# TeamOfProfGuo/Few_Shot_Seg_CWT

Measured on AMD Instinct MI355X. Metric: episodes/sec (473x473, 1-shot, R50) at 1/2/4/8 MI355X; mIoU vs ref, higher is better.
Workload: dtype fp32 (conv stack at fp32 width on the bf16 MFMA: every fp32 operand split exactly into bf16 hi + mid + lo, the six products >= 2^-24 |a||b| summed in fp32; inner loop, CWT, classifier fp32); 1 GPU; CWT inference episode (validate_transformer, batch_size_val=1): PASCAL split-0 1-shot ResNet-50 PSPNet 473x473, adapt_iter 200, heads 4; image_size=473, shot=1, layers=50

## Files before the change

### few_shot_seg_cwt_amd/_lib.py

```python
from __future__ import annotations

import ctypes as C
import os
import threading

import torch

_HERE = os.path.dirname(os.path.abspath(__file__))
LIB_PATH = os.environ.get("CWT_LIB_PATH") or os.path.join(_HERE, "libcwt.so")

_P = C.c_void_p
_I = C.c_int
_F = C.c_float
_I64 = C.c_int64

SIGNATURES = {
    "cwt_version": (C.c_char_p, []),
    "cwt_last_error": (C.c_char_p, []),
    "cwt_ctx_create": (_I, [_I, C.POINTER(_P)]),
    "cwt_ctx_destroy": (_I, [_P]),
    "cwt_backbone_load": (_I, [_P, _I, _I, C.POINTER(C.c_char_p), C.POINTER(_P), C.POINTER(_I64), _F,
                               C.POINTER(_P)]),
    "cwt_backbone_destroy": (_I, [_P]),
    "cwt_backbone_set_precision": (_I, [_P, _I]),
    "cwt_extract_features": (_I, [_P, _P, _P, _I, _I, _P, _P]),
    "cwt_extract_features_train_bn": (_I, [_P, _P, _P, _I, _I, _P, _F, _F, C.c_uint64, _P]),
    "cwt_backbone_read_bn": (_I, [_P, C.c_char_p, _P, _I]),
    "cwt_preprocess_image": (_I, [_P, _P, _I, _I, _I, _I, C.POINTER(_F), C.POINTER(_F), C.POINTER(_F), _I, _I, _P,
                                  _P]),
    "cwt_preprocess_label": (_I, [_P, _P, _I, _I, _I, _I, _I, _I, _P, _P]),
    "cwt_workspace_bytes": (C.c_size_t, [_P]),
    "cwt_inner_adapt": (_I, [_P, _P, _P, _I, _I, _I, _I, _I, _F, _I, _P, _P]),
    "cwt_inner_adapt_batch": (_I, [_P, _P, _P, _I, _I, _I, _I, _I, _I, _F, _I, _P, _P]),
    "cwt_normalize": (_I, [_P, _P, _I, _I, _I, _P, _P, _P, _P]),
    "cwt_attention_fwd": (_I, [_P, _P, _P, _I, _I, _I, _I, _P, _P, _P, _P, _P, _P, _P, _P]),
    "cwt_attention_saved_floats": (C.c_size_t, [_I, _I, _I, _I]),
    "cwt_attention_bwd": (_I, [_P, _P, _P, _I, _I, _I, _I, _P, _P, _P, _P, _P, _P, _P, _P, _P, _P, _P, _P, _P]),
    "cwt_attention_fwd_train": (_I, [_P, _P, _P, _I, _I, _I, _I, _P, _P, _P, _P, _P, _P, _P, _F, _F, C.c_uint64,
                                     _P]),
    "cwt_attention_bwd_train": (_I, [_P, _P, _P, _I, _I, _I, _I, _P, _P, _P, _P, _P, _P, _P, _P, _P, _P, _P, _P, _F,
                                     _F, C.c_uint64, _P]),
    "cwt_classify": (_I, [_P, _P, _P, _I, _I, _I, _P, _P]),
    "cwt_attention_infer": (_I, [_P, _P, _P, _I, _I, _I, _I, _P, _P, _P, _P, _P, _I64, _P, _P, _P, _P]),
    "cwt_classify_scaled": (_I, [_P, _P, _P, _P, _I, _I, _I, _P, _P]),
    "cwt_episode_tail": (_I, [_P, _P, _P, _I, _I, _I, _I, _P, _P, _P, _P, _P, _P, _I64, _P, _P, _P, _P, _P, _P,
                              _P]),
    "cwt_inner_adapt_tail": (_I, [_P, _P, _P, _I, _I, _I, _I, _I, _F, _I, _P, _P, _P, _P, _P, _P, _P, _P, _I64, _P, _P,
                                  _P, _P, _P, _P, _P]),
    "cwt_seg_metrics": (_I, [_P, _P, _P, _I, _I, _I, _I, _P, _P, _P]),
    "cwt_seg_metrics_pair": (_I, [_P, _P, _P, _P, _I, _I, _I, _I, _P, _P, _P, _P]),
    "cwt_seg_ce_fwd_bwd": (_I, [_P, _P, _P, _I, _I, _I, _I, _P, _P, _P]),
    "cwt_classify_bwd": (_I, [_P, _P, _P, _I, _I, _I, _P, _P]),
    "cwt_iou_preds": (_I, [_P, _P, _P, _I64, _I, _I, _P, _P]),
    "cwt_cos_classify": (_I, [_P, _P, _I, _I, _I, _I, _P, _P, _P, _P, _I, _P, _P]),
    "cwt_cos_classify_bwd": (_I, [_P, _P, _I, _I, _I, _I, _P, _P, _P, _P, _I, _P, _P, _P, _P, _P, _P]),
    "cwt_corr": (_I, [_P, _P, _P, _I, _I, _I, _I, _P, _P]),
    "cwt_mutual_matching": (_I, [_P, _P, _I, _I, _I, _I, _P, _P]),
    "cwt_match_corr_forward": (_I, [_P, _P, _I, _I, _I, _I, _P, _I, _F, _P, _I, _P, _P, _P]),
    "cwt_match_corr_forward_cv4": (_I, [_P, _P, _I, _I, _I, _I, _P, _I, _F, _P, _I, _P, _P, _P]),
    "cwt_match_masks": (_I, [_P, _P, _I, _I, _I, _P, _P, _P, _P]),
    "cwt_channel_sum": (_I, [_P, _P, _I, _I, _I64, _P, _P]),
    "cwt_sce_descriptor": (_I, [_P, _P, _I, _I, _I, _I, _I, _I, _P, _P]),
    "cwt_match_readout": (_I, [_P, _P, _I, _I, _I, _F, _P, _I, _P, _P]),
    "cwt_match_masks_train": (_I, [_P, _P, _I, _I, _I, _P, _P, _P, _F, C.c_uint64, _P]),
    "cwt_match_readout_backward": (_I, [_P, _P, _I, _I, _I, _F, _P, _I, _P, _P, _P, _P, _P]),
    "cwt_weight_average": (_I, [_P, _P, _I, _I, _I, _I, _P, _P, _P, _P, _P, _P, _P, _P]),
    "cwt_mmn_blend": (_I, [_P, _P, _P, _I, _I64, _F, _P, _P, _P]),
    "cwt_match_corr_saved_floats": (_I, [_I, _I, _I, _I, _I, _I, C.POINTER(_I64)]),
    "cwt_match_corr_forward_train": (_I, [_P, _P, _I, _I, _I, _I, _P, _I, _F, _P, _I, _P, _P, _P, _P]),
    "cwt_match_corr_backward": (_I, [_P, _P, _I, _I, _I, _I, _P, _I, _F, _P, _I, _P, _P, _P, _P, _P, _P, _P]),
    "cwt_corr_backward": (_I, [_P, _P, _P, _I, _I, _I, _I, _P, _P, _P, _I, _I, _P]),
    "cwt_weight_average_train": (_I, [_P, _P, _I, _I, _I, _I, _P, _P, _P, _P, _P, _P, _P, _P, _P, _P]),
    "cwt_weight_average_backward": (_I, [_P, _P, _I, _I, _I, _I, _P, _P, _P, _P, _P, _P, _P, _P, _P, _P, _P, _P, _P,
                                         _P, _P, _P]),
    "cwt_mmn_blend_backward": (_I, [_P, _P, _P, _I, _I64, _F, _P, _P, _P]),
    "cwt_linear_backward": (_I, [_P, _P, _I64, _I, _P, _I, _P, _P, _P, _P, _I, _P, _P]),
    "cwt_deform_attn_backward": (_I, [_P, _P, _P, _P, _I, _I, _I, _I, _I, _I, _P, _P, _P, _P, _P]),
    "cwt_norm_blend_backward": (_I, [_P, _P, _P, _I64, _I, _F, _P, _P, _P, _P]),
    "cwt_linear": (_I, [_P, _P, _I64, _I, _P, _P, _I, _I, _I, _P, _P]),
    "cwt_sine_pos_add": (_I, [_P, _P, _I, _I, _I, _I, _F, _I, _F, _F, _P, _P]),
    "cwt_deform_attn": (_I, [_P, _P, _P, _P, _I, _I, _I, _I, _I, _I, _P, _P]),
    "cwt_norm_blend": (_I, [_P, _P, _P, _I64, _I, _F, _P, _P]),
    "cwt_extract_features_mid": (_I, [_P, _P, _P, _I, _I, _P, _P, _P, _P, _P]),
    "cwt_sgd_step": (_I, [_P, _P, _P, _P, _I64, _F, _F, _F, _I, _I, _P]),
    "cwt_pretrain_create": (_I, [_P, _I, _I, _I, C.POINTER(C.c_char_p), C.POINTER(_P), C.POINTER(_I64), _F,
                                 C.POINTER(_P)]),
    "cwt_pretrain_destroy": (_I, [_P]),
    "cwt_pretrain_step": (_I, [_P, _P, _P, _P, _I, _I, _P, _P, _P]),
    "cwt_pretrain_forward": (_I, [_P, _P, _P, _I, _I, _I, _P, _P]),
    "cwt_pretrain_get": (_I, [_P, C.c_char_p, _I, _P, _I64]),
    "cwt_pretrain_evaluate": (_I, [_P, _P, _P, _P, _I, _I, _I, _P, _P, _P]),
    "cwt_pretrain_set": (_I, [_P, C.c_char_p, _I, _P, _I64]),
    "cwt_pretrain_num_params": (_I, [_P, C.POINTER(_I64), C.POINTER(_I64)]),
    "cwt_cu_count": (_I, [_P, _P]),
    "cwt_adapt_workgroups": (_I, [_P, _I, _I, _I, _I, _I, _P]),
    "cwt_adapt_fuses_tail": (_I, [_P, _I, _I, _I, _I, _P]),
    "cwt_stream_create_masked": (_I, [_P, _P, _I, _P]),
    "cwt_stream_destroy": (_I, [_P]),
    "cwt_debug_conv": (_I, [_P, _P, _I, _I, _I, _I, _I, _P, _P, _P, _I, _I, _I, _I, _I, _P, _I, _I, _P, _I, _I,
                            _I, _I, _I, _I, _P]),
    "cwt_debug_split_act": (_I, [_P, _P, _I64, _I, _I, _P, _P]),
    "cwt_debug_unsplit_act": (_I, [_P, _P, _I64, _I, _P, _I, _P]),
    "cwt_debug_pack_wsplit": (_I, [_P, _P, _I, _I, _I, _P, _P]),
    "cwt_debug_conv_s": (_I, [_P, _P, _I, _I, _I, _I, _P, _P, _P, _I, _I, _I, _I, _I, _P, _I, _P, _I, _P, _I, _I,
                              _P, _I, _I, _I, _P]),
    "cwt_debug_conv_b16": (_I, [_P, _P, _I, _I, _I, _I, _P, _P, _P, _I, _I, _I, _I, _I, _P, _I, _P, _I, _P, _I, _I,
                                _P, _I, _I, _I, _P]),
    "cwt_debug_cp4d_layer": (_I, [_P, _P, _I, _I, _I, _I, _I, _I, _I, _P, _P, _P, _P, _P, _I, _P]),
    "cwt_debug_conv_f32d": (_I, [_P, _P, _I, _I, _I, _I, _P, _P, _P, _I, _I, _I, _I, _I, _P, _I, _I, _P, _I, _I, _I,
                                 _I, _I, _P]),
    "cwt_debug_conv_x6": (_I, [_P, _P, _I, _I, _I, _I, _P, _P, _P, _I, _I, _I, _I, _I, _P, _I, _I, _P, _I, _I, _I,
                               _I, _I, _P]),
    "cwt_debug_conv_x6w": (_I, [_P, _P, _I, _I, _I, _I, _P, _P, _P, _I, _I, _I, _I, _I, _P, _I, _I, _P, _I, _I, _I,
                                _I, _I, _P]),
    "cwt_debug_conv_form": (_I, [_I, _I, _I, _I, C.POINTER(_I)]),
    "cwt_debug_conv_plan": (_I, [_I, _I, _I, _I, _I, C.POINTER(_I)]),
    "cwt_debug_census": (_I, [_P, _I, _P, _P]),
    "cwt_debug_tail_stamps": (_I, [_P, _P, _I64, _P]),
    "cwt_debug_occupy": (_I, [_P, _I, _I, _P]),
    "cwt_debug_pretrain_op": (_I, [_P, _I, C.POINTER(_P), C.POINTER(_I64), C.POINTER(_F), _P]),
    "cwt_debug_backbone_op": (_I, [_P, _I, C.POINTER(_P), C.POINTER(_I64), C.POINTER(_F), _P]),
    "cwt_debug_adapt_stamps": (_I, [_P, _P, _I64, C.POINTER(_I64)]),
    "cwt_ctx_set_adapt_units": (_I, [_P, _I]),
    "cwt_ctx_status": (_I, [_P, C.POINTER(C.c_uint32), _I]),
    "cwt_ctx_set_conv_arith": (_I, [_P, _I]),
    "cwt_debug_adapt_spin_limit": (_I, [_P, _I64]),
    "cwt_debug_pretrain_capture": (_I, [_P, _I]),
    "cwt_debug_pretrain_tensor": (_I, [_P, C.c_char_p, _P, _I64]),
    "cwt_profile_enable": (_I, [_P, _I]),
    "cwt_profile_count": (_I, [_P]),
    "cwt_profile_record": (_I, [_P, _I, C.c_char_p, _I, C.POINTER(C.c_double), C.POINTER(C.c_double),
                                C.POINTER(_F)]),
}

_lib = None
_lock = threading.RLock()
_ctx = {}


class CwtError(RuntimeError):
    pass


def check_provenance(version: str, path: str):
    from . import build as _build
    if os.environ.get("CWT_LIB_PATH") or not os.path.isdir(_build.CSRC):
        return
    want = _build.source_hash()
    got = version.rsplit("src=", 1)[-1] if "src=" in version else None
    if got != want:
        raise CwtError(f"{path} is stale: built from sources {got}, the tree's are {want}; "
                       "run `python -m few_shot_seg_cwt_amd.build`")


def load_library(path: str = LIB_PATH):
    global _lib
    with _lock:
        if _lib is None:
            if not os.path.exists(path):
                raise CwtError(f"{path} not built: run `python -m few_shot_seg_cwt_amd.build` "
                               "(the product path has no CPU fallback)")
            lib = C.CDLL(path)
            for name, (res, args) in SIGNATURES.items():
                fn = getattr(lib, name)
                fn.restype = res
                fn.argtypes = args
            check_provenance(lib.cwt_version().decode(), path)
            _lib = lib
    return _lib


def lib():
    return load_library()


def check(rc: int, what: str = ""):
    if rc != 0:
        msg = lib().cwt_last_error().decode(errors="replace")
        raise CwtError(f"{what} failed (code {rc}): {msg}")


_override = threading.local()
_extra_ctx = {}


def _create_ctx(device: int):
    p = C.c_void_p()
    rc = load_library().cwt_ctx_create(device, C.byref(p))
    if rc != 0:
        raise CwtError(f"cwt_ctx_create failed: {_lib.cwt_last_error().decode()}")
    return p


def ctx(device: int | None = None):
    if not torch.cuda.is_available():
        raise CwtError("libcwt needs a HIP device (torch.cuda.is_available() is False); no CPU fallback")
    if device is None:
        device = torch.cuda.current_device()
    sel = getattr(_override, "ctx", None)
    if sel is not None and sel[0] == device:
        return sel[1]
    with _lock:
        if device not in _ctx:
            _ctx[device] = _create_ctx(device)
        return _ctx[device]


def new_ctx(device: int | None = None):
    if device is None:
        device = torch.cuda.current_device()
    ctx(device)
    with _lock:
        p = _create_ctx(device)
        _extra_ctx.setdefault(device, []).append(p)
        return p


def destroy_ctx(p, device: int | None = None) -> None:
    if device is None:
        device = torch.cuda.current_device()
    with _lock:
        lst = _extra_ctx.get(device, [])
        for i, q in enumerate(lst):
            if q is p or getattr(q, "value", None) == getattr(p, "value", p):
                del lst[i]
                check(load_library().cwt_ctx_destroy(p), "cwt_ctx_destroy")
                return
    raise CwtError("destroy_ctx: not an additional context of this device")


class using_ctx:

    def __init__(self, c, device: int | None = None):
        self.c, self.device = c, torch.cuda.current_device() if device is None else device

    def __enter__(self):
        self.prev = getattr(_override, "ctx", None)
        _override.ctx = (self.device, self.c)
        return self.c

    def __exit__(self, *exc):
        _override.ctx = self.prev
        return False


def all_ctx(device: int | None = None):
    if device is None:
        device = torch.cuda.current_device()
    return [ctx(device)] + list(_extra_ctx.get(device, []))


STATUS_ADAPT_BARRIER = 1
STATUS_TAIL_BARRIER = 2


def check_status(device: int | None = None, clear: bool = True) -> None:
    w = C.c_uint32()
    bad = 0
    for c in all_ctx(device):
        check(lib().cwt_ctx_status(c, C.byref(w), int(clear)), "cwt_ctx_status")
        bad |= w.value
    if bad & STATUS_TAIL_BARRIER:
        raise CwtError("the fused episode tail's grid barrier timed out (its workgroups were not all co-resident): "
                       "the CWT output, logits and IoU counts of an episode on this device are wrong")
    if bad & STATUS_ADAPT_BARRIER:
        raise CwtError("the persistent inner loop's grid barrier timed out (its workgroups were not all "
                       "co-resident): the adapted classifier W of an episode on this device is wrong")
# ... 77 lines not shown
```

### few_shot_seg_cwt_amd/csrc/api_debug.hip

```cpp
#include <algorithm>
#include <cstdlib>

#include "../../include/cwt_debug.h"
#include "conv_forms.h"
#include "ctx.h"

using namespace cwt;

namespace cwt {
__global__ void census_kernel(unsigned* out) {
  unsigned hw, xcc;
  asm volatile("s_getreg_b32 %0, hwreg(HW_REG_HW_ID)" : "=s"(hw));
  asm volatile("s_getreg_b32 %0, hwreg(HW_REG_XCC_ID)" : "=s"(xcc));
  if (threadIdx.x == 0) {
    out[2 * blockIdx.x] = hw;
    out[2 * blockIdx.x + 1] = xcc;
  }
}
}

static int debug_conv_s(cwt_ctx* ctx, int prec, const void* xs, int N, int Hi, int Wi, int Ci, const void* ws,
                        const float* scale, const float* shift, int Co, int k, int stride, int pad, int dil,
                        const float* res, int res_ld, const void* res_s, int relu, float* y, int y_ld, int y_off,
                        void* ys, int bm, int bn, int nsplit, void* stream) {
// ... 96 lines not shown
  return launch_conv(a, p, 0, part, pf, (hipStream_t)stream);
}

int cwt_debug_census(cwt_ctx* ctx, int nblocks, unsigned* out, void* stream) {
  if (!ctx) return fail(CWT_EARG, "ctx is NULL");
  CWT_CHECK(out && nblocks > 0, "bad arguments");
  CWT_HIP(hipSetDevice(ctx->device));
  hipLaunchKernelGGL(census_kernel, dim3(nblocks), dim3(64), 0, (hipStream_t)stream, out);
  CWT_LAUNCH_CHECK();
  return 0;
}

int cwt_debug_split_act(cwt_ctx* ctx, const float* x, int64_t P, int C, int ld, void* out, void* stream) {
  if (!ctx) return fail(CWT_EARG, "ctx is NULL");
  CWT_CHECK(x && out && P >= 0 && C % 32 == 0 && ld >= C && ld % 4 == 0, "bad arguments");
  CWT_HIP(hipSetDevice(ctx->device));
  return launch_split_act(x, P, C, ld, (__bf16*)out, (hipStream_t)stream);
}

int cwt_debug_unsplit_act(cwt_ctx* ctx, const void* s, int64_t P, int C, float* out, int ld, void* stream) {
  if (!ctx) return fail(CWT_EARG, "ctx is NULL");
  CWT_CHECK(s && out && P >= 0 && C % 32 == 0 && ld >= C && ld % 4 == 0, "bad arguments");
  CWT_HIP(hipSetDevice(ctx->device));
  return launch_unsplit_act((const __bf16*)s, P, C, out, ld, (hipStream_t)stream);
}

int cwt_debug_pack_wsplit(cwt_ctx* ctx, const float* w, int Co, int k, int Ci, void* out, void* stream) {
  if (!ctx) return fail(CWT_EARG, "ctx is NULL");
  CWT_CHECK(w && out && Co > 0 && Ci % 32 == 0 && (k == 1 || k == 3), "bad arguments");
  CWT_HIP(hipSetDevice(ctx->device));
  float* wp;
  int rc;
  const long K = (long)k * k * Ci;
  if ((rc = ws(ctx, "dbg.wpack", (size_t)Co * K, &wp))) return rc;
  if ((rc = launch_repack_cblock(w, wp, Co, k * k, Ci, (hipStream_t)stream))) return rc;
  return launch_split_act(wp, Co, (int)K, (int)K, (__bf16*)out, (hipStream_t)stream);
}

int cwt_debug_backbone_op(cwt_ctx* ctx, int op, void* const* b, const int64_t* ia, const float* fa, void* stream) {
  if (!ctx) return fail(CWT_EARG, "ctx is NULL");
  CWT_CHECK(b && ia, "null argument");
  CWT_HIP(hipSetDevice(ctx->device));
  hipStream_t st = (hipStream_t)stream;
  auto lay_ok = [](int64_t l) { return l == ACT_F32 || l == ACT_SPLIT || l == ACT_BF16; };
  float* p;
  int rc;
  if (op == 0) {
    const int N = (int)ia[0], S = (int)ia[1];
    CWT_CHECK(b[0] && b[1] && b[2] && b[3] && b[4] && N > 0 && S > 0 && lay_ok(ia[2]), "stem conv1");
    return launch_stem_conv1((const float*)b[0], N, S, (const float*)b[1], (const float*)b[2], (const float*)b[3],
                             (float*)b[4], down2(S), st, (int)ia[2], (int)ia[3]);
  }
  if (op == 1) {
    const int N = (int)ia[0], H = (int)ia[1], W = (int)ia[2], C = (int)ia[3], lay = (int)ia[4];
    CWT_CHECK(b[0] && b[1] && N > 0 && H > 0 && W > 0 && C > 0 && lay_ok(ia[4]), "maxpool");
    const int Ho = down2(H), Wo = down2(W);
    if (lay == ACT_BF16) return launch_maxpool3s2_b16((const __bf16*)b[0], N, H, W, C, (__bf16*)b[1], Ho, Wo, st);
    if (lay == ACT_SPLIT) return launch_maxpool3s2_s((const __bf16*)b[0], N, H, W, C, (__bf16*)b[1], Ho, Wo, st);
    CWT_CHECK(C % 4 == 0, "maxpool: C % 4");
    return launch_maxpool3s2((const float*)b[0], N, H, W, C, (float*)b[1], Ho, Wo, st);
  }
  if (op == 2) {
    const int N = (int)ia[0], h = (int)ia[1], w = (int)ia[2], ld = (int)ia[3];
    CWT_CHECK(b[0] && b[1] && N > 0 && h > 0 && w > 0 && ld >= 2048 && lay_ok(ia[4]), "ppm");
    if ((rc = ws(ctx, "dbg.ppm", ((size_t)N * h * 16 + (size_t)N * 256) * 2048, &p))) return rc;
    return launch_ppm((const float*)b[0], N, h, w, ld, kBins, 4, p, (float*)b[1], st, (int)ia[4]);
  }
  if (op == 3) {
    int M[4];
    const float *Bt[4], *sc[4], *sh[4];
    long Mtot = 0;
    int nbn = 0;
    for (int q = 0; q < 4; ++q) {
      CWT_CHECK(ia[q] > 0 && ia[q] <= 4096 && b[1 + q], "ppm gemm: problem");
      M[q] = (int)ia[q];
      Mtot += M[q];
      Bt[q] = (const float*)b[1 + q];
      sc[q] = (const float*)b[5 + q];
      sh[q] = (const float*)b[9 + q];
      CWT_CHECK(!sc[q] == !sh[q], "ppm gemm: scale without shift");
      nbn += sc[q] != nullptr;
    }
    const int N = (int)ia[4], K = (int)ia[5], kc = (int)ia[6];
    int form = (int)ia[7];
    CWT_CHECK(b[0] && b[13] && N > 0 && K > 0 && (nbn == 0 || nbn == 4) && form <= 1, "ppm gemm");
    if (form < 0) form = Mtot <= kPpmGemmMaxRows ? 0 : 1;
    CWT_CHECK(form == 0 || kc == 32 || kc == 64, "ppm gemm: K chunk");
    const size_t part_floats = (size_t)(form == 0 ? 8 : K / kc) * Mtot * N;
    if ((rc = ws(ctx, "dbg.parts", part_floats, &p))) return rc;
    return form == 0 ? launch_ppm_gemm((const float*)b[0], K, Bt, M, 4, N, K, nbn ? sc : nullptr, nbn ? sh : nullptr,
                                       p, part_floats, (float*)b[13], st)
                     : launch_smallm_gemm((const float*)b[0], K, Bt, M, 4, N, K, kc, p, part_floats,
                                          nbn ? sc : nullptr, nbn ? sh : nullptr, (float*)b[13], st);
  }
  if (op == 4) {
    CWT_CHECK(fa && b[0] && b[2] && b[3] && b[4] && ia[0] > 0 && ia[1] > 0 && ia[1] <= 2048 && lay_ok(ia[2]) &&
                  ia[6] > 0,
              "bn_train");
    BnTrainArgs a;
    memset(&a, 0, sizeof(a));
    a.y = b[0];
    a.M = (long)ia[0];
    a.C = (int)ia[1];
    a.layout = (int)ia[2];
    a.ld = (int)ia[3];
    a.res = b[1];
    a.res_ld = (int)ia[4];
    a.relu = (int)ia[5];
    a.rows_per_image = (long)ia[6];
    a.seed = (unsigned long long)ia[7];
    a.bn = (float*)b[2];
    a.scale = (float*)b[3];
    a.shift = (float*)b[4];
    a.eps = fa[0];
    a.momentum = fa[1];
    a.drop_p = fa[2];
    CWT_CHECK(a.layout != ACT_F32 || a.ld >= a.C, "bn_train: ld < C");
    const size_t pf = bn_train_part_floats(a.M, a.C);
    float* bsc;
    if ((rc = ws(ctx, "dbg.bn.part", pf, &p)) || (rc = ws(ctx, "dbg.bn.bsc", 2 * 2048, &bsc))) return rc;
    return launch_bn_train(a, p, pf, bsc, st);
  }
  if (op == 5) {
    CWT_CHECK(b[0] && b[1] && ia[0] > 0, "widen");
    return launch_widen_bf16((const __bf16*)b[0], (long)ia[0], (float*)b[1], st);
  }
  return fail(CWT_EARG, "cwt_debug_backbone_op: unknown op");
}

int cwt_debug_conv_s(cwt_ctx* ctx, const void* xs, int N, int Hi, int Wi, int Ci, const void* ws, const float* scale,
                     const float* shift, int Co, int k, int stride, int pad, int dil, const float* res, int res_ld,
                     const void* res_s, int relu, float* y, int y_ld, int y_off, void* ys, int bm, int bn, int nsplit,
                     void* stream) {
  return debug_conv_s(ctx, 3, xs, N, Hi, Wi, Ci, ws, scale, shift, Co, k, stride, pad, dil, res, res_ld, res_s, relu, y,
                      y_ld, y_off, ys, bm, bn, nsplit, stream);
}

int cwt_debug_conv_f32d(cwt_ctx* ctx, const float* x, int N, int Hi, int Wi, int Ci, const float* w_packed,
                        const float* scale, const float* shift, int Co, int k, int stride, int pad, int dil,
                        const float* res, int res_ld, int relu, float* y, int y_ld, int y_off, int bm, int bn,
                        int nsplit, void* stream) {
  return debug_conv_s(ctx, 0, x, N, Hi, Wi, Ci, w_packed, scale, shift, Co, k, stride, pad, dil, res, res_ld, nullptr,
                      relu, y, y_ld, y_off, nullptr, bm, bn, nsplit, stream);
}

int cwt_debug_conv_x6(cwt_ctx* ctx, const float* x, int N, int Hi, int Wi, int Ci, const float* w_packed,
                      const float* scale, const float* shift, int Co, int k, int stride, int pad, int dil,
                      const float* res, int res_ld, int relu, float* y, int y_ld, int y_off, int bm, int bn,
                      int nsplit, void* stream) {
  return debug_conv_s(ctx, 6, x, N, Hi, Wi, Ci, w_packed, scale, shift, Co, k, stride, pad, dil, res, res_ld, nullptr,
                      relu, y, y_ld, y_off, nullptr, bm, bn, nsplit, stream);
}

int cwt_debug_conv_form(int prec, int bm, int bn, int var, int* out4) {
  CWT_CHECK(out4, "out4 is NULL");
  const ConvForm* f = find_conv_form(prec, bm, bn, var);
  if (!f) return fail(CWT_EARG, "no such conv form (conv_forms.h)");
  out4[0] = f->waves_m;
  out4[1] = f->waves_n;
  out4[2] = f->nstg;
  out4[3] = f->pf;
  return 0;
}

int cwt_debug_conv_plan(int prec, int M, int Co, int K, int batch, int* out5) {
  CWT_CHECK(out5 && M > 0 && Co > 0 && K > 0 && batch >= 0, "bad arguments");
  CWT_CHECK(prec == 0 || prec == 1 || prec == 3 || prec == 6, "prec must be 0, 1, 3 or 6");
  const ConvPlan p = plan_conv_s(prec, M, Co, K, batch);
  const int v[5] = {p.bm, p.bn, p.var, p.nsplit, p.kt_per_split};
  std::copy(v, v + 5, out5);
  if (!find_conv_form(prec, p.bm, p.bn, p.var)) return fail(CWT_EARG, "the plan's form is no such conv form");
  return 0;
}

int cwt_debug_conv_x6w(cwt_ctx* ctx, const float* x, int N, int Hi, int Wi, int Ci, const float* w_packed,
                       const float* scale, const float* shift, int Co, int k, int stride, int pad, int dil,
                       const float* res, int res_ld, int relu, float* y, int y_ld, int y_off, int bm, int bn,
                       int nsplit, void* stream) {
  const int m = nsplit == 4 ? 4 : 2;
  if (!ctx) return fail(CWT_EARG, "ctx is NULL");
  CWT_CHECK(x && w_packed && scale && shift && y, "null buffer");
  CWT_CHECK(nsplit == 0 || nsplit == 1 || nsplit == 2 || nsplit == 4, "nsplit (the Winograd tile) must be 0, 2 or 4");
  CWT_CHECK(k == 3 && stride == 1 && pad == dil && dil >= 1, "winograd form: 3x3, stride 1, padding = dilation");
  CWT_CHECK(Ci % 32 == 0 && Co % 64 == 0 && N >= 1 && Hi >= 1 && Wi >= 1, "need Ci % 32 == 0, Co % 64 == 0");
  CWT_CHECK(y_ld >= y_off + Co && y_ld % 4 == 0 && y_off % 4 == 0 && (!res || res_ld % 4 == 0), "bad strides");
  int rc;
  ConvPlan named;
  if (bm > 0 && (rc = force_conv_form(6, bm, bn, Co, &named))) return rc;
  CWT_HIP(hipSetDevice(ctx->device));
  const hipStream_t st = (hipStream_t)stream;
  const int P = (m + 2) * (m + 2);
  const size_t n = (size_t)P * Co * Ci;
  float* U;
  __bf16 *us, *ul;
  if ((rc = ws(ctx, "dbg.wU", n, &U)) || (rc = ws(ctx, "dbg.wUs", n * 2, &us)) || (rc = ws(ctx, "dbg.wUl", n, &ul)))
    return rc;
  static const bool w3_cache = getenv("CWT_DBG_W3_CACHE") && getenv("CWT_DBG_W3_CACHE")[0] == '1';
  static const void* u_src = nullptr;
  static long u_n = 0;
  static void* u_dst = nullptr;
  if (!(w3_cache && u_src == w_packed && u_n == (long)n * m && u_dst == us)) {
    if ((rc = launch_wino_weights(w_packed, Co, Ci, U, st, m)) ||
        (rc = launch_split_w3(U, (long)P * Co, Ci, us, ul, st)))
      return rc;
    u_src = w_packed;
    u_n = (long)n * m;
    u_dst = us;
  }
  return run_wino_conv(ctx, x, N, Hi, Wi, Ci, Co, dil, m, us, ul, scale, shift, res, res_ld, relu, y, y_ld, y_off, 0,
                       st, bm, bn);
}

int cwt_debug_conv_b16(cwt_ctx* ctx, const void* xs, int N, int Hi, int Wi, int Ci, const void* ws, const float* scale,
                       const float* shift, int Co, int k, int stride, int pad, int dil, const float* res, int res_ld,
                       const void* res_s, int relu, float* y, int y_ld, int y_off, void* ys, int bm, int bn,
                       int nsplit, void* stream) {
  return debug_conv_s(ctx, 1, xs, N, Hi, Wi, Ci, ws, scale, shift, Co, k, stride, pad, dil, res, res_ld, res_s, relu, y,
                      y_ld, y_off, ys, bm, bn, nsplit, stream);
}

int cwt_debug_cp4d_layer(cwt_ctx* ctx, const float* x, int B, int hA, int wA, int hB, int wB, int cin, int cout,
                         const float* Wa, const float* ba, const float* Wb, const float* bb, float* y, int variant,
                         void* stream) {
  if (!ctx || !x || !Wa || !ba || !Wb || !bb || !y) return fail(CWT_EARG, "null argument");
  if (B < 1 || hA < 1 || wA < 1 || hB < 1 || wB < 1) return fail(CWT_EARG, "bad shape");
  return launch_cp4d_layer_variant(x, B, hA, wA, hB, wB, cin, cout, Wa, ba, Wb, bb, y, variant, (hipStream_t)stream);
}

int cwt_debug_occupy(cwt_ctx* ctx, int nwg, int us, void* stream) {
  if (!ctx) return fail(CWT_EARG, "ctx is NULL");
  CWT_CHECK(nwg >= 1 && nwg <= 256 && us >= 1 && us <= 100000, "occupy: 1 <= nwg <= 256, 1 <= us <= 100000");
  CWT_HIP(hipSetDevice(ctx->device));
  return launch_occupy(nwg, us, (hipStream_t)stream);
}

int cwt_debug_tail_stamps(cwt_ctx* ctx, unsigned long long* host_out, int64_t max_count, int64_t* count) {
  if (!ctx || !count) return fail(CWT_EARG, "null argument");
  CWT_HIP(hipSetDevice(ctx->device));
  auto it = ctx->ws.find("tail.stamps");
  *count = (it == ctx->ws.end() || !ctx->tail_stamp_G) ? 0 : (int64_t)ctx->tail_stamp_G * 16;
  if (host_out && *count > 0 && max_count > 0) {
    CWT_HIP(hipDeviceSynchronize());
    CWT_HIP(hipMemcpy(host_out, it->second.p, (size_t)std::min<int64_t>(max_count, *count) * 8, hipMemcpyDeviceToHost));
  }
  return 0;
}

int cwt_debug_adapt_stamps(cwt_ctx* ctx, unsigned long long* host_out, int64_t max_count, int64_t* count) {
  if (!ctx || !count) return fail(CWT_EARG, "null argument");
  CWT_HIP(hipSetDevice(ctx->device));
  *count = g_adapt_stamps ? g_adapt_stamps_n : 0;
  if (host_out && g_adapt_stamps && max_count > 0) {
    CWT_HIP(hipDeviceSynchronize());
    CWT_HIP(hipMemcpy(host_out, g_adapt_stamps, (size_t)std::min<int64_t>(max_count, g_adapt_stamps_n) * 8,
                      hipMemcpyDeviceToHost));
  }
  return 0;
}

int cwt_debug_adapt_spin_limit(cwt_ctx* ctx, int64_t limit) {
  if (!ctx) return fail(CWT_EARG, "ctx is NULL");
  CWT_CHECK(limit >= 0, "limit must be >= 0");
  ctx->adapt_spin_limit = (long)limit;
  return 0;
}

}
```

### few_shot_seg_cwt_amd/csrc/api_extract.hip

```cpp
#include <algorithm>
#include <cmath>
#include <cstdlib>

#include "conv_forms.h"
#include "ctx.h"

namespace cwt {

struct Block {
  ConvLayer c1, c2, c3, down;
  bool has_down = false;
};

struct Backbone {
  int layers = 0;
  int device = 0;
  int precision = CWT_CONV_FP32;
  ConvLayer stem[3];
  std::vector<Block> blocks[4];
  ConvLayer ppm[4];
  float* ppm_wt[4] = {};
  ConvLayer bott;
  float* ppm_q[4] = {};
  float* ppm_q_raw[4] = {};
  float* ones = nullptr;
  float* zeros = nullptr;
  float eps = 1e-5f;
  std::map<std::string, std::pair<float*, int>> bn_by_name;
  std::vector<void*> allocs;
};

struct HostParams {
  std::map<std::string, std::pair<const float*, int64_t>> m;
  const float* get(const std::string& k, int64_t numel, std::string* err) const {
    auto it = m.find(k);
    if (it == m.end() || it->second.first == nullptr) {
      *err = "missing tensor '" + k + "'";
      return nullptr;
    }
    if (it->second.second != numel) {
      *err = "tensor '" + k + "' has " + std::to_string(it->second.second) + " elements, expected " +
             std::to_string(numel);
      return nullptr;
    }
    return it->second.first;
  }
};

static int upload(Backbone* bb, const std::vector<float>& v, float** out) {
  void* p = nullptr;
  CWT_HIP(hipMalloc(&p, v.size() * sizeof(float)));
  CWT_HIP(hipMemcpy(p, v.data(), v.size() * sizeof(float), hipMemcpyHostToDevice));
  bb->allocs.push_back(p);
  *out = (float*)p;
  return 0;
}

static uint16_t bf16_rne(float f) {
  uint32_t u;
  memcpy(&u, &f, 4);
  if ((u & 0x7F800000u) == 0x7F800000u) return (uint16_t)(u >> 16);
  u += 0x7FFFu + ((u >> 16) & 1u);
  return (uint16_t)(u >> 16);
}

static float bf16_to_float(uint16_t h) {
  uint32_t u = (uint32_t)h << 16;
  float f;
  memcpy(&f, &u, 4);
  return f;
}

static int upload_u16(Backbone* bb, const std::vector<uint16_t>& v, __bf16** out) {
  void* p = nullptr;
  CWT_HIP(hipMalloc(&p, v.size() * sizeof(uint16_t)));
  CWT_HIP(hipMemcpy(p, v.data(), v.size() * sizeof(uint16_t), hipMemcpyHostToDevice));
  bb->allocs.push_back(p);
  *out = (__bf16*)p;
  return 0;
}

static int load_conv(Backbone* bb, const HostParams& hp, const std::string& wname, const std::string& bnp, int Ci,
                     int Co, int k, int stride, int pad, int dil, float eps, bool stem1, ConvLayer* L,
                     int ci_total = -1, int ci_off = 0) {
  if (ci_total < 0) ci_total = Ci;
  std::string err;
  const float* w = hp.get(wname, (int64_t)Co * ci_total * k * k, &err);
  if (!w) return fail(CWT_EARG, err);
  const float* g = hp.get(bnp + ".weight", Co, &err);
  const float* b = g ? hp.get(bnp + ".bias", Co, &err) : nullptr;
  const float* rm = b ? hp.get(bnp + ".running_mean", Co, &err) : nullptr;
  const float* rv = rm ? hp.get(bnp + ".running_var", Co, &err) : nullptr;
  if (!rv) return fail(CWT_EARG, err);
  L->Ci = Ci;
  L->Co = Co;
  L->k = k;
  L->stride = stride;
  L->pad = pad;
  L->dil = dil;
  const int K = k * k * Ci;
  std::vector<float> packed((size_t)Co * K);
  for (int co = 0; co < Co; ++co)
    for (int ci = 0; ci < Ci; ++ci)
      for (int ky = 0; ky < k; ++ky)
        for (int kx = 0; kx < k; ++kx) {
          const float v = w[(((size_t)co * ci_total + ci_off + ci) * k + ky) * k + kx];
          if (stem1)
            packed[((size_t)(ci * 9 + ky * 3 + kx)) * Co + co] = v;
          else
            packed[(size_t)co * K + packed_k(ci, ky * k + kx, k * k)] = v;
        }
  std::vector<float> sc(Co), sh(Co);
  for (int c = 0; c < Co; ++c) {
    const float invstd = 1.0f / std::sqrt(rv[c] + eps);
    sc[c] = g[c] * invstd;
    sh[c] = b[c] - rm[c] * sc[c];
  }
  int rc;
  if ((rc = upload(bb, packed, &L->w))) return rc;
  if (!stem1) {
    std::vector<uint16_t> hi(packed.size()), lo(packed.size()), lo3(packed.size());
    for (size_t i = 0; i < packed.size(); ++i) {
      const float v = packed[i];
      hi[i] = bf16_rne(v);
      const float r = v - bf16_to_float(hi[i]);
      lo[i] = bf16_rne(r);
      lo3[i] = bf16_rne(r - bf16_to_float(lo[i]));
    }
    std::vector<uint16_t> sl(2 * packed.size());
    for (size_t r = 0; r < (size_t)Co; ++r)
      for (int kb = 0; kb < K / 32; ++kb)
        for (int i = 0; i < 32; ++i) {
          const size_t src = r * K + kb * 32 + i, dst = (r * (K / 32) + kb) * 64 + i;
          sl[dst] = hi[src];
          sl[dst + 32] = lo[src];
        }
    if ((rc = upload_u16(bb, sl, &L->w_s))) return rc;
    if (K % 32 == 0 && (rc = upload_u16(bb, lo3, &L->w_l))) return rc;
    static const bool wino4 = getenv("CWT_WINO") && getenv("CWT_WINO")[0] == '4';
    if (k == 3 && stride == 1 && Ci >= 128 && Ci % 32 == 0) {
      for (const int m : {2, 4}) {
        if ((m == 2 && Ci < 256) || (m == 4 && !wino4)) continue;
        const int P = (m + 2) * (m + 2);
        const size_t n = (size_t)P * Co * Ci;
        void *U = nullptr, *us = nullptr, *ul = nullptr;
        CWT_HIP(hipMalloc(&us, n * 4));
        bb->allocs.push_back(us);
        CWT_HIP(hipMalloc(&ul, n * 2));
        bb->allocs.push_back(ul);
        CWT_HIP(hipMalloc(&U, n * 4));
        rc = launch_wino_weights(L->w, Co, Ci, (float*)U, nullptr, m);
        if (!rc) rc = launch_split_w3((const float*)U, (long)P * Co, Ci, (__bf16*)us, (__bf16*)ul, nullptr);
        const hipError_t e = hipDeviceSynchronize();
        (void)hipFree(U);
        if (rc) return rc;
        if (e != hipSuccess) return fail((int)e, "winograd weight transform");
        (m == 2 ? L->wino_s : L->wino4_s) = (__bf16*)us;
        (m == 2 ? L->wino_l : L->wino4_l) = (__bf16*)ul;
      }
    }
    if (Ci % 64 == 0) {
      std::vector<uint16_t> b16(packed.size());
      for (int co = 0; co < Co; ++co)
        for (int ci = 0; ci < Ci; ++ci)
          for (int tap = 0; tap < k * k; ++tap)
            b16[(size_t)co * K + packed_k64(ci, tap, k * k)] = hi[(size_t)co * K + packed_k(ci, tap, k * k)];
      if ((rc = upload_u16(bb, b16, &L->w_b))) return rc;
    }
  }
  if ((rc = upload(bb, sc, &L->scale))) return rc;
  if ((rc = upload(bb, sh, &L->shift))) return rc;
  std::vector<float> bnp4((size_t)4 * Co);
  for (int c = 0; c < Co; ++c) {
    bnp4[c] = g[c];
    bnp4[Co + c] = b[c];
    bnp4[2 * Co + c] = rm[c];
    bnp4[3 * Co + c] = rv[c];
  }
  if ((rc = upload(bb, bnp4, &L->bn))) return rc;
  bb->bn_by_name[bnp] = {L->bn, Co};
  return 0;
}

static int load_ppm_fold(Backbone* bb, const HostParams& hp, float eps) {
  std::string err;
  for (int b = 0; b < 4; ++b) {
    const float* w = hp.get("ppm.features." + std::to_string(b) + ".1.weight", (int64_t)512 * 2048, &err);
    if (!w) return fail(CWT_EARG, err);
    std::vector<float> t((size_t)2048 * 512);
    for (int co = 0; co < 512; ++co)
      for (int ci = 0; ci < 2048; ++ci) t[(size_t)ci * 512 + co] = w[(size_t)co * 2048 + ci];
    int rc;
    if ((rc = upload(bb, t, &bb->ppm_wt[b]))) return rc;
  }
  const float* w = hp.get("bottleneck.0.weight", (int64_t)512 * 4096 * 9, &err);
  const float* g = w ? hp.get("bottleneck.1.weight", 512, &err) : nullptr;
  const float* rv = g ? hp.get("bottleneck.1.running_var", 512, &err) : nullptr;
  if (!rv) return fail(CWT_EARG, err);
  for (int b = 0; b < 4; ++b) {
    std::vector<float> q((size_t)512 * 4608), qr((size_t)512 * 4608);
    for (int co = 0; co < 512; ++co) {
      const float sc = g[co] * (1.0f / std::sqrt(rv[co] + eps));
      for (int ci = 0; ci < 512; ++ci)
        for (int tap = 0; tap < 9; ++tap) {
          const float v = w[((size_t)co * 4096 + 2048 + 512 * b + ci) * 9 + tap];
          qr[(size_t)ci * 4608 + tap * 512 + co] = v;
          q[(size_t)ci * 4608 + tap * 512 + co] = v * sc;
        }
    }
    int rc;
    if ((rc = upload(bb, q, &bb->ppm_q[b])) || (rc = upload(bb, qr, &bb->ppm_q_raw[b]))) return rc;
  }
  return 0;
}

static int load_backbone(int layers, const HostParams& hp, float eps, Backbone** out) {
  if (layers != 50 && layers != 101) return fail(CWT_EARG, "layers must be 50 or 101");
  Backbone* bb = new Backbone();
  bb->layers = layers;
  bb->eps = eps;
  int rc = 0;
  auto cleanup = [&]() {
    for (void* p : bb->allocs) (void)hipFree(p);
    delete bb;
  };
  if ((rc = load_conv(bb, hp, "layer0.0.weight", "layer0.1", 3, 64, 3, 2, 1, 1, eps, true, &bb->stem[0])) ||
      (rc = load_conv(bb, hp, "layer0.3.weight", "layer0.4", 64, 64, 3, 1, 1, 1, eps, false, &bb->stem[1])) ||
      (rc = load_conv(bb, hp, "layer0.6.weight", "layer0.7", 64, 128, 3, 1, 1, 1, eps, false, &bb->stem[2]))) {
    cleanup();
    return rc;
  }
  const int* nb = (layers == 50) ? kBlocks50 : kBlocks101;
  int inplanes = 128;
  const int planes_of[4] = {64, 128, 256, 512};
  for (int li = 0; li < 4; ++li) {
    const int planes = planes_of[li];
    for (int bi = 0; bi < nb[li]; ++bi) {
      Block B;
      int s2 = 1, d2 = 1, sd = 1;
      if (li == 1 && bi == 0) {
        s2 = 2;
        sd = 2;
      }
      if (li == 2) d2 = 2;
      if (li == 3) d2 = 4;
      const std::string p = "layer" + std::to_string(li + 1) + "." + std::to_string(bi);
      if ((rc = load_conv(bb, hp, p + ".conv1.weight", p + ".bn1", inplanes, planes, 1, 1, 0, 1, eps, false, &B.c1)) ||
          (rc = load_conv(bb, hp, p + ".conv2.weight", p + ".bn2", planes, planes, 3, s2, d2, d2, eps, false, &B.c2)) ||
          (rc = load_conv(bb, hp, p + ".conv3.weight", p + ".bn3", planes, planes * 4, 1, 1, 0, 1, eps, false,
                          &B.c3))) {
        cleanup();
        return rc;
      }
      if (bi == 0) {
        B.has_down = true;
        if ((rc = load_conv(bb, hp, p + ".downsample.0.weight", p + ".downsample.1", inplanes, planes * 4, 1, sd, 0, 1,
                            eps, false, &B.down))) {
          cleanup();
          return rc;
        }
      }
      inplanes = planes * 4;
      bb->blocks[li].push_back(B);
    }
  }
  for (int i = 0; i < 4; ++i) {
    const std::string p = "ppm.features." + std::to_string(i);
    if ((rc = load_conv(bb, hp, p + ".1.weight", p + ".2", 2048, 512, 1, 1, 0, 1, eps, false, &bb->ppm[i]))) {
      cleanup();
      return rc;
    }
  }
  if ((rc = load_conv(bb, hp, "bottleneck.0.weight", "bottleneck.1", 2048, 512, 3, 1, 1, 1, eps, false, &bb->bott,
                      4096, 0)) ||
      (rc = load_ppm_fold(bb, hp, eps)) || (rc = upload(bb, std::vector<float>(2048, 1.0f), &bb->ones)) ||
      (rc = upload(bb, std::vector<float>(2048, 0.0f), &bb->zeros))) {
    cleanup();
    return rc;
  }
  *out = bb;
  return 0;
}

ConvArgs make_args(const ConvCall& c) {
  ConvArgs a;
  memset(&a, 0, sizeof(a));
  const ConvLayer& L = *c.L;
  a.x = c.x;
  a.w = L.w;
  a.scale = L.scale;
  a.shift = L.shift;
  a.res = c.res;
  a.y = c.y;
  a.N = c.N;
  a.Hi = c.Hi;
  a.Wi = c.Wi;
  a.Ci = L.Ci;
  a.x_ld = c.x_ld;
  a.Ho = conv_out_size(c.Hi, L.k, L.stride, L.pad, L.dil);
  a.Wo = conv_out_size(c.Wi, L.k, L.stride, L.pad, L.dil);
  a.Co = L.Co;
  a.kh = a.kw = L.k;
  a.stride = L.stride;
  a.pad = L.pad;
  a.dil = L.dil;
  a.M = c.N * a.Ho * a.Wo;
  a.K = L.k * L.k * L.Ci;
  a.y_ld = c.y_ld;
  a.y_off = c.y_off;
  a.res_ld = c.res_ld;
  a.relu = c.relu;
  return a;
}

static int wino_tile_default(int Ci, int Co, int d, int Ho) {
  (void)Co;
  (void)d;
  (void)Ho;
  return Ci >= 256 ? 2 : 0;
}

int force_conv_form(int prec, int bm, int bn, int Co, ConvPlan* p) {
  const int var = bm / 1000;
  bm %= 1000;
  CWT_CHECK(find_conv_form(prec, bm, bn, 0),
            "tile must be one of 256x256, 256x128, 128x256, 128x128, 128x64, 64x128, 64x64");
  const ConvForm* f = fixed_tile_form(prec, var);
  if (!f) f = find_conv_form(prec, bm, bn, var);
  CWT_CHECK(f, "no such conv form: the variant does not exist on this tile (conv_forms.h)");
  CWT_CHECK(Co % f->bn == 0, "Co % bn");
  p->bm = f->bm;
  p->bn = f->bn;
  p->var = var;
  return 0;
}

int run_wino_conv(cwt_ctx* ctx, const float* x, int N, int H, int W, int Ci, int Co, int d, int m,
                         const __bf16* us, const __bf16* ul, const float* scale, const float* shift, const float* res,
                         int res_ld, int relu, float* y, int y_ld, int y_off, int stage, hipStream_t st, int bm,
                         int bn) {
  if (m != 2 && m != 4) return fail(CWT_EARG, "winograd: output tile must be 2 or 4");
  const WinoGeom g = wino_geom(N, H, W, d, m);
  if (g.T * Ci * 4 >= (1L << 31) || g.T * Co * 4 >= (1L << 31)) return fail(CWT_EARG, "winograd: plane too large");
  float *V, *Mb;
  const __bf16* zero = nullptr;
  int rc;
  ConvPlan p = plan_conv_s(6, (int)g.T, Co, Ci, g.P);
  if (bm > 0 && (rc = force_conv_form(6, bm, bn, Co, &p))) return rc;
  if ((rc = ws(ctx, "wino.V", (size_t)g.P * g.T * Ci, &V)) || (rc = ws(ctx, "wino.M", (size_t)g.P * g.T * Co, &Mb)) ||
      (rc = zero_line(ctx, &zero)))
    return rc;
  const int plev = 3;
  (void)stage;
  const double vb = 4.0 * g.P * g.T * Ci, mb = 4.0 * g.P * g.T * Co;
  Prof pin(ctx, st, "wino_in " + std::to_string(Ci) + "@" + std::to_string(H), 0.0,
           4.0 * N * H * W * Ci + vb, plev);
  rc = launch_wino_in(x, g, Ci, V, st);
  pin.end();
  if (rc) return rc;
  ConvSArgs a = conv_s_geom(1, (int)g.T, 1, Ci, Co, 1, 1, 0, 1);
  a.xs = (const __bf16*)V;
  a.ws = us;
  a.ws_lo = ul;
  a.zero = zero;
  a.scale = scale;
  a.shift = shift;
  a.part = Mb;
  a.batch = g.P;
  a.xs_bstride = g.T * Ci * 4;
  a.ws_bstride = (long)Co * Ci * 2;
  a.wl_bstride = (long)Co * Ci;
  Prof pg(ctx, st, "wino_gemm " + std::to_string(Ci) + "x" + std::to_string(Co) + "@" + std::to_string(H),
          2.0 * g.P * g.T * Ci * Co, vb + 6.0 * g.P * Co * Ci + mb, plev);
  rc = launch_conv_x3s(a, p, m == 4 ? 8 : stage == 6 ? 6 : 7, nullptr, 0, st, 6);
  pg.end();
  if (rc) return rc;
  const double ob = 4.0 * N * H * W * Co * (res ? 2.0 : 1.0);
  Prof pout(ctx, st, "wino_out " + std::to_string(Co) + "@" + std::to_string(H), 0.0, mb + ob, plev);
  rc = launch_wino_out(Mb, g, Co, scale, shift, res, res_ld, relu, y, y_ld, y_off, st);
  pout.end();
  return rc;
}

struct TrainBn {
  float momentum, drop_p;
  unsigned long long seed;
};

static int run_extract(cwt_ctx* ctx, const Backbone* bb, const float* img, int N, int S, float* feat,
                       hipStream_t st, const TrainBn* tb = nullptr, float* const* mid = nullptr) {
  const bool b16 = bb->precision == CWT_CONV_BF16 && !tb;
  const bool conv_split = ctx->conv_arith == CWT_CONV_ARITH_BF16X3 && !tb;
  const bool s_path = b16 || conv_split;
  const int layout = b16 ? ACT_BF16 : conv_split ? ACT_SPLIT : ACT_F32;
  static const bool f32d_env = !(getenv("CWT_CONV_F32D") && getenv("CWT_CONV_F32D")[0] == '0');
  const bool x6 = !s_path && !tb && ctx->conv_arith == CWT_CONV_ARITH_BF16X6;
  const bool f32d = !s_path && !tb && !x6 && f32d_env;
  const bool f32ops = f32d || x6;
  const bool dma = s_path || f32ops;
  const int prec = b16 ? 1 : conv_split ? 3 : x6 ? 6 : 0;
  const int Hs = down2(S), H1 = down2(Hs), h = down2(H1);
  const long sA = std::max({(long)N * Hs * Hs * 128, (long)N * H1 * H1 * 256, (long)N * h * h * 2048});
  const long sT1 = std::max((long)N * H1 * H1 * 128, (long)N * h * h * 512);
  const long sT2 = std::max((long)N * H1 * H1 * 64, (long)N * h * h * 512);
  const long sD = std::max((long)N * H1 * H1 * 256, (long)N * h * h * 2048);
  const long sCol = (long)N * h * 16 * 2048 + (long)N * 16 * 16 * 2048;
  const long sPool = (long)N * 50 * 2048;
  const long sPpm = (long)N * 50 * 512;
  const long sQ = (long)N * 50 * 4608;
  const long sR = (long)N * 12 * h * 3 * 512;
  const long sF = (long)N * h * h * 512;
  constexpr int kKcPpm = 32, kKcQ = 64;
  const long sPartS = std::max((long)(2048 / kKcPpm) * N * 50 * 512, (long)(512 / kKcQ) * N * 50 * 4608);

  float *A, *B, *T1, *T2, *D, *COL, *POOL, *PPM, *QB, *RB, *FB, *PARTS;
  int rc;
  if ((rc = ws(ctx, "bb.A", sA, &A)) || (rc = ws(ctx, "bb.B", sA, &B)) || (rc = ws(ctx, "bb.T1", sT1, &T1)) ||
      (rc = ws(ctx, "bb.T2", sT2, &T2)) || (rc = ws(ctx, "bb.D", sD, &D)) || (rc = ws(ctx, "bb.COL", sCol, &COL)) ||
      (rc = ws(ctx, "bb.POOL", sPool, &POOL)) || (rc = ws(ctx, "bb.PPM", sPpm, &PPM)) ||
      (rc = ws(ctx, "bb.Q", sQ, &QB)) || (rc = ws(ctx, "bb.R", sR, &RB)) || (rc = ws(ctx, "bb.F", sF, &FB)) ||
      (rc = ws(ctx, "bb.PARTS", sPartS, &PARTS)))
    return rc;

  std::vector<ConvCall> calls;
  std::vector<ConvArgs> args;
  int stage = 0;
  auto cc = [&](const ConvLayer* L, const float* x, int n, int Hi, int Wi, int x_ld, float* y, int y_ld, int y_off,
                const float* res, int res_ld, int relu) {
    ConvCall c{stage, L, x, n, Hi, Wi, x_ld, y, y_ld, y_off, res, res_ld, relu, stage == 6};
    calls.push_back(c);
    args.push_back(make_args(c));
  };
  cc(&bb->stem[1], A, N, Hs, Hs, 64, B, 64, 0, nullptr, 0, 1);
  cc(&bb->stem[2], B, N, Hs, Hs, 64, A, 128, 0, nullptr, 0, 1);
  const size_t n_stem_calls = calls.size();
  size_t last_of_layer[4] = {0, 0, 0, 0};
  float* cur = B;
  float* other = A;
  int H = H1;
  for (int li = 0; li < 4; ++li) {
    stage = li + 1;
    const int nbk = (int)bb->blocks[li].size();
    for (int bi = 0; bi < nbk; ++bi) {
      const Block& blk = bb->blocks[li][bi];
      const int Cin = blk.c1.Ci;
      const int Ho = (blk.c2.stride == 2) ? down2(H) : H;
      cc(&blk.c1, cur, N, H, H, Cin, T1, blk.c1.Co, 0, nullptr, 0, 1);
      cc(&blk.c2, T1, N, H, H, blk.c2.Ci, T2, blk.c2.Co, 0, nullptr, 0, 1);
      const float* res = cur;
      int res_ld = Cin;
      if (blk.has_down) {
        cc(&blk.down, cur, N, H, H, Cin, D, blk.down.Co, 0, nullptr, 0, 0);
        res = D;
        res_ld = blk.down.Co;
      }
      cc(&blk.c3, T2, N, Ho, Ho, blk.c3.Ci, other, blk.c3.Co, 0, res, res_ld, 1);
      if (bi == nbk - 1) last_of_layer[li] = calls.size() - 1;
      std::swap(cur, other);
      H = Ho;
    }
  }
  const size_t n_backbone_calls = calls.size();
  const float* L4 = cur;
  stage = 6;
  cc(&bb->bott, L4, N, h, h, 2048, feat, 512, 0, FB, 512, 1);

  size_t part_floats = 0;
  std::vector<ConvPlan> plans;
  for (size_t i = 0; i < calls.size(); ++i) {
    const ConvArgs& a = args[i];
    if (b16 && !calls[i].L->w_b) return fail(CWT_ESTATE, "bf16 conv weights missing (Ci % 64 != 0)");
    ConvPlan pl = dma ? plan_conv_s(prec, a.M, a.Co, a.K) : plan_conv(a.M, a.Co, a.K);
    plans.push_back(pl);
    if (pl.nsplit > 1) part_floats = std::max(part_floats, (size_t)pl.nsplit * a.M * a.Co);
  }
  const __bf16* zero = nullptr;
  if (dma && (rc = zero_line(ctx, &zero))) return rc;
  float *BNPART = nullptr, *BNSC = nullptr;
  size_t bn_part_floats = 0;
  if (tb) {
    bn_part_floats = bn_train_part_floats((long)N * Hs * Hs, 64);
    for (auto& a : args) bn_part_floats = std::max(bn_part_floats, bn_train_part_floats(a.M, a.Co));
    if ((rc = ws(ctx, "bn.part", bn_part_floats, &BNPART)) || (rc = ws(ctx, "bn.bsc", 2 * 2048, &BNSC))) return rc;
  }
  auto bn_train = [&](const ConvLayer* L, void* y, int lay, int ld, long M, const void* res, int res_ld, int relu,
                      float drop_p, long rows_per_image) -> int {
    BnTrainArgs b;
    memset(&b, 0, sizeof(b));
    b.y = y;
    b.layout = lay;
    b.ld = ld;
    b.M = M;
    b.C = L->Co;
    b.res = res;
    b.res_ld = res_ld;
    b.relu = relu;
    b.bn = L->bn;
    b.scale = L->scale;
    b.shift = L->shift;
    b.eps = bb->eps;
    b.momentum = tb->momentum;
    b.drop_p = drop_p;
    b.seed = tb->seed;
    b.rows_per_image = rows_per_image;
    return launch_bn_train(b, BNPART, bn_part_floats, BNSC, st);
  };
  float* PART = nullptr;
  if (part_floats && (rc = ws(ctx, "bb.PART", part_floats, &PART))) return rc;
  auto c_wino = [&](const ConvCall& c) {
    return (c.L->wino_s || c.L->wino4_s) && c.L->k == 3 && c.L->stride == 1 && c.L->pad == c.L->dil &&
           c.x_ld == c.L->Ci;
  };
  auto run_call = [&](size_t i) -> int {
    ConvArgs a = args[i];
    const bool keep_res = calls[i].stage == 6;
    if (tb) {
      a.scale = bb->ones;
      a.shift = bb->zeros;
      a.relu = 0;
      if (!keep_res) a.res = nullptr;
    }
    static const int wino_env = getenv("CWT_WINO") && getenv("CWT_WINO")[0] ? atoi(getenv("CWT_WINO")) : -1;
    int wm = x6 && wino_env != 0 && c_wino(calls[i])
                 ? (wino_env == 2 || wino_env == 4 ? wino_env : wino_tile_default(a.Ci, a.Co, a.dil, a.Ho))
                 : 0;
    if (wm && !(wm == 4 ? calls[i].L->wino4_s : calls[i].L->wino_s)) wm = 0;
    const bool wino = wm != 0;
    const WinoGeom wg = wino_geom(a.N, a.Hi, a.Wi, a.dil, wm ? wm : 2);
    const ConvPlan pl = wino ? plan_conv_s(6, (int)wg.T, a.Co, a.Ci, wg.P) : plans[i];
    const double flops = 2.0 * a.M * a.Co * a.K;
    const double eb = b16 ? 2.0 : 4.0, ob = calls[i].out_f32 ? 4.0 : eb;
    const double bytes = eb * ((double)a.N * a.Hi * a.Wi * a.Ci + (double)a.Co * a.K) +
                         ob * ((double)a.M * a.Co + (a.res ? (double)a.M * a.Co : 0.0));
    Prof p(ctx, st,
           std::string(b16 ? "conv_igemm_b16<" : conv_split ? "conv_igemm_x3s<" : wino ? (wm == 4 ? "conv_igemm_x6w4<" : "conv_igemm_x6w<")
                       : x6 ? "conv_igemm_x6<" : f32d ? "conv_igemm_f32d<" : "conv_igemm_f32<") +
               std::to_string(pl.bm) + "," +
               std::to_string(pl.bn) + "," +
               std::to_string(calls[i].stage) + ">" +
               (pl.nsplit > 1 ? "+splitk" + std::to_string(pl.nsplit) : std::string()) + " " +
               std::to_string(a.Ci) + "x" + std::to_string(a.Co) + "k" + std::to_string(a.kh) + "s" +
               std::to_string(a.stride) + "d" + std::to_string(a.dil) + "@" + std::to_string(a.Ho),
           flops, bytes, calls[i].stage == 6 ? 1 : 2);
    int r;
    if (wino) {
      const ConvCall& c = calls[i];
      r = run_wino_conv(ctx, c.x, a.N, a.Hi, a.Wi, a.Ci, a.Co, a.dil, wm, wm == 4 ? c.L->wino4_s : c.L->wino_s,
                        wm == 4 ? c.L->wino4_l : c.L->wino_l, a.scale, a.shift, a.res, c.res_ld, a.relu, c.y, c.y_ld,
                        c.y_off, c.stage, st);
    } else if (dma) {
      ConvSArgs sa = conv_s_geom(a.N, a.Hi, a.Wi, a.Ci, a.Co, a.kh, a.stride, a.pad, a.dil);
      const ConvCall& c = calls[i];
      sa.xs = (const __bf16*)c.x;
      sa.ws = b16 ? c.L->w_b : f32d ? (const __bf16*)c.L->w : c.L->w_s;
      sa.ws_lo = x6 ? c.L->w_l : nullptr;
      sa.zero = zero;
      sa.scale = a.scale;
      sa.shift = a.shift;
      if (c.out_f32 || f32ops) {
        sa.y = c.y;
        sa.y_ld = c.y_ld;
        sa.y_off = c.y_off;
        sa.res = a.res;
        sa.res_ld = c.res_ld;
      } else {
        sa.ys = (__bf16*)c.y;
        sa.res_s = (const __bf16*)a.res;
      }
      sa.relu = a.relu;
      r = launch_conv_x3s(sa, pl, c.stage, PART, part_floats, st, prec);
    } else {
      r = launch_conv(a, pl, calls[i].stage, PART, part_floats, st);
    }
    p.end();
    if (r || !tb) return r;
    const ConvCall& c = calls[i];
    const bool f32 = c.out_f32 || !s_path;
    return bn_train(c.L, c.y, f32 ? ACT_F32 : layout, f32 ? c.y_ld : c.L->Co, a.M, keep_res ? nullptr : c.res,
                    f32 ? c.res_ld : c.L->Co, c.relu, c.stage == 6 ? tb->drop_p : 0.f, (long)a.Ho * a.Wo);
  };

  const long cells = (long)N * 50;
  const double ppm_flops = 2.0 * cells * 512 * 2048 + 2.0 * cells * 4608 * 512 +
                           2.0 * N * 12 * h * 3 * 512 * 3 * 6 + 2.0 * N * h * h * 512 * 36;
  double all_flops = 2.0 * N * Hs * Hs * 64 * 27 + ppm_flops, all_bytes = 0.0;
  for (auto& a : args) {
    all_flops += 2.0 * a.M * a.Co * a.K;
    all_bytes += 4.0 * ((double)a.N * a.Hi * a.Wi * a.Ci + (double)a.Co * a.K + (double)a.M * a.Co);
  }
  Prof whole(ctx, st, "extract_features N=" + std::to_string(N) + " S=" + std::to_string(S), all_flops, all_bytes, 1);
  {
    Prof p(ctx, st, "stem_conv1 3x64k3s2", 2.0 * N * Hs * Hs * 64 * 27, 4.0 * ((double)N * 3 * S * S + (double)N * Hs * Hs * 64));
    if ((rc = launch_stem_conv1(img, N, S, bb->stem[0].w, tb ? bb->ones : bb->stem[0].scale,
                                tb ? bb->zeros : bb->stem[0].shift, A, Hs, st, layout, tb ? 0 : 1)))
      return rc;
    p.end();
    if (tb && (rc = bn_train(&bb->stem[0], A, layout, 64, (long)N * Hs * Hs, nullptr, 0, 1, 0.f, (long)Hs * Hs)))
      return rc;
  }
  for (size_t i = 0; i < n_stem_calls; ++i)
    if ((rc = run_call(i))) return rc;
  {
    Prof p(ctx, st, "maxpool3s2", 0.0, 4.0 * ((double)N * Hs * Hs * 128 + (double)N * H1 * H1 * 128));
    if ((rc = layout == ACT_BF16    ? launch_maxpool3s2_b16((const __bf16*)A, N, Hs, Hs, 128, (__bf16*)B, H1, H1, st)
              : layout == ACT_SPLIT ? launch_maxpool3s2_s((const __bf16*)A, N, Hs, Hs, 128, (__bf16*)B, H1, H1, st)
                                    : launch_maxpool3s2(A, N, Hs, Hs, 128, B, H1, H1, st)))
      return rc;
    p.end();
  }
  for (size_t i = n_stem_calls; i < n_backbone_calls; ++i) {
    if ((rc = run_call(i))) return rc;
    for (int li = 1; li < 4 && mid; ++li) {
      if (i != last_of_layer[li] || !mid[li - 1]) continue;
      const ConvCall& c = calls[i];
      const ConvArgs& a = args[i];
      const long P = (long)a.M;
      if (layout == ACT_SPLIT)
        rc = launch_unsplit_act((const __bf16*)c.y, P, a.Co, mid[li - 1], a.Co, st);
      else if (layout == ACT_BF16)
        rc = launch_widen_bf16((const __bf16*)c.y, P * a.Co, mid[li - 1], st);
      else {
        const hipError_t e = hipMemcpyAsync(mid[li - 1], c.y, (size_t)P * a.Co * 4, hipMemcpyDeviceToDevice, st);
        rc = e == hipSuccess ? 0 : fail((int)e, "mid feature copy");
      }
      if (rc) return rc;
    }
  }
  {
    Prof p(ctx, st, "ppm_pool", 0.0, 4.0 * ((double)N * h * h * 2048 + (double)N * 50 * 2048));
    if ((rc = launch_ppm(L4, N, h, h, 2048, kBins, 4, COL, POOL, st, layout))) return rc;
    p.end();
  }
  int Mb[4];
  const float *Wp[4], *Wq[4], *Sc[4], *Sh[4];
  static const bool ppm_splitk = getenv("CWT_PPM_SPLITK") != nullptr;
  const bool few_cells = cells <= kPpmGemmMaxRows && !ppm_splitk;
  for (int i = 0; i < 4; ++i) {
    Mb[i] = N * kBins[i] * kBins[i];
    Wp[i] = bb->ppm_wt[i];
    Wq[i] = tb ? bb->ppm_q_raw[i] : bb->ppm_q[i];
    Sc[i] = bb->ppm[i].scale;
    Sh[i] = bb->ppm[i].shift;
  }
  {
    Prof p(ctx, st, "ppm_conv smallm 2048x512", 2.0 * cells * 512 * 2048, 4.0 * (4.0 * 2048 * 512 + cells * 2560.0));
    if ((rc = few_cells ? launch_ppm_gemm(POOL, 2048, Wp, Mb, 4, 512, 2048, tb ? nullptr : Sc, tb ? nullptr : Sh, PARTS,
                                          (size_t)sPartS, PPM, st)
                        : launch_smallm_gemm(POOL, 2048, Wp, Mb, 4, 512, 2048, kKcPpm, PARTS, (size_t)sPartS,
                                             tb ? nullptr : Sc, tb ? nullptr : Sh, PPM, st)))
      return rc;
    p.end();
  }
  if (tb) {
    long row0 = 0;
    for (int i = 0; i < 4; ++i) {
      if ((rc = bn_train(&bb->ppm[i], PPM + row0 * 512, ACT_F32, 512, Mb[i], nullptr, 0, 1, 0.f,
                         (long)kBins[i] * kBins[i])))
        return rc;
      row0 += Mb[i];
    }
  }
  {
    Prof p(ctx, st, "ppm_fold_q smallm 512x4608", 2.0 * cells * 4608 * 512, 4.0 * (4.0 * 512 * 4608 + cells * 5120.0));
    if ((rc = few_cells ? launch_ppm_gemm(PPM, 512, Wq, Mb, 4, 4608, 512, nullptr, nullptr, PARTS, (size_t)sPartS, QB, st)
                        : launch_smallm_gemm(PPM, 512, Wq, Mb, 4, 4608, 512, kKcQ, PARTS, (size_t)sPartS, nullptr,
                                             nullptr, QB, st)))
      return rc;
    p.end();
  }
  {
    Prof p(ctx, st, "ppm_field", 2.0 * N * 12 * h * 3 * 512 * 3 * 6 + 2.0 * N * h * h * 512 * 36,
           4.0 * ((double)cells * 4608 + 2.0 * sR + sF));
    if ((rc = launch_ppm_field(QB, N, h, h, kBins, RB, FB, st))) return rc;
    p.end();
  }
  rc = run_call(n_backbone_calls);
  whole.end();
  if (!rc && tb)
    for (int i = 0; i < 4 && !rc; ++i)
      rc = launch_scale_cols(bb->ppm_q_raw[i], bb->ppm_q[i], 512L * 4608, 512, bb->bott.scale, st);
  return rc;
}

}

using namespace cwt;

extern "C" {

int cwt_backbone_load(cwt_ctx* ctx, int layers, int n_tensors, const char* const* names,
                      const float* const* host_data, const int64_t* numel, float bn_eps, cwt_backbone** out) {
  if (!ctx || !names || !host_data || !numel || n_tensors <= 0 || !out) return fail(CWT_EARG, "null argument");
  CWT_HIP(hipSetDevice(ctx->device));
  HostParams hp;
  for (int i = 0; i < n_tensors; ++i) hp.m[names[i]] = {host_data[i], numel[i]};
  Backbone* bb = nullptr;
  int rc = load_backbone(layers, hp, bn_eps, &bb);
  if (rc) return rc;
  bb->device = ctx->device;
  *out = reinterpret_cast<cwt_backbone*>(bb);
  return 0;
}

int cwt_backbone_destroy(cwt_backbone* handle) {
  Backbone* bb = reinterpret_cast<Backbone*>(handle);
  if (!bb) return 0;
  (void)hipSetDevice(bb->device);
  (void)hipDeviceSynchronize();
  for (void* p : bb->allocs) (void)hipFree(p);
  delete bb;
  return 0;
}

int cwt_backbone_set_precision(cwt_backbone* handle, int precision) {
  Backbone* bb = reinterpret_cast<Backbone*>(handle);
  if (!bb) return fail(CWT_EARG, "backbone is NULL");
  if (precision != CWT_CONV_FP32 && precision != CWT_CONV_BF16)
    return fail(CWT_EARG, "precision must be CWT_CONV_FP32 (0) or CWT_CONV_BF16 (1)");
  bb->precision = precision;
  return 0;
}

int cwt_extract_features(cwt_ctx* ctx, const cwt_backbone* handle, const float* img, int N, int S, float* feat,
                         void* stream) {
  if (!ctx) return fail(CWT_EARG, "ctx is NULL");
  const Backbone* bb = reinterpret_cast<const Backbone*>(handle);
  if (!bb) return fail(CWT_ESTATE, "backbone is NULL (cwt_backbone_load)");
  if (bb->device != ctx->device) return fail(CWT_EARG, "backbone and context are on different devices");
  CWT_CHECK(img && feat, "null buffer");
  CWT_CHECK(N >= 1 && S >= 9 && (S - 1) % 8 == 0, "need N >= 1 and (S-1) % 8 == 0 (pspnet.py:150)");
  CWT_HIP(hipSetDevice(ctx->device));
  return run_extract(ctx, bb, img, N, S, feat, (hipStream_t)stream);
}

int cwt_extract_features_mid(cwt_ctx* ctx, const cwt_backbone* handle, const float* img, int N, int S, float* feat,
                             float* l2, float* l3, float* l4, void* stream) {
  if (!ctx) return fail(CWT_EARG, "ctx is NULL");
  const Backbone* bb = reinterpret_cast<const Backbone*>(handle);
  if (!bb) return fail(CWT_ESTATE, "backbone is NULL (cwt_backbone_load)");
  if (bb->device != ctx->device) return fail(CWT_EARG, "backbone and context are on different devices");
  CWT_CHECK(img && feat, "null buffer");
  CWT_CHECK(N >= 1 && S >= 9 && (S - 1) % 8 == 0, "need N >= 1 and (S-1) % 8 == 0 (pspnet.py:150)");
  CWT_HIP(hipSetDevice(ctx->device));
  float* const mid[3] = {l2, l3, l4};
  return run_extract(ctx, bb, img, N, S, feat, (hipStream_t)stream, nullptr, mid);
}

int cwt_extract_features_train_bn(cwt_ctx* ctx, cwt_backbone* handle, const float* img, int N, int S, float* feat,
                                  float momentum, float dropout_p, uint64_t seed, void* stream) {
  if (!ctx) return fail(CWT_EARG, "ctx is NULL");
  Backbone* bb = reinterpret_cast<Backbone*>(handle);
  if (!bb) return fail(CWT_ESTATE, "backbone is NULL (cwt_backbone_load)");
  if (bb->device != ctx->device) return fail(CWT_EARG, "backbone and context are on different devices");
  CWT_CHECK(img && feat, "null buffer");
  CWT_CHECK(N >= 1 && S >= 9 && (S - 1) % 8 == 0, "need N >= 1 and (S-1) % 8 == 0 (pspnet.py:150)");
  CWT_CHECK(N >= 2, "Expected more than 1 value per channel when training (the PPM bin-1 BatchNorm2d needs N >= 2)");
  CWT_CHECK(momentum >= 0.f && momentum <= 1.f && dropout_p >= 0.f && dropout_p < 1.f, "bad momentum / dropout_p");
  CWT_HIP(hipSetDevice(ctx->device));
  TrainBn tb{momentum, dropout_p, (unsigned long long)seed};
  return run_extract(ctx, bb, img, N, S, feat, (hipStream_t)stream, &tb);
}

int cwt_backbone_read_bn(const cwt_backbone* handle, const char* name, float* out, int C) {
  const Backbone* bb = reinterpret_cast<const Backbone*>(handle);
  if (!bb) return fail(CWT_ESTATE, "backbone is NULL (cwt_backbone_load)");
  CWT_CHECK(name && out, "null argument");
  auto it = bb->bn_by_name.find(name);
  if (it == bb->bn_by_name.end()) return fail(CWT_EARG, std::string("no BatchNorm2d named ") + name);
  CWT_CHECK(it->second.second == C, "C does not match the BatchNorm2d's channel count");
  CWT_HIP(hipSetDevice(bb->device));
  CWT_HIP(hipDeviceSynchronize());
  CWT_HIP(hipMemcpy(out, it->second.first, sizeof(float) * 4 * C, hipMemcpyDeviceToHost));
  return 0;
}

int cwt_preprocess_image(cwt_ctx* ctx, const void* src, int src_dtype, int H, int W, int S, const float* mean,
                         const float* std_, const float* pad, int flip_h, int flip_v, float* dst, void* stream) {
  if (!ctx) return fail(CWT_EARG, "ctx is NULL");
  CWT_CHECK(src && dst && mean && std_, "null argument");
  CWT_CHECK(src_dtype == CWT_U8 || src_dtype == CWT_F32, "src_dtype must be CWT_U8 or CWT_F32");
  CWT_CHECK(H >= 1 && W >= 1 && S >= 8, "bad sizes");
  CWT_HIP(hipSetDevice(ctx->device));
  return launch_episode_image(src, src_dtype == CWT_F32, H, W, S, mean, std_, pad, flip_h, flip_v, dst,
                              (hipStream_t)stream);
}

int cwt_preprocess_label(cwt_ctx* ctx, const uint8_t* src, int H, int W, int S, int class_chosen, int flip_h,
                         int flip_v, int64_t* dst, void* stream) {
  if (!ctx) return fail(CWT_EARG, "ctx is NULL");
  CWT_CHECK(src && dst, "null argument");
  CWT_CHECK(H >= 1 && W >= 1 && S >= 8, "bad sizes");
  CWT_HIP(hipSetDevice(ctx->device));
  return launch_episode_label(src, H, W, S, class_chosen, flip_h, flip_v, (long long*)dst, (hipStream_t)stream);
}

}
```

### few_shot_seg_cwt_amd/csrc/bn_train.hip

```cpp
#include "common.h"
#include "kernels.h"

namespace cwt {

typedef __bf16 bf16x8 __attribute__((ext_vector_type(8)));

constexpr int kBnRows = 256;

__device__ __forceinline__ float act_load1(const void* y, int layout, int ld, int C, long row, int c) {
  if (layout == ACT_F32) return ((const float*)y)[row * ld + c];
  if (layout == ACT_BF16) return (float)((const __bf16*)y)[row * C + c];
  const __bf16* p = (const __bf16*)y + (row * (C >> 5) + (c >> 5)) * 64 + (c & 31);
  return (float)p[0] + (float)p[32];
}

__device__ __forceinline__ void act_load8(const void* y, int layout, int ld, int C, long row, int c0, float* v) {
  if (layout == ACT_F32) {
    const float* p = (const float*)y + row * ld + c0;
    const f32x4 a = *(const f32x4*)p, b = *(const f32x4*)(p + 4);
#pragma unroll
    for (int q = 0; q < 4; ++q) {
      v[q] = a[q];
      v[q + 4] = b[q];
    }
// ... 6 lines not shown
    const bf16x8 h = *(const bf16x8*)p, l = *(const bf16x8*)(p + 32);
#pragma unroll
    for (int q = 0; q < 8; ++q) v[q] = (float)h[q] + (float)l[q];
  }
}

__device__ __forceinline__ void act_store8(void* y, int layout, int ld, int C, long row, int c0, const float* v) {
  if (layout == ACT_F32) {
    float* p = (float*)y + row * ld + c0;
    *(f32x4*)p = f32x4{v[0], v[1], v[2], v[3]};
    *(f32x4*)(p + 4) = f32x4{v[4], v[5], v[6], v[7]};
  } else if (layout == ACT_BF16) {
    bf16x8 h;
#pragma unroll
    for (int q = 0; q < 8; ++q) h[q] = (__bf16)v[q];
    *(bf16x8*)((__bf16*)y + row * C + c0) = h;
  } else {
    bf16x8 h, l;
#pragma unroll
    for (int q = 0; q < 8; ++q) {
      h[q] = (__bf16)v[q];
      l[q] = (__bf16)(v[q] - (float)h[q]);
    }
    __bf16* p = (__bf16*)y + (row * (C >> 5) + (c0 >> 5)) * 64 + (c0 & 31);
    *(bf16x8*)p = h;
    *(bf16x8*)(p + 32) = l;
  }
}

__global__ __launch_bounds__(256) void bn_stats_kernel(const void* __restrict__ y, int layout, int ld, long M, int C,
                                                       float* __restrict__ part) {
  __shared__ float sn[4][64], sm[4][64], sq[4][64];
  const int lane = threadIdx.x & 63, rg = threadIdx.x >> 6;
  const int c = blockIdx.y * 64 + lane;
  const long r0 = (long)blockIdx.x * kBnRows;
  float n = 0.f, mean = 0.f, m2 = 0.f;
  if (c < C) {
    for (int i = rg; i < kBnRows; i += 4) {
      const long r = r0 + i;
      if (r >= M) break;
      const float v = act_load1(y, layout, ld, C, r, c);
      n += 1.f;
      const float d = v - mean;
      mean += d / n;
      m2 += d * (v - mean);
    }
  }
  sn[rg][lane] = n;
  sm[rg][lane] = mean;
  sq[rg][lane] = m2;
  __syncthreads();
  if (rg == 0 && c < C) {
    for (int g = 1; g < 4; ++g) {
      const float nb = sn[g][lane];
      if (nb == 0.f) continue;
      const float nt = n + nb, d = sm[g][lane] - mean;
      mean += d * (nb / nt);
      m2 += sq[g][lane] + d * d * (n * nb / nt);
      n = nt;
    }
    const long plane = (long)gridDim.x * C;
    const long o = (long)blockIdx.x * C + c;
    part[o] = n;
    part[plane + o] = mean;
    part[2 * plane + o] = m2;
  }
}

__global__ void bn_finalize_kernel(const float* __restrict__ part, int nblk, int C, float* __restrict__ bn,
                                   float* __restrict__ scale, float* __restrict__ shift, float eps, float momentum,
                                   float* __restrict__ bsc) {
  const int c = blockIdx.x * blockDim.x + threadIdx.x;
  if (c >= C) return;
  const long plane = (long)nblk * C;
  double n = 0.0, mean = 0.0, m2 = 0.0;
  for (int b = 0; b < nblk; ++b) {
    const double nb = part[(long)b * C + c];
    if (nb == 0.0) continue;
    const double mb = part[plane + (long)b * C + c], qb = part[2 * plane + (long)b * C + c];
    const double nt = n + nb, d = mb - mean;
    mean += d * (nb / nt);
    m2 += qb + d * d * (n * nb / nt);
    n = nt;
  }
  const float gamma = bn[c], beta = bn[C + c];
  const float var_b = (float)(m2 / n);
  const float mu = (float)mean;
  const float sc = gamma / sqrtf(var_b + eps);
  bsc[c] = sc;
  bsc[C + c] = beta - mu * sc;
  const float rm = (1.f - momentum) * bn[2 * C + c] + momentum * mu;
  const float rv = (1.f - momentum) * bn[3 * C + c] + momentum * (float)(m2 / (n - 1.0));
  bn[2 * C + c] = rm;
  bn[3 * C + c] = rv;
  const float esc = gamma * (1.0f / sqrtf(rv + eps));
  scale[c] = esc;
  shift[c] = beta - rm * esc;
}

__global__ __launch_bounds__(256) void bn_apply_kernel(BnTrainArgs a, const float* __restrict__ bsc) {
  const long idx = (long)blockIdx.x * blockDim.x + threadIdx.x;
  const int cg = a.C >> 3;
  if (idx >= a.M * cg) return;
  const long row = idx / cg;
  const int c0 = (int)(idx - row * cg) * 8;
  float v[8], r[8];
  act_load8(a.y, a.layout, a.ld, a.C, row, c0, v);
  if (a.res) act_load8(a.res, a.layout, a.res_ld, a.C, row, c0, r);
  const long img = row / a.rows_per_image;
#pragma unroll
  for (int q = 0; q < 8; ++q) {
    const int c = c0 + q;
    float t = fmaf(v[q], bsc[c], bsc[a.C + c]);
    if (a.res) t += r[q];
    if (a.relu) t = fmaxf(t, 0.f);
    if (a.drop_p > 0.f) t *= dropout_scale(a.drop_p, a.seed, 3, (unsigned long long)img * a.C + c);
    v[q] = t;
  }
  act_store8(a.y, a.layout, a.ld, a.C, row, c0, v);
}

size_t bn_train_part_floats(long M, int C) { return (size_t)3 * cdiv(M, (long)kBnRows) * C; }

int launch_bn_train(const BnTrainArgs& a, float* part, size_t part_floats, float* batch_sc, hipStream_t st) {
  if (a.M < 2) return fail(CWT_EARG, "Expected more than 1 value per channel when training (BatchNorm2d)");
  if (a.C % 64 != 0 || (a.layout == ACT_F32 && (a.ld % 4 != 0 || a.res_ld % 4 != 0)))
    return fail(CWT_EARG, "bn_train: C % 64 == 0 and 16 B aligned rows required");
  if (bn_train_part_floats(a.M, a.C) > part_floats) return fail(CWT_ESTATE, "bn_train: partial workspace too small");
  const int nblk = (int)cdiv(a.M, (long)kBnRows);
  hipLaunchKernelGGL(bn_stats_kernel, dim3(nblk, a.C / 64), dim3(256), 0, st, (const void*)a.y, a.layout, a.ld, a.M,
                     a.C, part);
  CWT_LAUNCH_CHECK();
  hipLaunchKernelGGL(bn_finalize_kernel, dim3(cdiv(a.C, 256)), dim3(256), 0, st, (const float*)part, nblk, a.C, a.bn,
                     a.scale, a.shift, a.eps, a.momentum, batch_sc);
  CWT_LAUNCH_CHECK();
  const long total = a.M * (a.C / 8);
  hipLaunchKernelGGL(bn_apply_kernel, dim3(cdiv(total, 256L)), dim3(256), 0, st, a, (const float*)batch_sc);
  CWT_LAUNCH_CHECK();
  return 0;
}

__global__ void scale_cols_kernel(const float* __restrict__ src, float* __restrict__ dst, long n, int period,
                                  const float* __restrict__ sc) {
  const long i = (long)blockIdx.x * blockDim.x + threadIdx.x;
  if (i < n) dst[i] = src[i] * sc[i % period];
}

int launch_scale_cols(const float* src, float* dst, long n, int period, const float* sc, hipStream_t st) {
  hipLaunchKernelGGL(scale_cols_kernel, dim3(cdiv(n, 256L)), dim3(256), 0, st, src, dst, n, period, sc);
  CWT_LAUNCH_CHECK();
  return 0;
}

}
```

### few_shot_seg_cwt_amd/csrc/conv_body.h

```cpp
#pragma once
#include "common.h"
#include "kernels.h"

namespace cwt {

typedef __bf16 bf16x8 __attribute__((ext_vector_type(8)));

#define CWT_LDS __attribute__((address_space(3)))
#define CWT_GLB __attribute__((address_space(1)))

__device__ __forceinline__ void glds16(const void* src, char* lds_dst) {
  __builtin_amdgcn_global_load_lds((const CWT_GLB void*)src, (CWT_LDS void*)lds_dst, 16, 0, 0);
}

template <int N>
__device__ __forceinline__ void wait_vmcnt() {
  asm volatile("s_waitcnt vmcnt(%0)" ::"n"(N) : "memory");
}

template <int LPT>
__device__ __forceinline__ void wait_tiles(int n) {
  if (n <= 0)
    wait_vmcnt<0>();
  else if (n == 1)
// ... 30 lines not shown
      r.b = f32x4{0.f, 0.f, 0.f, 0.f};
    } else {
      const __bf16* rp = a.res_s + ((long)m * (a.Co >> 5) + (co >> 5)) * 64 + (co & 31);
      r.a = *(const f32x4*)rp;
      r.b = *(const f32x4*)(rp + 32);
    }
  } else {
    r.a = r.b = f32x4{0.f, 0.f, 0.f, 0.f};
  }
  return r;
}

template <int PREC>
__device__ __forceinline__ void store_out8(const ConvSArgs& a, int m, int co, const float* v, const float* sc,
                                           const float* sh, const Res8& rs) {
  float o[8];
#pragma unroll
  for (int i = 0; i < 8; ++i) o[i] = fmaf(v[i], sc[i], sh[i]);
  if (a.res) {
#pragma unroll
    for (int i = 0; i < 4; ++i) {
      o[i] += rs.a[i];
      o[4 + i] += rs.b[i];
    }
  } else if (a.res_s) {
    const bf16x8 rh = __builtin_bit_cast(bf16x8, rs.a), rl = __builtin_bit_cast(bf16x8, rs.b);
#pragma unroll
    for (int i = 0; i < 8; ++i) o[i] += PREC == 1 ? (float)rh[i] : (float)rh[i] + (float)rl[i];
  }
  if (a.relu) {
#pragma unroll
    for (int i = 0; i < 8; ++i) o[i] = fmaxf(o[i], 0.f);
  }
  if (a.y) {
    f32x4* yp = (f32x4*)(a.y + (long)m * a.y_ld + a.y_off + co);
    yp[0] = f32x4{o[0], o[1], o[2], o[3]};
    yp[1] = f32x4{o[4], o[5], o[6], o[7]};
  }
  if (a.ys) {
    bf16x8 hi, lo;
#pragma unroll
    for (int i = 0; i < 8; ++i) {
      hi[i] = (__bf16)o[i];
      lo[i] = (__bf16)(o[i] - (float)hi[i]);
    }
    if (PREC == 1) {
      *(bf16x8*)(a.ys + (long)m * a.Co + co) = hi;
    } else {
      __bf16* sp = a.ys + ((long)m * (a.Co >> 5) + (co >> 5)) * 64 + (co & 31);
      *(bf16x8*)sp = hi;
      *(bf16x8*)(sp + 32) = lo;
    }
  }
}

__device__ __forceinline__ void split3_bf16(const f32x4& x0, const f32x4& x1, bf16x8& h, bf16x8& m, bf16x8& l) {
#pragma unroll
  for (int i = 0; i < 8; ++i) {
    const float v = i < 4 ? x0[i] : x1[i - 4];
    const __bf16 hv = (__bf16)v;
    const float r = v - (float)hv;
    const __bf16 mv = (__bf16)r;
    h[i] = hv;
    m[i] = mv;
    l[i] = (__bf16)(r - (float)mv);
  }
}

template <int BM, int BN, int WAVES_M, int WAVES_N, int NSTG, int PREC, int PF>
__device__ __forceinline__ void conv_s_body(const ConvSArgs& a) {
  static_assert(PREC == 0 || PREC == 1 || PREC == 3 || PREC == 6,
                "PREC: 3 = bf16x3 over the S-layout, 1 = plain bf16, 0 = exact fp32 (f32 MFMA), "
                "6 = fp32 operands split three ways in registers (bf16x6)");
  constexpr int NW = WAVES_M * WAVES_N;
  constexpr int WM = BM / WAVES_M, WN = BN / WAVES_N;
  constexpr int FM = WM / 16, FN = WN / 16;
  constexpr int LA = BM / (8 * NW), LB = BN / (8 * NW);
  constexpr int NLO = PREC == 6 ? BN / 16 : 0;
  constexpr int LBL = PREC == 6 ? (NLO + NW - 1) / NW : 0;
  constexpr int LPT = LA + LB + LBL;
  constexpr int LO_OFF = (BM + BN) * 128;
  constexpr int STG_BYTES = (BM + BN) * 128 + (PREC == 6 ? BN * 64 : 0);
  static_assert(LA * 8 * NW == BM && LB * 8 * NW == BN, "tile rows must split into 8-row pieces per wave");
  static_assert(NSTG >= 2 && NSTG <= 6, "ring depth");
  constexpr int EP_ROWS = WM < 32 ? WM : 32;
  constexpr int EP_LD = WN + 4;
  constexpr int EP_BYTES = NW * EP_ROWS * EP_LD * 4;
  constexpr int SMEM = NSTG * STG_BYTES > EP_BYTES ? NSTG * STG_BYTES : EP_BYTES;
  __shared__ __attribute__((aligned(16))) char smem[SMEM];

  const int tid = threadIdx.x;
  const int lane = tid & 63;
  const int wv = __builtin_amdgcn_readfirstlane(tid >> 6);
  const int wm = wv / WAVES_N, wn = wv % WAVES_N;
  int mt, nt, ks;
  conv_tile_coords(mt, nt, ks);
  const bool batched = PREC == 6 && a.batch > 1;
  const int bidx = batched ? ks : 0;
  if (batched) ks = 0;
  const char* xs_b = (const char*)a.xs + (batched ? bidx * a.xs_bstride : 0L);
  const __bf16* ws_b = a.ws + (batched ? bidx * a.ws_bstride : 0L);
  const __bf16* wl_b = a.ws_lo + (batched ? bidx * a.wl_bstride : 0L);
  float* part_b = a.part + (batched ? (long)bidx * a.M * a.Co : 0L);
  const int m0 = mt * BM, n0 = nt * BN;
  const int kt_begin = ks * a.kt_per_split;
  const int kt_end = min(a.ktiles, kt_begin + a.kt_per_split);
  const int T = kt_end - kt_begin;
  if constexpr ((PF & 64) != 0) {
    asm volatile("" ::"s"(T));
    return;
  }


  const int lrow = lane >> 3, lslot = lane & 7;
  const int cblocks = a.Ci >> (PREC == 1 ? 6 : 5);
  int a_ih0[LA], a_iw0[LA], a_pix0[LA], a_ch[LA];
  const int HoWo = a.Ho * a.Wo;
#pragma unroll
  for (int j = 0; j < LA; ++j) {
    const int r = (wv * LA + j) * 8 + lrow;
    a_ch[j] = (lslot ^ ((r >> 1) & 7)) * 8;
    const int m = m0 + r;
    if (m < a.M) {
      const int n = m / HoWo;
      const int rem = m - n * HoWo;
      const int oh = rem / a.Wo;
      const int ow = rem - oh * a.Wo;
      a_ih0[j] = oh * a.stride - a.pad;
      a_iw0[j] = ow * a.stride - a.pad;
      a_pix0[j] = (n * a.Hi + a_ih0[j]) * a.Wi + a_iw0[j];
    } else {
      a_ih0[j] = -(1 << 28);
      a_iw0[j] = 0;
      a_pix0[j] = 0;
    }
  }
  const int b_rowlen = a.ktiles_total * 64;
  int b_off[LB];
#pragma unroll
  for (int j = 0; j < LB; ++j) {
    const int r = (wv * LB + j) * 8 + lrow;
    b_off[j] = (n0 + r) * b_rowlen + (lslot ^ ((r >> 1) & 7)) * 8;
  }

  int i_cb, i_ky, i_kx;
  {
    const int taps = a.kh * a.kw;
    i_cb = kt_begin / taps;
    const int tap = kt_begin - i_cb * taps;
    i_ky = tap / a.kw;
    i_kx = tap - i_ky * a.kw;
  }
  int i_kt = kt_begin;
  __amdgpu_buffer_rsrc_t rsA, rsB, rsL;
  int a_roff[LA], b_voff[LB], l_voff[LBL > 0 ? LBL : 1];
#if defined(__HIP_DEVICE_COMPILE__)
  if constexpr ((PF & 8) != 0) {
    const int cbl = a.Ci >> (PREC == 1 ? 6 : 5);
    const long a_bytes = (long)a.N * a.Hi * a.Wi * cbl * 128;
    rsA = __builtin_amdgcn_make_buffer_rsrc((void*)xs_b, (short)0, (int)a_bytes, 0x00020000);
    rsB = __builtin_amdgcn_make_buffer_rsrc((void*)ws_b, (short)0, (int)((long)a.Co * a.ktiles_total * 128), 0x00020000);
#pragma unroll
    for (int j = 0; j < LA; ++j) a_roff[j] = (a_pix0[j] * cbl * 64 + a_ch[j]) * 2;
#pragma unroll
    for (int j = 0; j < LB; ++j) b_voff[j] = b_off[j] * 2;
    if constexpr (PREC == 6) {
      rsL = __builtin_amdgcn_make_buffer_rsrc((void*)wl_b, (short)0, (int)((long)a.Co * a.ktiles_total * 64),
                                              0x00020000);
#pragma unroll
      for (int j = 0; j < LBL; ++j) {
        const int q = (wv * LBL + j) % NLO;
        const int r = q * 16 + (lane >> 2);
        l_voff[j] = (n0 + r) * a.ktiles_total * 64 + (((lane & 3) ^ ((r >> 2) & 3)) << 4);
      }
    }
  }
#endif
  auto issue = [&](int stg) {
    if (PF & 4) return;
    char* sb = smem + stg * STG_BYTES;
#if defined(__HIP_DEVICE_COMPILE__)
    if constexpr ((PF & 8) != 0) {
      const int dy = i_ky * a.dil, dx = i_kx * a.dil;
      const int uni = ((dy * a.Wi + dx) * cblocks + i_cb) * 128;
#pragma unroll
      for (int j = 0; j < LA; ++j) {
        const int ih = a_ih0[j] + dy, iw = a_iw0[j] + dx;
        const bool in = (unsigned)ih < (unsigned)a.Hi && (unsigned)iw < (unsigned)a.Wi;
        __builtin_amdgcn_raw_ptr_buffer_load_lds(rsA, (CWT_LDS void*)(sb + (wv * LA + j) * 1024), 16,
                                                 in ? a_roff[j] + uni : (int)0x80000000, 0, 0, 0);
      }
#pragma unroll
      for (int j = 0; j < LB; ++j)
        __builtin_amdgcn_raw_ptr_buffer_load_lds(rsB, (CWT_LDS void*)(sb + BM * 128 + (wv * LB + j) * 1024), 16,
                                                 b_voff[j], i_kt * 128, 0, 0);
      if constexpr (PREC == 6) {
#pragma unroll
        for (int j = 0; j < LBL; ++j)
          __builtin_amdgcn_raw_ptr_buffer_load_lds(rsL, (CWT_LDS void*)(sb + LO_OFF + ((wv * LBL + j) % NLO) * 1024), 16,
                                                   l_voff[j], i_kt * 64, 0, 0);
      }
      ++i_kt;
      if (++i_kx == a.kw) {
        i_kx = 0;
        if (++i_ky == a.kh) {
          i_ky = 0;
          ++i_cb;
        }
      }
      return;
    }
#endif
    const int dy = i_ky * a.dil, dx = i_kx * a.dil;
    const int shift = dy * a.Wi + dx;
#pragma unroll
    for (int j = 0; j < LA; ++j) {
      const int ih = a_ih0[j] + dy, iw = a_iw0[j] + dx;
      const bool in = (unsigned)ih < (unsigned)a.Hi && (unsigned)iw < (unsigned)a.Wi;
      const __bf16* src = in ? a.xs + ((a_pix0[j] + shift) * cblocks + i_cb) * 64 + a_ch[j] : a.zero;
      glds16(src, sb + (wv * LA + j) * 1024);
    }
#pragma unroll
    for (int j = 0; j < LB; ++j) glds16(a.ws + b_off[j] + i_kt * 64, sb + BM * 128 + (wv * LB + j) * 1024);
    ++i_kt;
    if (++i_kx == a.kw) {
      i_kx = 0;
      if (++i_ky == a.kh) {
        i_ky = 0;
        ++i_cb;
      }
    }
  };

  f32x4 acc[FM][FN];
#pragma unroll
  for (int i = 0; i < FM; ++i)
#pragma unroll
    for (int j = 0; j < FN; ++j) acc[i][j] = f32x4{0.f, 0.f, 0.f, 0.f};

  const int fr = lane & 15, fk = lane >> 4;
  const int swz = (fr >> 1) & 7;
  const int off_hi = fr * 128 + ((fk ^ swz) << 4);
  const int off_lo = fr * 128 + (((4 + fk) ^ swz) << 4);
  const int off_a0 = PREC == 6 ? fr * 128 + (((2 * fk) ^ swz) << 4) : off_hi;
  const int off_a1 = PREC == 6 ? fr * 128 + (((2 * fk + 1) ^ swz) << 4) : off_lo;
  const int off_l = fr * 64 + ((fk ^ ((fr >> 2) & 3)) << 4);
  const int a_row0 = wm * WM, b_row0 = BM + wn * WN;

  constexpr bool LAZY_B = PREC == 6 && (PF & 3) == 0 && FN >= 8;
  struct Frags {
    bf16x8 ah[FM], al[FM], bh[LAZY_B ? 1 : FN], bl[LAZY_B ? 1 : FN];
    bf16x8 bo[PREC == 6 && !LAZY_B ? FN : 1];
  };
  auto read_frags = [&](Frags& F, int stg) {
    const char* sb = smem + stg * STG_BYTES;
#pragma unroll
    for (int j = 0; j < (LAZY_B ? 0 : FN); ++j) {
      const char* p = sb + (b_row0 + j * 16) * 128;
      F.bh[j] = *(const bf16x8*)(p + off_hi);
      F.bl[j] = *(const bf16x8*)(p + off_lo);
    }
#pragma unroll
    for (int i = 0; i < FM; ++i) {
      const char* p = sb + (a_row0 + i * 16) * 128;
      F.ah[i] = *(const bf16x8*)(p + off_a0);
      F.al[i] = *(const bf16x8*)(p + off_a1);
    }
    if constexpr (PREC == 6 && !LAZY_B) {
#pragma unroll
      for (int j = 0; j < FN; ++j) F.bo[j] = *(const bf16x8*)(sb + LO_OFF + (wn * WN + j * 16) * 64 + off_l);
    }
  };
  auto mfmas = [&](const Frags& F, int stg) {
    if (PF & 2) {
#pragma unroll
      for (int i = 0; i < FM; ++i) asm volatile("" ::"v"(F.ah[i]), "v"(F.al[i]));
#pragma unroll
      for (int j = 0; j < (LAZY_B ? 1 : FN); ++j)
        asm volatile("" ::"v"(F.bh[j]), "v"(F.bl[j]), "v"(F.bo[j < (PREC == 6 && !LAZY_B ? FN : 1) ? j : 0]));
      return;
    }
    if constexpr (LAZY_B) {
      const char* sb = smem + stg * STG_BYTES;
      bf16x8 as[FM][3];
#pragma unroll
      for (int i = 0; i < FM; ++i)
        if constexpr ((PF & 16) != 0) {
          as[i][0] = F.ah[i];
          as[i][1] = F.al[i];
          as[i][2] = F.ah[i];
        } else {
          split3_bf16(__builtin_bit_cast(f32x4, F.ah[i]), __builtin_bit_cast(f32x4, F.al[i]), as[i][0], as[i][1],
                      as[i][2]);
        }
#pragma unroll
      for (int j = 0; j < FN; ++j) {
        const char* p = sb + (b_row0 + j * 16) * 128;
        const bf16x8 bh = *(const bf16x8*)(p + off_hi), bm = *(const bf16x8*)(p + off_lo);
        const bf16x8 bl = *(const bf16x8*)(sb + LO_OFF + (wn * WN + j * 16) * 64 + off_l);
#pragma unroll
        for (int i = 0; i < FM; ++i) {
          acc[i][j] = __builtin_amdgcn_mfma_f32_16x16x32_bf16(as[i][1], bm, acc[i][j], 0, 0, 0);
          acc[i][j] = __builtin_amdgcn_mfma_f32_16x16x32_bf16(as[i][2], bh, acc[i][j], 0, 0, 0);
          acc[i][j] = __builtin_amdgcn_mfma_f32_16x16x32_bf16(as[i][0], bl, acc[i][j], 0, 0, 0);
          acc[i][j] = __builtin_amdgcn_mfma_f32_16x16x32_bf16(as[i][1], bh, acc[i][j], 0, 0, 0);
          acc[i][j] = __builtin_amdgcn_mfma_f32_16x16x32_bf16(as[i][0], bm, acc[i][j], 0, 0, 0);
          acc[i][j] = __builtin_amdgcn_mfma_f32_16x16x32_bf16(as[i][0], bh, acc[i][j], 0, 0, 0);
        }
      }
    } else if constexpr (PREC == 6) {
#pragma unroll
      for (int i = 0; i < FM; ++i) {
        bf16x8 ah, am, al;
        split3_bf16(__builtin_bit_cast(f32x4, F.ah[i]), __builtin_bit_cast(f32x4, F.al[i]), ah, am, al);
#pragma unroll
        for (int j = 0; j < FN; ++j) {
          acc[i][j] = __builtin_amdgcn_mfma_f32_16x16x32_bf16(am, F.bl[j], acc[i][j], 0, 0, 0);
          acc[i][j] = __builtin_amdgcn_mfma_f32_16x16x32_bf16(al, F.bh[j], acc[i][j], 0, 0, 0);
          acc[i][j] = __builtin_amdgcn_mfma_f32_16x16x32_bf16(ah, F.bo[j], acc[i][j], 0, 0, 0);
          acc[i][j] = __builtin_amdgcn_mfma_f32_16x16x32_bf16(am, F.bh[j], acc[i][j], 0, 0, 0);
          acc[i][j] = __builtin_amdgcn_mfma_f32_16x16x32_bf16(ah, F.bl[j], acc[i][j], 0, 0, 0);
          acc[i][j] = __builtin_amdgcn_mfma_f32_16x16x32_bf16(ah, F.bh[j], acc[i][j], 0, 0, 0);
        }
      }
    } else {
#pragma unroll
    for (int i = 0; i < FM; ++i)
#pragma unroll
      for (int j = 0; j < FN; ++j) {
        if (PREC == 0) {
          const f32x4 a0 = __builtin_bit_cast(f32x4, F.ah[i]), a1 = __builtin_bit_cast(f32x4, F.al[i]);
          const f32x4 b0 = __builtin_bit_cast(f32x4, F.bh[j]), b1 = __builtin_bit_cast(f32x4, F.bl[j]);
#pragma unroll
          for (int s = 0; s < 4; ++s) acc[i][j] = __builtin_amdgcn_mfma_f32_16x16x4f32(a0[s], b0[s], acc[i][j], 0, 0, 0);
#pragma unroll
          for (int s = 0; s < 4; ++s) acc[i][j] = __builtin_amdgcn_mfma_f32_16x16x4f32(a1[s], b1[s], acc[i][j], 0, 0, 0);
        } else if (PREC == 1) {
          acc[i][j] = __builtin_amdgcn_mfma_f32_16x16x32_bf16(F.ah[i], F.bh[j], acc[i][j], 0, 0, 0);
          acc[i][j] = __builtin_amdgcn_mfma_f32_16x16x32_bf16(F.al[i], F.bl[j], acc[i][j], 0, 0, 0);
        } else {
          acc[i][j] = __builtin_amdgcn_mfma_f32_16x16x32_bf16(F.al[i], F.bh[j], acc[i][j], 0, 0, 0);
          acc[i][j] = __builtin_amdgcn_mfma_f32_16x16x32_bf16(F.ah[i], F.bl[j], acc[i][j], 0, 0, 0);
          acc[i][j] = __builtin_amdgcn_mfma_f32_16x16x32_bf16(F.ah[i], F.bh[j], acc[i][j], 0, 0, 0);
// ... 115 lines not shown
```

### few_shot_seg_cwt_amd/csrc/conv_forms.h

```cpp
#pragma once
#include <type_traits>

#include "kernels.h"

namespace cwt {

#define CWT_CONV_FORMS(X, A)                                                                   \
  X(256, 256, 0, 2, 4, 2, 0, 0) A(256, 256, 1, 0) A(256, 256, 2, 0)                            \
  X(256, 128, 0, 4, 2, 3, 0, 0) X(256, 128, 1, 4, 2, 3, 1, 0) A(256, 128, 2, 1)                \
  X(128, 256, 0, 2, 4, 3, 0, 0) X(128, 256, 1, 2, 4, 3, 1, 0) A(128, 256, 2, 1)                \
  X(128, 128, 0, 2, 2, 3, 0, 0) X(128, 128, 1, 2, 2, 3, 1, 0) X(128, 128, 2, 2, 4, 3, 1, 0)    \
  X(128, 128, 4, 2, 2, 2, 0, 0)                                                                \
  X(128, 64, 0, 2, 2, 3, 0, 0) X(128, 64, 1, 2, 2, 3, 1, 0) X(128, 64, 2, 4, 2, 3, 1, 0)       \
  X(64, 128, 0, 2, 2, 3, 0, 0) X(64, 128, 1, 2, 2, 3, 1, 0) X(64, 128, 2, 2, 4, 3, 1, 0)       \
  X(64, 64, 0, 2, 2, 4, 0, 0) X(64, 64, 1, 2, 2, 4, 1, 0) X(64, 64, 2, 2, 4, 4, 1, 0)          \
         \
  X(64, 64, 8, 2, 2, 4, 2, 1) X(64, 64, 9, 2, 2, 4, 4, 1)                                      \
                                             \
  X(128, 128, 10, 2, 4, 3, 3, 1) X(128, 128, 11, 2, 4, 3, 5, 1)

#define CWT_CONV_FORMS_X6(X, A)                                                                \
  X(256, 256, 3, 4, 2, 2, 0, 0) X(256, 128, 3, 8, 1, 2, 0, 0) X(128, 256, 3, 4, 2, 2, 0, 0)    \
  X(128, 128, 3, 4, 1, 3, 0, 0) X(128, 128, 5, 4, 1, 2, 0, 0)                                  \
  X(128, 64, 3, 4, 1, 3, 0, 0) X(128, 64, 5, 4, 1, 2, 0, 0)                                    \
  X(64, 128, 3, 4, 1, 3, 0, 0) X(64, 128, 5, 4, 1, 2, 0, 0)                                    \
  X(64, 64, 3, 4, 1, 4, 0, 0)                                                                  \
    \
      \
                                           \
  X(128, 128, 12, 4, 1, 2, 16, 0) X(128, 128, 14, 4, 1, 2, 4, 0) X(128, 128, 15, 4, 1, 2, 2, 0) \
  X(128, 128, 16, 4, 1, 2, 6, 0) X(128, 128, 17, 4, 1, 2, 38, 0) X(128, 128, 18, 4, 1, 2, 64, 0) \
                                                \
  X(256, 256, 13, 4, 2, 2, 16, 0)

struct ConvForm {
  int bm, bn, var, waves_m, waves_n, nstg, pf;
  bool fixed_tile;
  int alias;
};
const ConvForm* find_conv_form(int prec, int bm, int bn, int var);
const ConvForm* fixed_tile_form(int prec, int var);

template <int LAST, class F>
void with_stage(int stage, F&& f) {
  if constexpr (LAST > 0)
    if (stage >= 0 && stage < LAST) return with_stage<LAST - 1>(stage, f);
  f(std::integral_constant<int, LAST>{});
}

template <class Fam, int STAGE>
void launch_form(const ConvPlan& p, const ConvSArgs& a, dim3 grid, hipStream_t st) {
#define CWT_ROW(BM, BN, VAR, WM, WN, NS, PF, FIXED)     \
  if (p.bm == BM && p.bn == BN && p.var == VAR)         \
    return Fam::template launch<BM, BN, WM, WN, NS, (FIXED && Fam::kStudyStage0) ? 0 : STAGE, PF>(a, grid, st);
#define CWT_ALIAS(BM, BN, VAR, TARGET)
  CWT_CONV_FORMS(CWT_ROW, CWT_ALIAS)
  if constexpr (Fam::kX6) {
    CWT_CONV_FORMS_X6(CWT_ROW, CWT_ALIAS)
  }
#undef CWT_ROW
#undef CWT_ALIAS
}

#define CWT_CONV_FAMILY(NAME, KERNEL, X6, STUDY_STAGE0)                                        \
  struct NAME {                                                                                \
    static constexpr bool kX6 = X6, kStudyStage0 = STUDY_STAGE0;                               \
    template <int BM, int BN, int WM, int WN, int NS, int STAGE, int PF>                       \
    static void launch(const ConvSArgs& a, dim3 grid, hipStream_t st) {                        \
      hipLaunchKernelGGL((KERNEL<BM, BN, WM, WN, NS, STAGE, PF>), grid, dim3(WM * WN * 64), 0, st, a); \
    }                                                                                          \
  }

}
```

### few_shot_seg_cwt_amd/csrc/conv_plans_x6.inc

```
{1800, 128, 128, 128, 128, 1, 5, 16},
{1800, 256, 256, 128, 128, 1, 5, 16},
{1800, 512, 2048, 128, 128, 1, 5, 16},
{2048, 512, 512, 128, 128, 1, 5, 16},
{3362, 128, 128, 128, 128, 1, 5, 16},
{3362, 512, 2048, 128, 128, 1, 5, 16},
{3528, 256, 256, 128, 128, 1, 5, 16},
{3600, 128, 128, 128, 128, 1, 4, 16},
{3600, 256, 256, 128, 128, 1, 5, 16},
{3600, 512, 2048, 128, 128, 1, 5, 16},
{3872, 512, 512, 128, 128, 1, 5, 16},
{4096, 512, 512, 128, 128, 1, 5, 16},
{5400, 128, 128, 128, 128, 1, 4, 16},
{5400, 256, 256, 128, 128, 1, 5, 16},
{5400, 512, 2048, 128, 128, 1, 5, 16},
{6144, 512, 512, 128, 128, 1, 5, 16},
{13122, 256, 512, 128, 128, 1, 5},
{13122, 256, 1024, 128, 128, 2, 5},
{13122, 256, 2304, 128, 128, 2, 5},
{13122, 512, 1024, 128, 128, 1, 5},
{13122, 512, 2048, 128, 128, 1, 5},
{13122, 512, 4608, 128, 128, 1, 5},
{13122, 512, 18432, 128, 128, 1, 5},
{13122, 1024, 256, 256, 256, 1, 0},
{13122, 1024, 512, 256, 256, 1, 0},
{13122, 2048, 512, 128, 128, 1, 4},
{13122, 2048, 1024, 128, 128, 1, 4},
{14400, 128, 512, 64, 64, 1, 0},
{14400, 128, 1152, 128, 128, 4, 5},
{14400, 256, 512, 128, 128, 1, 5},
{14400, 256, 1024, 128, 128, 2, 5},
{14400, 256, 2304, 128, 128, 2, 5},
{14400, 512, 128, 128, 256, 1, 0},
{14400, 512, 256, 128, 128, 1, 5},
{14400, 512, 1024, 128, 128, 1, 5},
{14400, 512, 2048, 128, 128, 1, 5},
{14400, 512, 4608, 128, 128, 1, 5},
{14400, 512, 18432, 128, 128, 1, 5},
{14400, 1024, 256, 256, 256, 1, 0},
{14400, 1024, 512, 256, 256, 1, 0},
{14400, 2048, 512, 128, 128, 1, 4},
{14400, 2048, 1024, 128, 128, 1, 5},
{21600, 256, 512, 128, 128, 1, 5},
{21600, 256, 1024, 128, 128, 1, 5},
{21600, 256, 2304, 128, 128, 2, 5},
{21600, 512, 1024, 128, 128, 1, 4},
{21600, 512, 2048, 128, 128, 1, 5},
{21600, 512, 4608, 128, 128, 2, 5},
{21600, 512, 18432, 128, 128, 4, 5},
{21600, 1024, 256, 128, 128, 1, 4},
{21600, 1024, 512, 128, 128, 1, 4},
{21600, 2048, 512, 128, 128, 1, 4},
{21600, 2048, 1024, 128, 128, 1, 4},
{56644, 64, 128, 64, 64, 1, 0},
{56644, 64, 256, 64, 64, 1, 0},
{56644, 64, 576, 64, 64, 1, 0},
{56644, 128, 256, 128, 128, 1, 5},
{56644, 256, 64, 256, 256, 1, 0},
{56644, 256, 128, 256, 256, 1, 0},
{224676, 64, 576, 64, 64, 1, 0},
{224676, 128, 576, 128, 128, 1, 4},
{450, 128, 128, 128, 128, 1, 5, 36},
{450, 512, 2048, 128, 128, 1, 5, 36},
{512, 256, 256, 128, 128, 1, 5, 36},
{512, 512, 512, 128, 128, 1, 5, 36},
{7200, 256, 2304, 128, 128, 4, 5},
{7200, 512, 4608, 128, 128, 2, 5},
{7200, 512, 18432, 128, 128, 2, 5},
{7200, 128, 512, 64, 64, 1, 3},
{7200, 128, 1152, 64, 64, 2, 3},
{7200, 256, 512, 64, 128, 1, 5},
{7200, 256, 1024, 64, 128, 2, 5},
{7200, 512, 128, 128, 64, 1, 5},
{7200, 512, 256, 64, 128, 1, 5},
{7200, 512, 1024, 64, 128, 1, 5},
{7200, 512, 2048, 128, 128, 2, 5},
{7200, 1024, 256, 128, 128, 1, 5},
{7200, 1024, 512, 128, 128, 1, 5},
{7200, 2048, 512, 128, 128, 1, 5},
{7200, 2048, 1024, 128, 128, 1, 5},
{13122, 128, 512, 64, 64, 1, 3},
{13122, 128, 1152, 64, 64, 1, 3},
{13122, 512, 128, 128, 128, 1, 4},
{13122, 512, 256, 128, 128, 1, 5},
{21600, 128, 512, 64, 128, 1, 5},
{21600, 128, 1152, 64, 128, 1, 5},
{21600, 512, 128, 128, 128, 1, 4},
{21600, 512, 256, 128, 128, 1, 4},
{28322, 64, 128, 64, 64, 1, 0},
{28322, 64, 256, 64, 64, 1, 3},
{28322, 64, 576, 64, 64, 1, 3},
{28322, 128, 256, 128, 64, 1, 5},
{28322, 256, 64, 128, 128, 1, 4},
{28322, 256, 128, 128, 128, 1, 4},
{51842, 64, 128, 128, 64, 1, 5},
{51842, 64, 256, 128, 64, 1, 5},
{51842, 64, 576, 128, 64, 1, 5},
{51842, 128, 256, 128, 128, 1, 5},
{51842, 256, 64, 256, 256, 1, 0},
{51842, 256, 128, 256, 256, 1, 0},
{84966, 64, 128, 128, 64, 1, 5},
{84966, 64, 256, 128, 64, 1, 5},
{84966, 64, 576, 128, 64, 1, 5},
{84966, 128, 256, 128, 128, 1, 4},
{84966, 256, 64, 128, 128, 1, 4},
{84966, 256, 128, 128, 128, 1, 4},
{112338, 64, 576, 128, 64, 1, 5},
{112338, 128, 576, 128, 128, 1, 5},
{206082, 64, 576, 128, 64, 1, 5},
{206082, 128, 576, 128, 128, 1, 4},
{337014, 64, 576, 128, 64, 1, 5},
{337014, 128, 576, 128, 128, 1, 5},
```

### few_shot_seg_cwt_amd/csrc/conv_x3s.hip

```cpp
#include <algorithm>
#include <iterator>

#include "conv_body.h"
#include "conv_forms.h"

namespace cwt {
template <int BM, int BN, int WAVES_M, int WAVES_N, int NSTG, int STAGE, int PF = 0>
__global__ __launch_bounds__(WAVES_M* WAVES_N * 64) void conv_igemm_x3s(ConvSArgs a) {
  conv_s_body<BM, BN, WAVES_M, WAVES_N, NSTG, 3, (PF | 8)>(a);
}
template <int BM, int BN, int WAVES_M, int WAVES_N, int NSTG, int STAGE, int PF = 0>
__global__ __launch_bounds__(WAVES_M* WAVES_N * 64) void conv_igemm_b16(ConvSArgs a) {
  conv_s_body<BM, BN, WAVES_M, WAVES_N, NSTG, 1, (PF | 8)>(a);
}
template <int BM, int BN, int WAVES_M, int WAVES_N, int NSTG, int STAGE, int PF = 0>
__global__ __launch_bounds__(WAVES_M* WAVES_N * 64) void conv_igemm_f32d(ConvSArgs a) {
  conv_s_body<BM, BN, WAVES_M, WAVES_N, NSTG, 0, (PF | 8)>(a);
}

template <int NS, int PREC>
__global__ void conv_s_splitk_epilogue(ConvSArgs a, int nsplit) {
  const int g8 = a.Co >> 3;
  const long idx = (long)blockIdx.x * blockDim.x + threadIdx.x;
  if (idx >= (long)a.M * g8) return;
// ... 53 lines not shown
  const int g8 = C >> 3;
  const long idx = (long)blockIdx.x * blockDim.x + threadIdx.x;
  if (idx >= P * g8) return;
  const long p = idx / g8;
  const int c = (int)(idx - p * g8) * 8;
  const __bf16* sp = s + (p * (C >> 5) + (c >> 5)) * 64 + (c & 31);
  const bf16x8 hi = *(const bf16x8*)sp, lo = *(const bf16x8*)(sp + 32);
  f32x4 v0, v1;
#pragma unroll
  for (int i = 0; i < 4; ++i) {
    v0[i] = (float)hi[i] + (float)lo[i];
    v1[i] = (float)hi[4 + i] + (float)lo[4 + i];
  }
  *(f32x4*)(out + p * ld + c) = v0;
  *(f32x4*)(out + p * ld + c + 4) = v1;
}

__global__ void widen_bf16_kernel(const __bf16* x, long n, float* y) {
  for (long i = (long)blockIdx.x * 256 + threadIdx.x; i < n; i += (long)gridDim.x * 256) y[i] = (float)x[i];
}

int launch_widen_bf16(const __bf16* x, long n, float* y, hipStream_t st) {
  hipLaunchKernelGGL(widen_bf16_kernel, dim3((unsigned)std::min<long>(65536, (n + 255) / 256)), dim3(256), 0, st, x, n, y);
  CWT_LAUNCH_CHECK();
  return 0;
}

int launch_split_act(const float* x, long P, int C, int ld, __bf16* out, hipStream_t st) {
  if (C % 32) return fail(CWT_EARG, "split_act: C % 32");
  const long n = P * (C / 8);
  hipLaunchKernelGGL(split_act_kernel, dim3((unsigned)((n + 255) / 256)), dim3(256), 0, st, x, P, C, ld, out);
  CWT_LAUNCH_CHECK();
  return 0;
}

int launch_unsplit_act(const __bf16* s, long P, int C, float* out, int ld, hipStream_t st) {
  if (C % 32) return fail(CWT_EARG, "unsplit_act: C % 32");
  const long n = P * (C / 8);
  hipLaunchKernelGGL(unsplit_act_kernel, dim3((unsigned)((n + 255) / 256)), dim3(256), 0, st, s, P, C, out, ld);
  CWT_LAUNCH_CHECK();
  return 0;
}

CWT_CONV_FAMILY(FamX3s, conv_igemm_x3s, false, true);
CWT_CONV_FAMILY(FamB16, conv_igemm_b16, false, true);
CWT_CONV_FAMILY(FamF32d, conv_igemm_f32d, false, true);

#define CWT_ROW(BM, BN, VAR, WM, WN, NS, PF, FIXED) {BM, BN, VAR, WM, WN, NS, PF, FIXED != 0, -1},
#define CWT_ALIAS(BM, BN, VAR, TARGET) {BM, BN, VAR, 0, 0, 0, 0, false, TARGET},
static constexpr ConvForm kConvForms[] = {CWT_CONV_FORMS(CWT_ROW, CWT_ALIAS)};
static constexpr ConvForm kConvFormsX6[] = {CWT_CONV_FORMS(CWT_ROW, CWT_ALIAS) CWT_CONV_FORMS_X6(CWT_ROW, CWT_ALIAS)};
#undef CWT_ROW
#undef CWT_ALIAS

template <class Pred>
static const ConvForm* find_form_if(int prec, Pred pred) {
  if (prec != 0 && prec != 1 && prec != 3 && prec != 6) return nullptr;
  const ConvForm* t = prec == 6 ? kConvFormsX6 : kConvForms;
  const size_t n = prec == 6 ? std::size(kConvFormsX6) : std::size(kConvForms);
  const ConvForm* e = std::find_if(t, t + n, pred);
  return e == t + n ? nullptr : e;
}

const ConvForm* find_conv_form(int prec, int bm, int bn, int var) {
  const auto row = [&](int v) {
    return find_form_if(prec, [=](const ConvForm& f) { return f.bm == bm && f.bn == bn && f.var == v; });
  };
  const ConvForm* f = row(var);
  return f && f->alias >= 0 ? row(f->alias) : f;
}

const ConvForm* fixed_tile_form(int prec, int var) {
  return find_form_if(prec, [=](const ConvForm& f) { return f.fixed_tile && f.var == var; });
}

struct MeasuredPlan {
  int M, Co, K, bm, bn, nsplit, var, batch = 0;
};
static const MeasuredPlan kMeasuredPlansS[] = {
#include "conv_plans_x3s.inc"
    {}};
static const MeasuredPlan kMeasuredPlansB16[] = {
#include "conv_plans_b16.inc"
    {}};
static const MeasuredPlan kMeasuredPlansF32D[] = {
#include "conv_plans_f32d.inc"
    {}};
static const MeasuredPlan kMeasuredPlansX6[] = {
#include "conv_plans_x6.inc"
    {}};

static const int kPlanTiles[7][2] = {{256, 256}, {256, 128}, {128, 256}, {128, 128}, {128, 64}, {64, 128}, {64, 64}};

ConvPlan plan_heuristic_s(int M, int Co, int ktiles) {
  constexpr long kMinWG = 200;
  ConvPlan best;
  for (auto& c : kPlanTiles) {
    if (Co % c[1] != 0) continue;
    const long tiles = (long)cdiv(M, c[0]) * (Co / c[1]);
    int ks = 1;
    while (tiles * ks < kMinWG && ktiles / (ks * 2) >= 8) ks *= 2;
    ConvPlan p;
    p.bm = c[0];
    p.bn = c[1];
    p.kt_per_split = cdiv(ktiles, ks);
    p.nsplit = cdiv(ktiles, p.kt_per_split);
    if (tiles * p.nsplit >= kMinWG) return p;
    best = p;
  }
  return best;
}

static ConvPlan plan_heuristic_batched(int M, int Co, int ktiles, int batch) {
  ConvPlan best;
  for (auto& c : kPlanTiles) {
    if (Co % c[1] != 0) continue;
    ConvPlan p;
    p.bm = c[0];
    p.bn = c[1];
    p.kt_per_split = ktiles;
    p.nsplit = 1;
    best = p;
    if ((long)cdiv(M, c[0]) * (Co / c[1]) * batch >= 200) return p;
  }
  return best;
}

template <size_t N>
static ConvPlan plan_from_table(const MeasuredPlan (&table)[N], int M, int Co, int K, int kdepth, int batch) {
  const int ktiles = K / kdepth;
  for (const MeasuredPlan& e : table)
    if (e.batch == batch && e.M == M && e.Co == Co && e.K == K && e.bn > 0 && Co % e.bn == 0 &&
        (batch == 0 || e.nsplit == 1)) {
      ConvPlan p;
      p.bm = e.bm;
      p.bn = e.bn;
      p.var = e.var;
      p.kt_per_split = cdiv(ktiles, e.nsplit);
      p.nsplit = cdiv(ktiles, p.kt_per_split);
      return p;
    }
  return batch ? plan_heuristic_batched(M, Co, ktiles, batch) : plan_heuristic_s(M, Co, ktiles);
}

ConvPlan plan_conv_s(int prec, int M, int Co, int K, int batch) {
  switch (prec) {
    case 0: return plan_from_table(kMeasuredPlansF32D, M, Co, K, 32, batch);
    case 1: return plan_from_table(kMeasuredPlansB16, M, Co, K, 64, batch);
    case 6: return plan_from_table(kMeasuredPlansX6, M, Co, K, 32, batch);
    default: return plan_from_table(kMeasuredPlansS, M, Co, K, 32, batch);
  }
}

template <int PREC>
static void launch_splitk_s(const ConvSArgs& a, int nsplit, hipStream_t st) {
  const long n = (long)a.M * (a.Co / 8);
  const dim3 g((unsigned)((n + 255) / 256)), b(256);
  switch (nsplit) {
    case 2: hipLaunchKernelGGL((conv_s_splitk_epilogue<2, PREC>), g, b, 0, st, a, nsplit); break;
    case 3: hipLaunchKernelGGL((conv_s_splitk_epilogue<3, PREC>), g, b, 0, st, a, nsplit); break;
    case 4: hipLaunchKernelGGL((conv_s_splitk_epilogue<4, PREC>), g, b, 0, st, a, nsplit); break;
    case 8: hipLaunchKernelGGL((conv_s_splitk_epilogue<8, PREC>), g, b, 0, st, a, nsplit); break;
    default: hipLaunchKernelGGL((conv_s_splitk_epilogue<0, PREC>), g, b, 0, st, a, nsplit); break;
  }
}

int launch_conv_x3s(ConvSArgs a, const ConvPlan& p, int stage, float* part_ws, size_t part_ws_floats,
                    hipStream_t st, int prec) {
  if (prec != 0 && prec != 1 && prec != 3 && prec != 6)
    return fail(CWT_EARG, "conv precision must be 3 (bf16x3), 1 (bf16), 0 (exact fp32) or 6 (bf16x6)");
  const ConvForm* form = find_conv_form(prec, p.bm, p.bn, p.var);
  if (!form) return fail(CWT_EARG, "no such conv form (conv_forms.h)");
  const bool batched = prec == 6 && a.batch > 1;
  if ((prec == 0 || prec == 6) && (a.ys || a.res_s || (!a.y && !batched)))
    return fail(CWT_EARG, "fp32-operand conv: fp32 output and residual only");
  if (batched && (p.nsplit != 1 || !a.part || a.kh != 1 || a.kw != 1))
    return fail(CWT_EARG, "batched x6 GEMMs: 1x1, no split-K, raw output to part");
  if (prec == 6 && !a.ws_lo) return fail(CWT_ESTATE, "x6 conv: the weights' lo plane is missing");
  if (!a.xs || !a.ws || !a.zero) return fail(CWT_ESTATE, "S-layout conv needs its input, weights and a zero line");
  const int kb = prec == 1 ? 64 : 32;
  if (a.Ci % kb || a.Co % 64 || a.Co % p.bn)
    return fail(CWT_EARG, prec == 1 ? "bf16 conv: need Ci % 64 == 0, Co % 64 == 0"
                                    : "x3s conv: need Ci % 32 == 0, Co % 64 == 0");
  a.ktiles = a.K / kb;
  a.ktiles_total = a.ktiles;
  a.kt_per_split = p.kt_per_split;
  const int nsplit = p.nsplit;
  if (nsplit < 1 || (long)p.kt_per_split * nsplit < a.ktiles) return fail(CWT_EARG, "conv plan does not cover K");
  ConvSArgs main = a;
  if (batched) {
  } else if (nsplit > 1) {
    if ((size_t)nsplit * a.M * a.Co > part_ws_floats) return fail(CWT_ESTATE, "split-K workspace too small");
    main.part = part_ws;
  } else {
    main.part = nullptr;
  }
  dim3 grid(cdiv(a.M, p.bm), a.Co / p.bn, nsplit * (batched ? a.batch : 1));
  ConvPlan row = p;
  row.var = form->var;
  const auto launch = [&](auto fam) {
    with_stage<6>(stage, [&](auto s) { launch_form<decltype(fam), decltype(s)::value>(row, main, grid, st); });
  };
  if (prec == 6)
    launch_tiles_x6(stage, main, row, grid, st);
  else if (prec == 0)
    launch(FamF32d{});
  else if (prec == 1)
    launch(FamB16{});
  else
    launch(FamX3s{});
  CWT_LAUNCH_CHECK();
  if (nsplit > 1 && !batched) {
    main.part = part_ws;
    if (prec == 1)
      launch_splitk_s<1>(main, nsplit, st);
    else if (prec == 0 || prec == 6)
      launch_splitk_s<0>(main, nsplit, st);
    else
      launch_splitk_s<3>(main, nsplit, st);
    CWT_LAUNCH_CHECK();
  }
  return 0;
}

}
```

### few_shot_seg_cwt_amd/csrc/ctx.h

```cpp
#pragma once
#include <hip/hip_runtime.h>

#include <cstring>
#include <map>
#include <string>
#include <vector>

#include "../../include/cwt.h"
#include "common.h"
#include "kernels.h"

namespace cwt {

struct WsBuf {
  void* p = nullptr;
  size_t bytes = 0;
};

}

struct cwt_ctx {
  int device = 0;
  std::map<std::string, cwt::WsBuf> ws;
  size_t ws_total = 0;
  int prof_level = 0;
  struct Rec {
    std::string name;
    double flops, bytes;
    hipEvent_t e0, e1;
    int fslot = -1;
    int fpart = 0;
  };
  unsigned long long* fstamps = nullptr;
  int fstamp_next = 0;
  std::vector<Rec> recs;
  std::vector<hipEvent_t> evpool;
  size_t ev_used = 0;
  cwt::AdaptGraphCache adapt_graphs;
  bool use_graph = true;
  int conv_arith = CWT_CONV_ARITH_BF16X6;
  int adapt_upw = 0;
  unsigned* status_host = nullptr;
  unsigned* status_dev = nullptr;
  long adapt_spin_limit = 0;
  unsigned tail_epoch = ~0u;
  int tail_G = 0;
  int tail_stamp_G = 0;
  const float* fold_w = nullptr;
  const float* fold_fc = nullptr;
  int64_t fold_ver = -1;
  int fold_H = 0;
  hipStream_t aux = nullptr;
  hipEvent_t ev_fork = nullptr, ev_join = nullptr;
};

namespace cwt {

struct Prof {
  cwt_ctx* c;
  hipStream_t st;
  int idx = -1;
  Prof(cwt_ctx* ctx, hipStream_t s, const std::string& name, double flops, double bytes, int level = 2,
       bool deferred = false)
      : c(ctx), st(s) {
    if (c->prof_level < level || !push(name, flops, bytes) || deferred) return;
    (void)hipEventRecord(c->recs[idx].e0, st);
  }
  void end() {
    if (idx >= 0) (void)hipEventRecord(c->recs[idx].e1, st);
    idx = -1;
  }
  hipEvent_t ev0() const { return idx >= 0 ? c->recs[idx].e0 : nullptr; }
  hipEvent_t ev1() const { return idx >= 0 ? c->recs[idx].e1 : nullptr; }

 private:
  bool push(const std::string& name, double flops, double bytes) {
    hipEvent_t ev[2];
    for (int k = 0; k < 2; ++k) {
      if (c->ev_used == c->evpool.size()) {
        hipEvent_t e;
        if (hipEventCreate(&e) != hipSuccess) return false;
        c->evpool.push_back(e);
      }
      ev[k] = c->evpool[c->ev_used++];
    }
    c->recs.push_back({name, flops, bytes, ev[0], ev[1]});
    idx = (int)c->recs.size() - 1;
    return true;
  }
};

int ensure_ws(cwt_ctx* ctx, const std::string& name, size_t bytes, void** out);
template <class T>
int ws(cwt_ctx* ctx, const char* name, size_t count, T** out) {
  void* p = nullptr;
  const int rc = ensure_ws(ctx, name, count * sizeof(T), &p);
  *out = (T*)p;
  return rc;
}
int zero_line(cwt_ctx* ctx, const __bf16** out);

int gemm_f32d_mode();
bool gemm_f32d_ok(int M, int N, int K, const void* A, const void* Bm, const void* Cm, const void* res);
int gemm_f32d(cwt_ctx* ctx, const float* A, const float* Bm, int M, int N, int K, float* Cm, const float* bias,
              const float* res, int res_ld, hipStream_t st, int relu = 0);
int readout_gemm(cwt_ctx* ctx, const float* P, const float* vt, int B, int NA, int Cv, int ldp, float* out,
                 hipStream_t st);
int gemm_nt(cwt_ctx* ctx, const float* A, const float* W, int M, int N, int K, float* C, hipStream_t st);

static const int kBlocks50[4] = {3, 4, 6, 3};
static const int kBlocks101[4] = {3, 4, 23, 3};
static const int kBins[4] = {1, 2, 3, 6};

static inline int down2(int x) { return (x - 1) / 2 + 1; }
static inline long ld32(long n) { return (n + 31) & ~31L; }

static inline int conv_out_size(int in, int k, int stride, int pad, int dil) {
  return (in + 2 * pad - dil * (k - 1) - 1) / stride + 1;
}

static inline ConvSArgs conv_s_geom(int N, int Hi, int Wi, int Ci, int Co, int k, int stride, int pad, int dil) {
  ConvSArgs a;
  memset(&a, 0, sizeof(a));
  a.N = N;
  a.Hi = Hi;
  a.Wi = Wi;
  a.Ci = Ci;
  a.Ho = conv_out_size(Hi, k, stride, pad, dil);
  a.Wo = conv_out_size(Wi, k, stride, pad, dil);
  a.Co = Co;
  a.kh = a.kw = k;
  a.stride = stride;
  a.pad = pad;
  a.dil = dil;
  a.M = N * a.Ho * a.Wo;
  a.K = k * k * Ci;
  return a;
}

struct ConvLayer {
  int Ci = 0, Co = 0, k = 1, stride = 1, pad = 0, dil = 1;
  float* w = nullptr;
  __bf16* w_s = nullptr;
  __bf16* w_l = nullptr;
  __bf16* wino_s = nullptr;
  __bf16* wino_l = nullptr;
  __bf16* wino4_s = nullptr;
  __bf16* wino4_l = nullptr;
  __bf16* w_b = nullptr;
  float* scale = nullptr;
  float* shift = nullptr;
  float* bn = nullptr;
};

struct ConvCall {
  int stage;
  const ConvLayer* L;
  const float* x;
  int N, Hi, Wi, x_ld;
  float* y;
  int y_ld, y_off;
  const float* res;
  int res_ld;
  int relu;
  bool out_f32;
};

ConvArgs make_args(const ConvCall& c);
int force_conv_form(int prec, int bm, int bn, int Co, ConvPlan* p);
int run_wino_conv(cwt_ctx* ctx, const float* x, int N, int H, int W, int Ci, int Co, int d, int m, const __bf16* us,
                  const __bf16* ul, const float* scale, const float* shift, const float* res, int res_ld, int relu,
                  float* y, int y_ld, int y_off, int stage, hipStream_t st, int bm = 0, int bn = 0);

}
```

### few_shot_seg_cwt_amd/csrc/kernels.h

```cpp
#pragma once
#include <vector>

#include "common.h"

namespace cwt {

struct ConvArgs {
  const float* x;
  const float* w;
  const float* scale;
  const float* shift;
  const float* res;
  float* y;
  float* part;
  int N, Hi, Wi, Ci, x_ld;
  int Ho, Wo, Co, kh, kw, stride, pad, dil;
  int M, K, ktiles, kt_per_split;
  int y_ld, y_off, res_ld;
  int relu;
};

struct ConvSArgs {
  const __bf16* xs;
  const __bf16* ws;
  const __bf16* ws_lo;
  const __bf16* zero;
  const float* scale;
  const float* shift;
  const float* res;
  const __bf16* res_s;
  float* y;
  __bf16* ys;
  float* part;
  int N, Hi, Wi, Ci;
  int Ho, Wo, Co, kh, kw, stride, pad, dil;
  int M, K, ktiles, ktiles_total, kt_per_split;
  int y_ld, y_off, res_ld;
  int relu;
  int batch;
  long xs_bstride, ws_bstride, wl_bstride;
};

__host__ __device__ __forceinline__ long packed_k(int ci, int tap, int taps) {
  return (long)(ci >> 5) * (taps * 32) + tap * 32 + (ci & 31);
}
__host__ __device__ __forceinline__ long packed_k64(int ci, int tap, int taps) {
  return (long)(ci >> 6) * (taps * 64) + tap * 64 + (ci & 63);
}

__device__ __forceinline__ void conv_tile_coords(int& mt, int& nt, int& ks) {
  const int T = gridDim.x * gridDim.y * gridDim.z;
  const int lin = blockIdx.x + gridDim.x * (blockIdx.y + gridDim.y * blockIdx.z);
  const int q = T >> 3, r = T & 7;
  const int xcd = lin & 7, slot = lin >> 3;
  const int L = (xcd < r) ? xcd * (q + 1) + slot : r * (q + 1) + (xcd - r) * q + slot;
  nt = L % gridDim.y;
  const int rest = L / gridDim.y;
  mt = rest % gridDim.x;
  ks = rest / gridDim.x;
}

__device__ __forceinline__ void conv_store_fragment(const ConvArgs& a, const f32x16& acc, int mbase, int co, int h,
                                                    int ks, float sc, float sh) {
  if (a.part) {
#pragma unroll
    for (int r = 0; r < 16; ++r) {
      const int m = mbase + (r & 3) + 8 * (r >> 2) + 4 * h;
      if (m < a.M) a.part[((long)ks * a.M + m) * a.Co + co] = acc[r];
    }
    return;
  }
  float rv[16];
  if (a.res) {
#pragma unroll
    for (int r = 0; r < 16; ++r) {
      const int m = min(mbase + (r & 3) + 8 * (r >> 2) + 4 * h, a.M - 1);
      rv[r] = a.res[(long)m * a.res_ld + co];
    }
  } else {
#pragma unroll
    for (int r = 0; r < 16; ++r) rv[r] = 0.f;
  }
#pragma unroll
  for (int r = 0; r < 16; ++r) {
    const int m = mbase + (r & 3) + 8 * (r >> 2) + 4 * h;
    float v = fmaf(acc[r], sc, sh) + rv[r];
    if (a.relu) v = fmaxf(v, 0.f);
    if (m < a.M) a.y[(long)m * a.y_ld + a.y_off + co] = v;
  }
}

struct ConvPlan {
  int bm = 128, bn = 128, kt_per_split = 1, nsplit = 1;
  int var = 0;
};

ConvPlan plan_conv(int M, int Co, int K);
int launch_conv(ConvArgs a, const ConvPlan& p, int stage, float* part_ws, size_t part_ws_floats, hipStream_t st);
int launch_splitk_epilogue(const ConvArgs& a, int nsplit, hipStream_t st);
ConvPlan plan_conv_s(int prec, int M, int Co, int K, int batch = 0);
struct WinoGeom {
  int N, H, W, d;
  int m;
  int P;
  int TY, TX;
  long T;
};
WinoGeom wino_geom(int N, int H, int W, int d, int m = 2);
int launch_wino_weights(const float* w_packed, int Co, int Ci, float* U, hipStream_t st, int m = 2);
int launch_wino_in(const float* x, const WinoGeom& g, int Ci, float* V, hipStream_t st);
int launch_wino_out(const float* Mb, const WinoGeom& g, int Co, const float* scale, const float* shift, const float* res,
                    int res_ld, int relu, float* y, int y_ld, int y_off, hipStream_t st);
int launch_conv_x3s(ConvSArgs a, const ConvPlan& p, int stage, float* part_ws, size_t part_ws_floats,
                    hipStream_t st, int prec = 3);
int launch_split_act(const float* x, long P, int C, int ld, __bf16* out, hipStream_t st);
int launch_split_w3(const float* w, long R, int K, __bf16* ws, __bf16* wl, hipStream_t st);
int launch_occupy(int nwg, int us, hipStream_t st);

struct AdaptGraphCache {
  struct Entry {
    int E, n, h, w, S, iters;
    const void *fws, *lbl, *sc, *acc, *wbuf, *dargs;
    hipGraphExec_t exec;
    bool same(const Entry& o) const {
      return E == o.E && n == o.n && h == o.h && w == o.w && S == o.S && iters == o.iters && fws == o.fws &&
             lbl == o.lbl && sc == o.sc && acc == o.acc && wbuf == o.wbuf && dargs == o.dargs;
    }
  };
  std::vector<Entry> entries;
  hipStream_t cap_stream = nullptr;
  ~AdaptGraphCache();
};

enum ActLayout { ACT_F32 = 0, ACT_SPLIT = 1, ACT_BF16 = 2 };
int launch_stem_conv1(const float* img, int N, int S, const float* w27x64, const float* scale,
                      const float* shift, float* out, int Ho, hipStream_t st, int layout = ACT_F32,
                      int relu = 1);
struct BnTrainArgs {
  void* y;
  int layout, ld;
  long M;
  int C;
  const void* res;
  int res_ld;
  int relu;
  float* bn;
  float* scale;
  float* shift;
  float eps, momentum;
  float drop_p;
  unsigned long long seed;
  long rows_per_image;
};
size_t bn_train_part_floats(long M, int C);
int launch_bn_train(const BnTrainArgs& a, float* part, size_t part_floats, float* batch_sc, hipStream_t st);
int launch_scale_cols(const float* src, float* dst, long n, int period, const float* sc, hipStream_t st);
void find_new_hw(int h, int w, int S, int* nh, int* nw);
int launch_episode_image(const void* src, int src_f32, int H, int W, int S, const float* mean, const float* stdv,
                         const float* pad, int flip_h, int flip_v, float* dst, hipStream_t st);
int launch_episode_label(const unsigned char* src, int H, int W, int S, int cls, int flip_h, int flip_v,
                         long long* dst, hipStream_t st);
int launch_maxpool3s2_s(const __bf16* in, int N, int H, int W, int C, __bf16* out, int Ho, int Wo, hipStream_t st);
int launch_maxpool3s2_b16(const __bf16* in, int N, int H, int W, int C, __bf16* out, int Ho, int Wo, hipStream_t st);
int launch_maxpool3s2(const float* in, int N, int H, int W, int C, float* out, int Ho, int Wo,
                      hipStream_t st);
int launch_ppm(const float* x, int N, int h, int w, int ld, const int* bins, int nbins, float* ws,
               float* pooled, hipStream_t st, int layout = ACT_F32);
int launch_repack_cblock(const float* src, float* dst, int Co, int taps, int Ci, hipStream_t st);
int launch_smallm_gemm(const float* A, int lda, const float* const* Bt, const int* M, int np, int N, int K, int kc,
                       float* part, size_t part_floats, const float* const* scale, const float* const* shift,
                       float* out, hipStream_t st);
constexpr int kPpmGemmMaxRows = 200;
int launch_ppm_gemm(const float* A, int lda, const float* const* Bt, const int* M, int np, int N, int K,
                    const float* const* scale, const float* const* shift, float* part, size_t part_floats,
                    float* out, hipStream_t st);
int launch_ppm_field(const float* Q, int N, int h, int w, const int* bins, float* R, float* F, hipStream_t st);
int launch_ppm_field_bwd(const float* dF, int N, int h, int w, const int* bins, float* dR, float* dQ, hipStream_t st);

struct MmBwdWs {
  float* rowmax;
  int* rowarg;
  float* colpv;
  int* colpi;
  float* colmax;
  int* colarg;
  float* srow;
  float* scol;
};
int launch_mutual_matching_bwd(const float* x, const float* dy, int B, int NA, int NB, int C, float* dx,
                               const MmBwdWs& ws, hipStream_t st);
int launch_relu_mask(const float* g, const float* out, long n, float* gm, hipStream_t st);
int cp4d_wgrad_part_floats(int cin, int cout);
int launch_cp4d_wgrad_mfma(const float* x, const float* gm, int B, int hA, int wA, int hB, int wB, int cin, int cout,
                           int G, float* part, hipStream_t st);
int launch_cp4d_wgrad(const float* x, const float* gm, int B, int hA, int wA, int hB, int wB, int cin, int cout,
                      float* part, size_t part_floats, float* dWa, float* dWb, float* db1, float* db2, hipStream_t st);
int launch_cp4d_dgrad(const float* g, int B, int hA, int wA, int hB, int wB, int gin, int gout, const float* Wa,
                      const float* Wb, float* dx, int accum, hipStream_t st);
int launch_match_softmax_bwd(const float* P, int ldp, const float* dA, int rows, int NB, float temp, int accum,
                             float* g, hipStream_t st);
int launch_token_norm(const float* x, long T, int C, float eps, float* xn, float* nrm, hipStream_t st);
int launch_token_norm_bwd(const float* xn, const float* nrm, const float* dxn, long T, int C, int ld_d, float eps,
                          int accum, float* dx, hipStream_t st);
int launch_wa_bwd(const float* tpg, int N, int h, int w, int co, const float* bt, const float* bp, const float* bg,
                  const float* dwavg, float* coef, float* dtpg, hipStream_t st);
size_t colsum_ws_floats(long R, int Cc);
int launch_colsum(const float* X, long R, int Cc, long ld, int accum, float* out, float* ws, size_t ws_floats,
                  hipStream_t st);
int launch_to_channels_first(const float* x, int B, int C, long P, float* y, hipStream_t st);
int launch_copy_pad(const float* X, long R, int Cc, int ld, float* out, hipStream_t st);
size_t deform_attn_bwd_ws_bytes(int B, int H, int W, int M, int D);
int launch_deform_attn_bwd(const float* value, const float* offsets, const float* logits, int B, int H, int W, int M,
                           int P, int D, const float* d_out, float* d_value, float* d_offsets, float* d_logits,
                           void* ws, hipStream_t st);
int launch_norm_blend_bwd(const float* a, const float* b, const float* d, long T, int C, float wt, float* d_a,
                          float* d_b, hipStream_t st);
int launch_copy_2d(const float* src, long R, int Cc, long lds, float* dst, long ldd, hipStream_t st);
int launch_mmn_blend_bwd(const float* d_fq, const float* d_mean, int B, long n, float att_wt, float* d_att,
                         float* d_fq_in, hipStream_t st);

struct AdaptScalars;
struct AdaptDevArgs;
struct FusedTail;

int launch_unsplit_act(const __bf16* s, long P, int C, float* out, int ld, hipStream_t st);
int launch_widen_bf16(const __bf16* x, long n, float* y, hipStream_t st);

int launch_adapt(const float* f, const int64_t* lbl64, int E, int n, int h, int w, int S, float lr, int iters,
                 float* W, float* f_ws, uint8_t* lbl_ws, AdaptScalars* sc, float* acc3, float* wbuf,
                 AdaptDevArgs* dargs, AdaptGraphCache* cache, int upw, unsigned* status, long spin_limit,
                 hipStream_t st, hipEvent_t ev_k0, hipEvent_t ev_k1, const FusedTail* tail = nullptr);
const char* adapt_kernel_name(int E, int n, int h, int w, int iters, int upw);
int adapt_persist_workgroups(int E, int n, int h, int w, int iters, int upw);
extern unsigned long long* g_adapt_stamps;
extern long g_adapt_stamps_n;
size_t adapt_ws_sizes(int E, int n, int h, int w, int S, size_t* fws, size_t* lbl, size_t* sc, size_t* acc,
                      size_t* wbuf, size_t* dargs);
int launch_seg_ce(const float* logits, const int64_t* target, int B, int h, int w, int S, float* loss_out,
                  float* dlogits, uint8_t* lbl_ws, AdaptScalars* sc, double* loss_num, hipStream_t st);

int launch_normalize(const float* f, int B, int Pb, float* out, const float* W0, float* logits0, hipStream_t st);
int launch_classify(const float* W, const float* f, int B, int Pb, float* logits, hipStream_t st);
int launch_classify_scaled(const float* W, const float* f, const float* inv, int B, int Pb, float* logits,
                           hipStream_t st);
int launch_classify_bwd(const float* dl, const float* f, int B, int Pb, float* dW, hipStream_t st);
int launch_seg_metrics(const float* logits, const int64_t* target, int B, int h, int w, int S, float* iut,
                       double* ce, unsigned* counts_ws, hipStream_t st, const float* logits2 = nullptr,
                       float* iut2 = nullptr);
int launch_iou_preds(const int64_t* preds, const int64_t* target, long n, int K, int ignore, float* iut,
                     unsigned* counts_ws, hipStream_t st);
int launch_sgd(float* p, const float* g, float* buf, long n, float lr, float mom, float wd, int nesterov, int first,
               hipStream_t st);

size_t attention_fold_floats(int C, int H);
int attention_fold(const float* w_qkvs, const float* fc_w, int C, int H, float* fold, float* ws, size_t ws_floats,
                   hipStream_t st);
size_t attention_infer_ws_floats(int B, int hw, int C, int H);
int attention_infer(const float* q, const float* f, int B, int hw, int C, int H, const float* fold, const float* fc_b,
                    const float* ln_w, const float* ln_b, float* out, float* inv_norm, float* logits0, float* ws,
                    hipStream_t st);
size_t attention_saved_floats(int B, int hw, int C, int H);
size_t attention_ws_floats(int B, int hw, int C, int H);
int attention_fwd(const float* q, const float* f, int B, int hw, int C, int H, const float* w_qkvs,
                  const float* fc_w, const float* fc_b, const float* ln_w, const float* ln_b, float* out,
                  float* saved, float* ws, hipStream_t st, float p_attn, float p_out, unsigned long long seed);
int attention_bwd(const float* q, const float* f, int B, int hw, int C, int H, const float* w_qkvs,
                  const float* fc_w, const float* fc_b, const float* ln_w, const float* ln_b, const float* saved,
// ... 62 lines not shown
```

### few_shot_seg_cwt_amd/csrc/wino.hip

```cpp
#include "common.h"
#include "kernels.h"

namespace cwt {

WinoGeom wino_geom(int N, int H, int W, int d, int m) {
  WinoGeom g;
  g.N = N;
  g.H = H;
  g.W = W;
  g.d = d;
  g.m = m;
  g.P = (m + 2) * (m + 2);
  g.TY = ((H + d - 1) / d + m - 1) / m;
  g.TX = ((W + d - 1) / d + m - 1) / m;
  g.T = (long)N * d * d * g.TY * g.TX;
  return g;
}

__global__ void wino_weights_kernel(const float* __restrict__ w, int Co, int Ci, float* __restrict__ U) {
  const long idx = (long)blockIdx.x * blockDim.x + threadIdx.x;
  if (idx >= (long)Co * Ci) return;
  const int co = (int)(idx / Ci), ci = (int)(idx - (long)co * Ci);
  const long K = 9L * Ci;
  double g[3][3];
#pragma unroll
  for (int t = 0; t < 9; ++t) g[t / 3][t % 3] = (double)w[(long)co * K + packed_k(ci, t, 9)];
  double gg[4][3];
#pragma unroll
  for (int c = 0; c < 3; ++c) {
    gg[0][c] = g[0][c];
    gg[1][c] = 0.5 * (g[0][c] + g[1][c] + g[2][c]);
    gg[2][c] = 0.5 * (g[0][c] - g[1][c] + g[2][c]);
    gg[3][c] = g[2][c];
  }
  const long plane = (long)Co * Ci;
#pragma unroll
  for (int r = 0; r < 4; ++r) {
    const double u[4] = {gg[r][0], 0.5 * (gg[r][0] + gg[r][1] + gg[r][2]), 0.5 * (gg[r][0] - gg[r][1] + gg[r][2]),
                         gg[r][2]};
#pragma unroll
    for (int c = 0; c < 4; ++c) U[(r * 4 + c) * plane + idx] = (float)u[c];
  }
}

__device__ __forceinline__ void wino4_g(const double g0, const double g1, const double g2, double u[6]) {
  u[0] = g0 / 4.0;
  u[1] = -(g0 + g1 + g2) / 6.0;
  u[2] = -(g0 - g1 + g2) / 6.0;
  u[3] = g0 / 24.0 + g1 / 12.0 + g2 / 6.0;
  u[4] = g0 / 24.0 - g1 / 12.0 + g2 / 6.0;
  u[5] = g2;
}

__global__ void wino4_weights_kernel(const float* __restrict__ w, int Co, int Ci, float* __restrict__ U) {
  const long idx = (long)blockIdx.x * blockDim.x + threadIdx.x;
  if (idx >= (long)Co * Ci) return;
  const int co = (int)(idx / Ci), ci = (int)(idx - (long)co * Ci);
  const long K = 9L * Ci;
  double g[3][3];
#pragma unroll
  for (int t = 0; t < 9; ++t) g[t / 3][t % 3] = (double)w[(long)co * K + packed_k(ci, t, 9)];
  double gg[6][3];
#pragma unroll
  for (int c = 0; c < 3; ++c) {
    double u[6];
    wino4_g(g[0][c], g[1][c], g[2][c], u);
#pragma unroll
    for (int r = 0; r < 6; ++r) gg[r][c] = u[r];
  }
  const long plane = (long)Co * Ci;
#pragma unroll
  for (int r = 0; r < 6; ++r) {
    double u[6];
    wino4_g(gg[r][0], gg[r][1], gg[r][2], u);
#pragma unroll
    for (int c = 0; c < 6; ++c) U[(r * 6 + c) * plane + idx] = (float)u[c];
  }
}

int launch_wino_weights(const float* w_packed, int Co, int Ci, float* U, hipStream_t st, int m) {
  const long n = (long)Co * Ci;
  if (m == 4)
    hipLaunchKernelGGL(wino4_weights_kernel, dim3((unsigned)cdiv(n, 256)), dim3(256), 0, st, w_packed, Co, Ci, U);
  else if (m == 2)
    hipLaunchKernelGGL(wino_weights_kernel, dim3((unsigned)cdiv(n, 256)), dim3(256), 0, st, w_packed, Co, Ci, U);
  else
    return fail(CWT_EARG, "winograd: output tile must be 2 or 4");
  CWT_LAUNCH_CHECK();
  return 0;
}

__device__ __forceinline__ long wino_xcd_index() {
  const unsigned nb = gridDim.x, b = blockIdx.x;
  const unsigned q = nb >> 3, r = nb & 7, xcd = b & 7, slot = b >> 3;
  const unsigned L = xcd < r ? xcd * (q + 1) + slot : r * (q + 1) + (xcd - r) * q + slot;
  return (long)L * blockDim.x + threadIdx.x;
}

__device__ __forceinline__ void wino_tile(long t, const WinoGeom& g, int& n, int& py, int& px, int& ti, int& tj) {
  tj = (int)(t % g.TX);
  long r = t / g.TX;
  ti = (int)(r % g.TY);
  r /= g.TY;
  px = (int)(r % g.d);
  r /= g.d;
  py = (int)(r % g.d);
  n = (int)(r / g.d);
}

__global__ __launch_bounds__(256) void wino_in_kernel(const float* __restrict__ x, WinoGeom g, int Ci,
                                                      float* __restrict__ V) {
  const int q4 = Ci >> 2;
  const long idx = wino_xcd_index();
  if (idx >= g.T * q4) return;
  const long t = idx / q4;
  const int c = (int)(idx - t * q4) * 4;
  int n, py, px, ti, tj;
  wino_tile(t, g, n, py, px, ti, tj);
  f32x4 D[4][4];
#pragma unroll
  for (int u = 0; u < 4; ++u) {
    const int iy = py + g.d * (2 * ti - 1 + u);
#pragma unroll
    for (int v = 0; v < 4; ++v) {
      const int ix = px + g.d * (2 * tj - 1 + v);
      const bool in = (unsigned)iy < (unsigned)g.H && (unsigned)ix < (unsigned)g.W;
      D[u][v] = in ? *(const f32x4*)(x + (((long)n * g.H + iy) * g.W + ix) * Ci + c) : f32x4{0.f, 0.f, 0.f, 0.f};
    }
  }
  f32x4 R[4][4];
#pragma unroll
  for (int v = 0; v < 4; ++v) {
    R[0][v] = D[0][v] - D[2][v];
    R[1][v] = D[1][v] + D[2][v];
    R[2][v] = D[2][v] - D[1][v];
    R[3][v] = D[1][v] - D[3][v];
  }
  const long plane = g.T * Ci;
  float* vp = V + t * Ci + c;
#pragma unroll
  for (int u = 0; u < 4; ++u) {
    const f32x4 o[4] = {R[u][0] - R[u][2], R[u][1] + R[u][2], R[u][2] - R[u][1], R[u][1] - R[u][3]};
#pragma unroll
    for (int v = 0; v < 4; ++v) *(f32x4*)(vp + (u * 4 + v) * plane) = o[v];
  }
}

__device__ __forceinline__ void wino4_bt(const f32x4 d[6], f32x4 r[6]) {
  r[0] = 4.f * d[0] - 5.f * d[2] + d[4];
  r[1] = (d[3] + d[4]) - 4.f * (d[1] + d[2]);
  r[2] = (d[4] - d[3]) + 4.f * (d[1] - d[2]);
  r[3] = (d[4] - d[2]) + 2.f * (d[3] - d[1]);
  r[4] = (d[4] - d[2]) + 2.f * (d[1] - d[3]);
  r[5] = 4.f * d[1] - 5.f * d[3] + d[5];
}

__global__ __launch_bounds__(256) void wino4_in_kernel(const float* __restrict__ x, WinoGeom g, int Ci,
                                                       float* __restrict__ V) {
  const int q4 = Ci >> 2;
  const long idx = wino_xcd_index();
  if (idx >= g.T * q4) return;
  const long t = idx / q4;
  const int c = (int)(idx - t * q4) * 4;
  int n, py, px, ti, tj;
  wino_tile(t, g, n, py, px, ti, tj);
  f32x4 R[6][6];
#pragma unroll
  for (int v = 0; v < 6; ++v) {
    const int ix = px + g.d * (4 * tj - 1 + v);
    f32x4 D[6];
#pragma unroll
    for (int u = 0; u < 6; ++u) {
      const int iy = py + g.d * (4 * ti - 1 + u);
      const bool in = (unsigned)iy < (unsigned)g.H && (unsigned)ix < (unsigned)g.W;
      D[u] = in ? *(const f32x4*)(x + (((long)n * g.H + iy) * g.W + ix) * Ci + c) : f32x4{0.f, 0.f, 0.f, 0.f};
    }
    f32x4 r[6];
    wino4_bt(D, r);
#pragma unroll
    for (int u = 0; u < 6; ++u) R[u][v] = r[u];
  }
  const long plane = g.T * Ci;
  float* vp = V + t * Ci + c;
#pragma unroll
  for (int u = 0; u < 6; ++u) {
    f32x4 o[6];
    wino4_bt(R[u], o);
#pragma unroll
    for (int v = 0; v < 6; ++v) *(f32x4*)(vp + (u * 6 + v) * plane) = o[v];
  }
}

int launch_wino_in(const float* x, const WinoGeom& g, int Ci, float* V, hipStream_t st) {
  if (Ci % 4) return fail(CWT_EARG, "wino_in: Ci % 4");
  const long n = g.T * (Ci / 4);
  if (g.m == 4)
    hipLaunchKernelGGL(wino4_in_kernel, dim3((unsigned)cdiv(n, 256)), dim3(256), 0, st, x, g, Ci, V);
  else if (g.m == 2)
    hipLaunchKernelGGL(wino_in_kernel, dim3((unsigned)cdiv(n, 256)), dim3(256), 0, st, x, g, Ci, V);
  else
    return fail(CWT_EARG, "winograd: output tile must be 2 or 4");
  CWT_LAUNCH_CHECK();
  return 0;
}

__global__ __launch_bounds__(256) void wino_out_kernel(const float* __restrict__ Mb, WinoGeom g, int Co,
                                                       const float* __restrict__ scale, const float* __restrict__ shift,
                                                       const float* __restrict__ res, int res_ld, int relu,
                                                       float* __restrict__ y, int y_ld, int y_off) {
  const int q4 = Co >> 2;
  const long idx = (long)blockIdx.x * blockDim.x + threadIdx.x;
  if (idx >= g.T * q4) return;
  const long t = idx / q4;
  const int c = (int)(idx - t * q4) * 4;
  int n, py, px, ti, tj;
  wino_tile(t, g, n, py, px, ti, tj);
  const long plane = g.T * Co;
  const float* mp = Mb + t * Co + c;
  f32x4 m[4][4];
#pragma unroll
  for (int u = 0; u < 4; ++u)
#pragma unroll
    for (int v = 0; v < 4; ++v) m[u][v] = *(const f32x4*)(mp + (u * 4 + v) * plane);
  f32x4 s[2][4];
#pragma unroll
  for (int v = 0; v < 4; ++v) {
    s[0][v] = m[0][v] + m[1][v] + m[2][v];
    s[1][v] = m[1][v] - m[2][v] - m[3][v];
  }
  const f32x4 sc = *(const f32x4*)(scale + c), sh = *(const f32x4*)(shift + c);
#pragma unroll
  for (int a = 0; a < 2; ++a) {
    const f32x4 o[2] = {s[a][0] + s[a][1] + s[a][2], s[a][1] - s[a][2] - s[a][3]};
    const int oy = py + g.d * (2 * ti + a);
#pragma unroll
    for (int b = 0; b < 2; ++b) {
      const int ox = px + g.d * (2 * tj + b);
      if (oy >= g.H || ox >= g.W) continue;
      const long pix = ((long)n * g.H + oy) * g.W + ox;
      f32x4 v;
#pragma unroll
      for (int i = 0; i < 4; ++i) v[i] = fmaf(o[b][i], sc[i], sh[i]);
      if (res) v += *(const f32x4*)(res + pix * res_ld + c);
      if (relu) {
#pragma unroll
        for (int i = 0; i < 4; ++i) v[i] = fmaxf(v[i], 0.f);
      }
      *(f32x4*)(y + pix * y_ld + y_off + c) = v;
    }
  }
}

__device__ __forceinline__ void wino4_at(const f32x4 m[6], f32x4 o[4]) {
  const f32x4 p12 = m[1] + m[2], m12 = m[1] - m[2], p34 = m[3] + m[4], m34 = m[3] - m[4];
  o[0] = m[0] + p12 + p34;
  o[1] = m12 + 2.f * m34;
  o[2] = p12 + 4.f * p34;
  o[3] = m12 + 8.f * m34 + m[5];
}

__global__ __launch_bounds__(256) void wino4_out_kernel(const float* __restrict__ Mb, WinoGeom g, int Co,
                                                        const float* __restrict__ scale, const float* __restrict__ shift,
                                                        const float* __restrict__ res, int res_ld, int relu,
                                                        float* __restrict__ y, int y_ld, int y_off) {
  const int q4 = Co >> 2;
  const long idx = (long)blockIdx.x * blockDim.x + threadIdx.x;
  if (idx >= g.T * q4) return;
  const long t = idx / q4;
  const int c = (int)(idx - t * q4) * 4;
  int n, py, px, ti, tj;
  wino_tile(t, g, n, py, px, ti, tj);
  const long plane = g.T * Co;
  const float* mp = Mb + t * Co + c;
  f32x4 s[4][6];
#pragma unroll
  for (int v = 0; v < 6; ++v) {
    f32x4 m[6], o[4];
#pragma unroll
    for (int u = 0; u < 6; ++u) m[u] = *(const f32x4*)(mp + (u * 6 + v) * plane);
    wino4_at(m, o);
#pragma unroll
    for (int a = 0; a < 4; ++a) s[a][v] = o[a];
  }
  const f32x4 sc = *(const f32x4*)(scale + c), sh = *(const f32x4*)(shift + c);
#pragma unroll
  for (int a = 0; a < 4; ++a) {
    f32x4 o[4];
    wino4_at(s[a], o);
    const int oy = py + g.d * (4 * ti + a);
    if (oy >= g.H) break;
#pragma unroll
    for (int b = 0; b < 4; ++b) {
      const int ox = px + g.d * (4 * tj + b);
      if (ox >= g.W) break;
      const long pix = ((long)n * g.H + oy) * g.W + ox;
      f32x4 v;
#pragma unroll
      for (int i = 0; i < 4; ++i) v[i] = fmaf(o[b][i], sc[i], sh[i]);
      if (res) v += *(const f32x4*)(res + pix * res_ld + c);
      if (relu) {
#pragma unroll
        for (int i = 0; i < 4; ++i) v[i] = fmaxf(v[i], 0.f);
      }
      *(f32x4*)(y + pix * y_ld + y_off + c) = v;
    }
  }
}

int launch_wino_out(const float* Mb, const WinoGeom& g, int Co, const float* scale, const float* shift, const float* res,
                    int res_ld, int relu, float* y, int y_ld, int y_off, hipStream_t st) {
  if (Co % 4 || y_ld % 4 || y_off % 4 || (res && res_ld % 4)) return fail(CWT_EARG, "wino_out: 16-B channel groups");
  const long n = g.T * (Co / 4);
  if (g.m == 4)
    hipLaunchKernelGGL(wino4_out_kernel, dim3((unsigned)cdiv(n, 256)), dim3(256), 0, st, Mb, g, Co, scale, shift, res,
                       res_ld, relu, y, y_ld, y_off);
  else if (g.m == 2)
    hipLaunchKernelGGL(wino_out_kernel, dim3((unsigned)cdiv(n, 256)), dim3(256), 0, st, Mb, g, Co, scale, shift, res,
                       res_ld, relu, y, y_ld, y_off);
  else
    return fail(CWT_EARG, "winograd: output tile must be 2 or 4");
  CWT_LAUNCH_CHECK();
  return 0;
}

}
```

### include/cwt_debug.h

```cpp
#ifndef CWT_DEBUG_H_
#define CWT_DEBUG_H_
#include "cwt.h"

#ifdef __cplusplus
extern "C" {
#endif

int cwt_debug_conv(cwt_ctx* ctx, const float* x, int N, int Hi, int Wi, int Ci, int x_ld,
                   const float* w_packed, const float* scale, const float* shift, int Co, int k,
                   int stride, int pad, int dil, const float* res, int res_ld, int relu, float* y,
                   int y_ld, int y_off, int bm, int bn, int nsplit, int precision, void* stream);

int cwt_debug_split_act(cwt_ctx* ctx, const float* x, int64_t P, int C, int ld, void* out, void* stream);
int cwt_debug_unsplit_act(cwt_ctx* ctx, const void* s, int64_t P, int C, float* out, int ld, void* stream);
int cwt_debug_pack_wsplit(cwt_ctx* ctx, const float* w, int Co, int k, int Ci, void* out, void* stream);
int cwt_debug_conv_s(cwt_ctx* ctx, const void* xs, int N, int Hi, int Wi, int Ci, const void* ws,
                     const float* scale, const float* shift, int Co, int k, int stride, int pad,
                     int dil, const float* res, int res_ld, const void* res_s, int relu, float* y,
                     int y_ld, int y_off, void* ys, int bm, int bn, int nsplit, void* stream);
int cwt_debug_conv_b16(cwt_ctx* ctx, const void* xs, int N, int Hi, int Wi, int Ci, const void* ws,
                       const float* scale, const float* shift, int Co, int k, int stride, int pad,
                       int dil, const float* res, int res_ld, const void* res_s, int relu, float* y,
                       int y_ld, int y_off, void* ys, int bm, int bn, int nsplit, void* stream);

int cwt_debug_conv_f32d(cwt_ctx* ctx, const float* x, int N, int Hi, int Wi, int Ci, const float* w_packed,
                        const float* scale, const float* shift, int Co, int k, int stride, int pad, int dil,
                        const float* res, int res_ld, int relu, float* y, int y_ld, int y_off, int bm, int bn,
                        int nsplit, void* stream);

int cwt_debug_conv_x6(cwt_ctx* ctx, const float* x, int N, int Hi, int Wi, int Ci, const float* w_packed,
                      const float* scale, const float* shift, int Co, int k, int stride, int pad, int dil,
                      const float* res, int res_ld, int relu, float* y, int y_ld, int y_off, int bm, int bn,
                      int nsplit, void* stream);

int cwt_debug_conv_form(int prec, int bm, int bn, int var, int* out4);
int cwt_debug_conv_plan(int prec, int M, int Co, int K, int batch, int* out5);

int cwt_debug_conv_x6w(cwt_ctx* ctx, const float* x, int N, int Hi, int Wi, int Ci, const float* w_packed,
                       const float* scale, const float* shift, int Co, int k, int stride, int pad, int dil,
                       const float* res, int res_ld, int relu, float* y, int y_ld, int y_off, int bm, int bn,
                       int nsplit, void* stream);

int cwt_debug_cp4d_layer(cwt_ctx* ctx, const float* x, int B, int hA, int wA, int hB, int wB, int cin, int cout,
                         const float* Wa, const float* ba, const float* Wb, const float* bb, float* y, int variant,
                         void* stream);

int cwt_debug_tail_stamps(cwt_ctx* ctx, unsigned long long* host_out, int64_t max_count, int64_t* count);

int cwt_debug_occupy(cwt_ctx* ctx, int nwg, int us, void* stream);

int cwt_debug_adapt_stamps(cwt_ctx* ctx, unsigned long long* host_out, int64_t max_count, int64_t* count);

int cwt_debug_adapt_spin_limit(cwt_ctx* ctx, int64_t limit);

int cwt_debug_pretrain_capture(cwt_pretrain* pt, int on);
int cwt_debug_pretrain_tensor(cwt_pretrain* pt, const char* name, float* host_out, int64_t numel);

int cwt_debug_census(cwt_ctx* ctx, int nblocks, unsigned* out, void* stream);

int cwt_cu_count(cwt_ctx* ctx, int* count);
int cwt_stream_create_masked(cwt_ctx* ctx, const uint32_t* mask, int mask_words, void** stream);
int cwt_stream_destroy(void* stream);

int cwt_debug_pretrain_op(cwt_ctx* ctx, int op, void* const* bufs, const int64_t* iargs, const float* fargs,
                          void* stream);

int cwt_debug_backbone_op(cwt_ctx* ctx, int op, void* const* bufs, const int64_t* iargs, const float* fargs,
                          void* stream);

#ifdef __cplusplus
}
#endif
#endif
```

Before: 387.8 episodes/s.

## Fuse downsample conv into conv3 as dual-source GEMM; fold split-K reduce into Winograd input

In blocks with a downsample branch, the 1x1 downsample conv and its BN are folded into the conv3 weights along K, so one dual-source implicit GEMM replaces two convs plus a residual read. Separately, when a split-K conv feeds a Winograd conv, its partials are reduced, scaled, shifted and ReLU'd inside the Winograd input transform instead of in a separate epilogue pass. Both are on by default for the x6 path and can be disabled with environment knobs. The costs are extra weight memory for the fused blocks, re-folding after training updates, and a partial read repeated per split for each overlapping Winograd tile.

```diff
diff --git a/few_shot_seg_cwt_amd/_lib.py b/few_shot_seg_cwt_amd/_lib.py
--- a/few_shot_seg_cwt_amd/_lib.py
+++ b/few_shot_seg_cwt_amd/_lib.py
@@ -113,6 +113,10 @@
                                _I, _I, _P]),
     "cwt_debug_conv_x6w": (_I, [_P, _P, _I, _I, _I, _I, _P, _P, _P, _I, _I, _I, _I, _I, _P, _I, _I, _P, _I, _I, _I,
                                 _I, _I, _P]),
+    "cwt_debug_conv_x6_dual": (_I, [_P, _P, _I, _I, _I, _I, _P, _I, _I, _I, _I, _P, _P, _P, _P, _P, _P, _I, _I, _P,
+                                    _I, _I, _I, _P]),
+    "cwt_debug_wino_in": (_I, [_P, _P, _I, _P, _P, _I, _I, _I, _I, _I, _I, _I, _P, _P]),
+    "cwt_debug_splitk_epilogue": (_I, [_P, _P, _I, _I, _I, _P, _P, _I, _P, _P]),
     "cwt_debug_conv_form": (_I, [_I, _I, _I, _I, C.POINTER(_I)]),
     "cwt_debug_conv_plan": (_I, [_I, _I, _I, _I, _I, C.POINTER(_I)]),
     "cwt_debug_census": (_I, [_P, _I, _P, _P]),
diff --git a/few_shot_seg_cwt_amd/csrc/api_debug.hip b/few_shot_seg_cwt_amd/csrc/api_debug.hip
--- a/few_shot_seg_cwt_amd/csrc/api_debug.hip
+++ b/few_shot_seg_cwt_amd/csrc/api_debug.hip
@@ -272,6 +272,85 @@
                       relu, y, y_ld, y_off, nullptr, bm, bn, nsplit, stream);
 }
 
+int cwt_debug_conv_x6_dual(cwt_ctx* ctx, const float* t, int N, int Ho, int Wo, int K1, const float* x, int Hi2,
+                           int Wi2, int K2, int stride2, const float* w3, const float* s3, const float* b3,
+                           const float* wd, const float* sd, const float* bd, int Co, int relu, float* y, int bm,
+                           int bn, int nsplit, void* stream) {
+  if (!ctx) return fail(CWT_EARG, "ctx is NULL");
+  CWT_CHECK(t && x && w3 && s3 && b3 && wd && sd && bd && y, "null buffer");
+  CWT_CHECK(N >= 1 && Ho >= 1 && Wo >= 1 && K1 > 0 && K2 > 0 && K1 % 32 == 0 && K2 % 32 == 0 && Co % 64 == 0,
+            "need K1 % 32 == 0, K2 % 32 == 0, Co % 64 == 0");
+  CWT_CHECK(stride2 >= 1 && (Ho - 1) * stride2 < Hi2 && (Wo - 1) * stride2 < Wi2, "second source too small");
+  const int K = K1 + K2;
+  ConvSArgs a = conv_s_geom(N, Ho, Wo, K1, Co, 1, 1, 0, 1);
+  int rc;
+  ConvPlan p = plan_conv_dual(a.M, Co, K);
+  if (bm > 0 && (rc = force_conv_form(6, bm, bn, Co, &p))) return rc;
+  if (nsplit > 0) {
+    p.kt_per_split = cdiv(K / 32, nsplit);
+    p.nsplit = cdiv(K / 32, p.kt_per_split);
+  }
+  CWT_HIP(hipSetDevice(ctx->device));
+  const hipStream_t st = (hipStream_t)stream;
+  float *wf, *shf, *ones, *part = nullptr;
+  __bf16 *w3s, *w3l;
+  if ((rc = zero_line(ctx, &a.zero)) || (rc = ws(ctx, "dbg.dual.w", (size_t)Co * K, &wf)) ||
+      (rc = ws(ctx, "dbg.dual.sh", (size_t)Co, &shf)) || (rc = ws(ctx, "dbg.dual.ones", (size_t)Co, &ones)) ||
+      (rc = ws(ctx, "dbg.dual.w3s", (size_t)Co * K * 2, &w3s)) || (rc = ws(ctx, "dbg.dual.w3l", (size_t)Co * K, &w3l)))
+    return rc;
+  static const bool w3_cache = getenv("CWT_DBG_W3_CACHE") && getenv("CWT_DBG_W3_CACHE")[0] == '1';
+  static const void* f_src = nullptr;
+  static long f_n = 0;
+  static void* f_dst = nullptr;
+  if (!(w3_cache && f_src == w3 && f_n == (long)Co * K && f_dst == w3s)) {
+    const std::vector<float> one(Co, 1.0f);
+    CWT_HIP(hipMemcpyAsync(ones, one.data(), sizeof(float) * Co, hipMemcpyHostToDevice, st));
+    CWT_HIP(hipStreamSynchronize(st));
+    if ((rc = launch_fold_dual(w3, s3, b3, K1, wd, sd, bd, K2, Co, wf, shf, st)) ||
+        (rc = launch_split_w3(wf, Co, K, w3s, w3l, st)))
+      return rc;
+    f_src = w3;
+    f_n = (long)Co * K;
+    f_dst = w3s;
+  }
+  a.K = K;
+  a.xs = (const __bf16*)t;
+  a.xs2 = (const __bf16*)x;
+  a.Hi2 = Hi2;
+  a.Wi2 = Wi2;
+  a.Ci2 = K2;
+  a.stride2 = stride2;
+  a.kt_switch = K1 / 32;
+  a.ws = w3s;
+  a.ws_lo = w3l;
+  a.scale = ones;
+  a.shift = shf;
+  a.relu = relu;
+  a.y = y;
+  a.y_ld = Co;
+  const size_t pf = (size_t)p.nsplit * a.M * Co;
+  if (p.nsplit > 1 && (rc = ws(ctx, "dbg.PART", pf, &part))) return rc;
+  return launch_conv_x3s(a, p, 0, part, pf, st, 6);
+}
+
+int cwt_debug_wino_in(cwt_ctx* ctx, const float* x, int nsplit, const float* scale, const float* shift, int relu,
+                      int N, int H, int W, int C, int d, int m, float* V, void* stream) {
+  if (!ctx) return fail(CWT_EARG, "ctx is NULL");
+  CWT_CHECK(x && V && N >= 1 && H >= 1 && W >= 1 && C >= 4 && C % 4 == 0 && d >= 1 && (m == 2 || m == 4), "wino_in");
+  CWT_CHECK(nsplit == 0 || (scale && shift && nsplit <= 64), "wino_in: split-K partials need scale and shift");
+  CWT_HIP(hipSetDevice(ctx->device));
+  const WinoGeom g = wino_geom(N, H, W, d, m);
+  return nsplit > 0 ? launch_wino_in_splitk(x, nsplit, scale, shift, relu, g, C, V, (hipStream_t)stream)
+                    : launch_wino_in(x, g, C, V, (hipStream_t)stream);
+}
+
+int cwt_debug_splitk_epilogue(cwt_ctx* ctx, const float* part, int nsplit, int M, int Co, const float* scale,
+                              const float* shift, int relu, float* y, void* stream) {
+  if (!ctx) return fail(CWT_EARG, "ctx is NULL");
+  CWT_HIP(hipSetDevice(ctx->device));
+  return launch_splitk_reduce_f32(part, nsplit, M, Co, scale, shift, relu, y, (hipStream_t)stream);
+}
+
 int cwt_debug_conv_form(int prec, int bm, int bn, int var, int* out4) {
   CWT_CHECK(out4, "out4 is NULL");
   const ConvForm* f = find_conv_form(prec, bm, bn, var);
diff --git a/few_shot_seg_cwt_amd/csrc/api_extract.hip b/few_shot_seg_cwt_amd/csrc/api_extract.hip
--- a/few_shot_seg_cwt_amd/csrc/api_extract.hip
+++ b/few_shot_seg_cwt_amd/csrc/api_extract.hip
@@ -10,6 +10,7 @@
 struct Block {
   ConvLayer c1, c2, c3, down;
   bool has_down = false;
+  ConvLayer fused;
 };
 
 struct Backbone {
@@ -214,6 +215,39 @@
   return 0;
 }
 
+static int fold_down(const Block& b, hipStream_t st) {
+  const int K1 = b.c3.Ci, K2 = b.down.Ci, Co = b.c3.Co;
+  int rc = launch_fold_dual(b.c3.w, b.c3.scale, b.c3.shift, K1, b.down.w, b.down.scale, b.down.shift, K2, Co,
+                            b.fused.w, b.fused.shift, st);
+  if (!rc) rc = launch_split_w3(b.fused.w, Co, K1 + K2, b.fused.w_s, b.fused.w_l, st);
+  return rc;
+}
+
+static int alloc_fused(Backbone* bb, Block* b) {
+  const size_t n = (size_t)b->c3.Co * (b->c3.Ci + b->down.Ci);
+  void *w = nullptr, *s = nullptr, *l = nullptr, *sh = nullptr;
+  CWT_HIP(hipMalloc(&w, n * 4));
+  bb->allocs.push_back(w);
+  CWT_HIP(hipMalloc(&s, n * 4));
+  bb->allocs.push_back(s);
+  CWT_HIP(hipMalloc(&l, n * 2));
+  bb->allocs.push_back(l);
+  CWT_HIP(hipMalloc(&sh, (size_t)b->c3.Co * 4));
+  bb->allocs.push_back(sh);
+  ConvLayer& F = b->fused;
+  F.Ci = b->c3.Ci;
+  F.Co = b->c3.Co;
+  F.w = (float*)w;
+  F.w_s = (__bf16*)s;
+  F.w_l = (__bf16*)l;
+  F.scale = bb->ones;
+  F.shift = (float*)sh;
+  const int rc = fold_down(*b, nullptr);
+  if (rc) return rc;
+  CWT_HIP(hipDeviceSynchronize());
+  return 0;
+}
+
 static int load_backbone(int layers, const HostParams& hp, float eps, Backbone** out) {
   if (layers != 50 && layers != 101) return fail(CWT_EARG, "layers must be 50 or 101");
   Backbone* bb = new Backbone();
@@ -278,6 +312,12 @@
     cleanup();
     return rc;
   }
+  for (int li = 0; li < 4; ++li)
+    for (Block& b : bb->blocks[li])
+      if (b.has_down && (rc = alloc_fused(bb, &b))) {
+        cleanup();
+        return rc;
+      }
   *out = bb;
   return 0;
 }
@@ -338,7 +378,7 @@
 int run_wino_conv(cwt_ctx* ctx, const float* x, int N, int H, int W, int Ci, int Co, int d, int m,
                          const __bf16* us, const __bf16* ul, const float* scale, const float* shift, const float* res,
                          int res_ld, int relu, float* y, int y_ld, int y_off, int stage, hipStream_t st, int bm,
-                         int bn) {
+                         int bn, const WinoSplitKSrc* sk) {
   if (m != 2 && m != 4) return fail(CWT_EARG, "winograd: output tile must be 2 or 4");
   const WinoGeom g = wino_geom(N, H, W, d, m);
   if (g.T * Ci * 4 >= (1L << 31) || g.T * Co * 4 >= (1L << 31)) return fail(CWT_EARG, "winograd: plane too large");
@@ -354,8 +394,9 @@
   (void)stage;
   const double vb = 4.0 * g.P * g.T * Ci, mb = 4.0 * g.P * g.T * Co;
   Prof pin(ctx, st, "wino_in " + std::to_string(Ci) + "@" + std::to_string(H), 0.0,
-           4.0 * N * H * W * Ci + vb, plev);
-  rc = launch_wino_in(x, g, Ci, V, st);
+           4.0 * N * H * W * Ci * (sk ? sk->nsplit : 1) + vb, plev);
+  rc = sk ? launch_wino_in_splitk(x, sk->nsplit, sk->scale, sk->shift, sk->relu, g, Ci, V, st)
+          : launch_wino_in(x, g, Ci, V, st);
   pin.end();
   if (rc) return rc;
   ConvSArgs a = conv_s_geom(1, (int)g.T, 1, Ci, Co, 1, 1, 0, 1);
@@ -399,6 +440,12 @@
   const bool f32ops = f32d || x6;
   const bool dma = s_path || f32ops;
   const int prec = b16 ? 1 : conv_split ? 3 : x6 ? 6 : 0;
+  const auto knob_on = [](const char* name) {
+    const char* v = getenv(name);
+    return !(v && v[0] == '0');
+  };
+  const bool fuse_down = x6 && knob_on("CWT_FUSE_DOWN");
+  const bool fuse_splitk = x6 && knob_on("CWT_FUSE_SPLITK_WINO");
   const int Hs = down2(S), H1 = down2(Hs), h = down2(H1);
   const long sA = std::max({(long)N * Hs * Hs * 128, (long)N * H1 * H1 * 256, (long)N * h * h * 2048});
   const long sT1 = std::max((long)N * H1 * H1 * 128, (long)N * h * h * 512);
@@ -449,12 +496,22 @@
       cc(&blk.c2, T1, N, H, H, blk.c2.Ci, T2, blk.c2.Co, 0, nullptr, 0, 1);
       const float* res = cur;
       int res_ld = Cin;
-      if (blk.has_down) {
-        cc(&blk.down, cur, N, H, H, Cin, D, blk.down.Co, 0, nullptr, 0, 0);
-        res = D;
-        res_ld = blk.down.Co;
+      if (blk.has_down && fuse_down) {
+        cc(&blk.fused, T2, N, Ho, Ho, blk.c3.Ci, other, blk.c3.Co, 0, nullptr, 0, 1);
+        ConvCall& c = calls.back();
+        c.x2 = cur;
+        c.Hi2 = c.Wi2 = H;
+        c.Ci2 = Cin;
+        c.stride2 = blk.down.stride;
+        args.back().K += Cin;
+      } else {
+        if (blk.has_down) {
+          cc(&blk.down, cur, N, H, H, Cin, D, blk.down.Co, 0, nullptr, 0, 0);
+          res = D;
+          res_ld = blk.down.Co;
+        }
+        cc(&blk.c3, T2, N, Ho, Ho, blk.c3.Ci, other, blk.c3.Co, 0, res, res_ld, 1);
       }
-      cc(&blk.c3, T2, N, Ho, Ho, blk.c3.Ci, other, blk.c3.Co, 0, res, res_ld, 1);
       if (bi == nbk - 1) last_of_layer[li] = calls.size() - 1;
       std::swap(cur, other);
       H = Ho;
@@ -470,7 +527,9 @@
   for (size_t i = 0; i < calls.size(); ++i) {
     const ConvArgs& a = args[i];
     if (b16 && !calls[i].L->w_b) return fail(CWT_ESTATE, "bf16 conv weights missing (Ci % 64 != 0)");
-    ConvPlan pl = dma ? plan_conv_s(prec, a.M, a.Co, a.K) : plan_conv(a.M, a.Co, a.K);
+    ConvPlan pl = calls[i].x2 ? plan_conv_dual(a.M, a.Co, a.K)
+                  : dma       ? plan_conv_s(prec, a.M, a.Co, a.K)
+                              : plan_conv(a.M, a.Co, a.K);
     plans.push_back(pl);
     if (pl.nsplit > 1) part_floats = std::max(part_floats, (size_t)pl.nsplit * a.M * a.Co);
   }
@@ -511,6 +570,20 @@
     return (c.L->wino_s || c.L->wino4_s) && c.L->k == 3 && c.L->stride == 1 && c.L->pad == c.L->dil &&
            c.x_ld == c.L->Ci;
   };
+  static const int wino_env = getenv("CWT_WINO") && getenv("CWT_WINO")[0] ? atoi(getenv("CWT_WINO")) : -1;
+  auto wino_tile = [&](size_t i) {
+    const ConvArgs& a = args[i];
+    int wm = x6 && wino_env != 0 && c_wino(calls[i])
+                 ? (wino_env == 2 || wino_env == 4 ? wino_env : wino_tile_default(a.Ci, a.Co, a.dil, a.Ho))
+                 : 0;
+    if (wm && !(wm == 4 ? calls[i].L->wino4_s : calls[i].L->wino_s)) wm = 0;
+    return wm;
+  };
+  auto partials_to_wino = [&](size_t i) {
+    return fuse_splitk && i + 1 < n_backbone_calls && plans[i].nsplit > 1 && calls[i].y == T1 && !calls[i].res &&
+           calls[i].y_off == 0 && calls[i].y_ld == args[i].Co && calls[i + 1].x == T1 && !wino_tile(i) &&
+           wino_tile(i + 1) != 0;
+  };
   auto run_call = [&](size_t i) -> int {
     ConvArgs a = args[i];
     const bool keep_res = calls[i].stage == 6;
@@ -520,17 +593,16 @@
       a.relu = 0;
       if (!keep_res) a.res = nullptr;
     }
-    static const int wino_env = getenv("CWT_WINO") && getenv("CWT_WINO")[0] ? atoi(getenv("CWT_WINO")) : -1;
-    int wm = x6 && wino_env != 0 && c_wino(calls[i])
-                 ? (wino_env == 2 || wino_env == 4 ? wino_env : wino_tile_default(a.Ci, a.Co, a.dil, a.Ho))
-                 : 0;
-    if (wm && !(wm == 4 ? calls[i].L->wino4_s : calls[i].L->wino_s)) wm = 0;
+    const int wm = wino_tile(i);
     const bool wino = wm != 0;
+    const bool part_out = partials_to_wino(i), part_in = i > 0 && partials_to_wino(i - 1);
     const WinoGeom wg = wino_geom(a.N, a.Hi, a.Wi, a.dil, wm ? wm : 2);
     const ConvPlan pl = wino ? plan_conv_s(6, (int)wg.T, a.Co, a.Ci, wg.P) : plans[i];
     const double flops = 2.0 * a.M * a.Co * a.K;
     const double eb = b16 ? 2.0 : 4.0, ob = calls[i].out_f32 ? 4.0 : eb;
-    const double bytes = eb * ((double)a.N * a.Hi * a.Wi * a.Ci + (double)a.Co * a.K) +
+    const ConvCall& cl = calls[i];
+    const double bytes = eb * ((double)a.N * a.Hi * a.Wi * a.Ci + (double)a.N * cl.Hi2 * cl.Wi2 * cl.Ci2 +
+                               (double)a.Co * a.K) +
                          ob * ((double)a.M * a.Co + (a.res ? (double)a.M * a.Co : 0.0));
     Prof p(ctx, st,
            std::string(b16 ? "conv_igemm_b16<" : conv_split ? "conv_igemm_x3s<" : wino ? (wm == 4 ? "conv_igemm_x6w4<" : "conv_igemm_x6w<")
@@ -539,15 +611,18 @@
                std::to_string(pl.bn) + "," +
                std::to_string(calls[i].stage) + ">" +
                (pl.nsplit > 1 ? "+splitk" + std::to_string(pl.nsplit) : std::string()) + " " +
-               std::to_string(a.Ci) + "x" + std::to_string(a.Co) + "k" + std::to_string(a.kh) + "s" +
+               std::to_string(a.Ci) + (cl.x2 ? "+" + std::to_string(cl.Ci2) : std::string()) + "x" +
+               std::to_string(a.Co) + "k" + std::to_string(a.kh) + "s" +
                std::to_string(a.stride) + "d" + std::to_string(a.dil) + "@" + std::to_string(a.Ho),
            flops, bytes, calls[i].stage == 6 ? 1 : 2);
     int r;
     if (wino) {
       const ConvCall& c = calls[i];
-      r = run_wino_conv(ctx, c.x, a.N, a.Hi, a.Wi, a.Ci, a.Co, a.dil, wm, wm == 4 ? c.L->wino4_s : c.L->wino_s,
-                        wm == 4 ? c.L->wino4_l : c.L->wino_l, a.scale, a.shift, a.res, c.res_ld, a.relu, c.y, c.y_ld,
-                        c.y_off, c.stage, st);
+      const WinoSplitKSrc sk{part_in ? plans[i - 1].nsplit : 0, part_in ? calls[i - 1].L->scale : nullptr,
+                             part_in ? calls[i - 1].L->shift : nullptr, part_in ? calls[i - 1].relu : 0};
+      r = run_wino_conv(ctx, part_in ? PART : c.x, a.N, a.Hi, a.Wi, a.Ci, a.Co, a.dil, wm,
+                        wm == 4 ? c.L->wino4_s : c.L->wino_s, wm == 4 ? c.L->wino4_l : c.L->wino_l, a.scale, a.shift,
+                        a.res, c.res_ld, a.relu, c.y, c.y_ld, c.y_off, c.stage, st, 0, 0, part_in ? &sk : nullptr);
     } else if (dma) {
       ConvSArgs sa = conv_s_geom(a.N, a.Hi, a.Wi, a.Ci, a.Co, a.kh, a.stride, a.pad, a.dil);
       const ConvCall& c = calls[i];
@@ -568,7 +643,17 @@
         sa.res_s = (const __bf16*)a.res;
       }
       sa.relu = a.relu;
-      r = launch_conv_x3s(sa, pl, c.stage, PART, part_floats, st, prec);
+      if (c.x2) {
+        sa.xs2 = (const __bf16*)c.x2;
+        sa.Hi2 = c.Hi2;
+        sa.Wi2 = c.Wi2;
+        sa.Ci2 = c.Ci2;
+        sa.stride2 = c.stride2;
+        sa.kt_switch = a.Ci / 32;
+        sa.K = a.K;
+      }
+      r = part_out ? launch_conv_x3s_partials(sa, pl, c.stage, PART, part_floats, st, prec)
+                   : launch_conv_x3s(sa, pl, c.stage, PART, part_floats, st, prec);
     } else {
       r = launch_conv(a, pl, calls[i].stage, PART, part_floats, st);
     }
@@ -679,6 +764,10 @@
   if (!rc && tb)
     for (int i = 0; i < 4 && !rc; ++i)
       rc = launch_scale_cols(bb->ppm_q_raw[i], bb->ppm_q[i], 512L * 4608, 512, bb->bott.scale, st);
+  if (!rc && tb)
+    for (int li = 0; li < 4 && !rc; ++li)
+      for (const Block& b : bb->blocks[li])
+        if (b.has_down && !rc) rc = fold_down(b, st);
   return rc;
 }
 
diff --git a/few_shot_seg_cwt_amd/csrc/bn_train.hip b/few_shot_seg_cwt_amd/csrc/bn_train.hip
--- a/few_shot_seg_cwt_amd/csrc/bn_train.hip
+++ b/few_shot_seg_cwt_amd/csrc/bn_train.hip
@@ -182,4 +182,25 @@
   return 0;
 }
 
-}
+__global__ void fold_dual_kernel(const float* __restrict__ w3, const float* __restrict__ s3,
+                                 const float* __restrict__ b3, int K1, const float* __restrict__ wd,
+                                 const float* __restrict__ sd, const float* __restrict__ bd, int K2, int Co,
+                                 float* __restrict__ out, float* __restrict__ shift_out) {
+  const int K = K1 + K2;
+  const long i = (long)blockIdx.x * blockDim.x + threadIdx.x;
+  if (i >= (long)Co * K) return;
+  const int co = (int)(i / K), k = (int)(i - (long)co * K);
+  out[i] = k < K1 ? w3[(long)co * K1 + k] * s3[co] : wd[(long)co * K2 + (k - K1)] * sd[co];
+  if (k == 0) shift_out[co] = b3[co] + bd[co];
+}
+
+int launch_fold_dual(const float* w3, const float* s3, const float* b3, int K1, const float* wd, const float* sd,
+                     const float* bd, int K2, int Co, float* out, float* shift_out, hipStream_t st) {
+  const long n = (long)Co * (K1 + K2);
+  hipLaunchKernelGGL(fold_dual_kernel, dim3(cdiv(n, 256L)), dim3(256), 0, st, w3, s3, b3, K1, wd, sd, bd, K2, Co, out,
+                     shift_out);
+  CWT_LAUNCH_CHECK();
+  return 0;
+}
+
+}
diff --git a/few_shot_seg_cwt_amd/csrc/conv_body.h b/few_shot_seg_cwt_amd/csrc/conv_body.h
--- a/few_shot_seg_cwt_amd/csrc/conv_body.h
+++ b/few_shot_seg_cwt_amd/csrc/conv_body.h
@@ -206,9 +206,24 @@
     i_kx = tap - i_ky * a.kw;
   }
   int i_kt = kt_begin;
-  __amdgpu_buffer_rsrc_t rsA, rsB, rsL;
-  int a_roff[LA], b_voff[LB], l_voff[LBL > 0 ? LBL : 1];
+  constexpr bool DUAL = (PF & 128) != 0;
+  static_assert(!DUAL || (PREC == 6 && (PF & 8) != 0), "dual A source: x6 with buffer addressing");
+  __amdgpu_buffer_rsrc_t rsA, rsB, rsL, rsA2;
+  int a_roff[LA], b_voff[LB], l_voff[LBL > 0 ? LBL : 1], a_roff2[DUAL ? LA : 1];
 #if defined(__HIP_DEVICE_COMPILE__)
+  if constexpr (DUAL) {
+    const int cbl2 = a.Ci2 >> 5;
+    rsA2 = __builtin_amdgcn_make_buffer_rsrc((void*)a.xs2, (short)0, (int)((long)a.N * a.Hi2 * a.Wi2 * cbl2 * 128),
+                                             0x00020000);
+#pragma unroll
+    for (int j = 0; j < LA; ++j) {
+      const int m = m0 + (wv * LA + j) * 8 + lrow;
+      const int n = m / HoWo, rem = m - n * HoWo;
+      const int oh = rem / a.Wo, ow = rem - oh * a.Wo;
+      const int pix2 = (n * a.Hi2 + oh * a.stride2) * a.Wi2 + ow * a.stride2;
+      a_roff2[j] = m < a.M ? (pix2 * cbl2 * 64 + a_ch[j]) * 2 : (int)0x80000000;
+    }
+  }
   if constexpr ((PF & 8) != 0) {
     const int cbl = a.Ci >> (PREC == 1 ? 6 : 5);
     const long a_bytes = (long)a.N * a.Hi * a.Wi * cbl * 128;
@@ -237,12 +252,25 @@
     if constexpr ((PF & 8) != 0) {
       const int dy = i_ky * a.dil, dx = i_kx * a.dil;
       const int uni = ((dy * a.Wi + dx) * cblocks + i_cb) * 128;
-#pragma unroll
-      for (int j = 0; j < LA; ++j) {
-        const int ih = a_ih0[j] + dy, iw = a_iw0[j] + dx;
-        const bool in = (unsigned)ih < (unsigned)a.Hi && (unsigned)iw < (unsigned)a.Wi;
-        __builtin_amdgcn_raw_ptr_buffer_load_lds(rsA, (CWT_LDS void*)(sb + (wv * LA + j) * 1024), 16,
-                                                 in ? a_roff[j] + uni : (int)0x80000000, 0, 0, 0);
+      bool second = false;
+      if constexpr (DUAL) {
+        second = i_kt >= a.kt_switch;
+        if (second) {
+          const unsigned uni2 = (unsigned)(i_kt - a.kt_switch) * 128u;
+#pragma unroll
+          for (int j = 0; j < LA; ++j)
+            __builtin_amdgcn_raw_ptr_buffer_load_lds(rsA2, (CWT_LDS void*)(sb + (wv * LA + j) * 1024), 16,
+                                                     (int)((unsigned)a_roff2[j] + uni2), 0, 0, 0);
+        }
+      }
+      if (!second) {
+#pragma unroll
+        for (int j = 0; j < LA; ++j) {
+          const int ih = a_ih0[j] + dy, iw = a_iw0[j] + dx;
+          const bool in = (unsigned)ih < (unsigned)a.Hi && (unsigned)iw < (unsigned)a.Wi;
+          __builtin_amdgcn_raw_ptr_buffer_load_lds(rsA, (CWT_LDS void*)(sb + (wv * LA + j) * 1024), 16,
+                                                   in ? a_roff[j] + uni : (int)0x80000000, 0, 0, 0);
+        }
       }
 #pragma unroll
       for (int j = 0; j < LB; ++j)
diff --git a/few_shot_seg_cwt_amd/csrc/conv_forms.h b/few_shot_seg_cwt_amd/csrc/conv_forms.h
--- a/few_shot_seg_cwt_amd/csrc/conv_forms.h
+++ b/few_shot_seg_cwt_amd/csrc/conv_forms.h
@@ -31,7 +31,13 @@
   X(128, 128, 12, 4, 1, 2, 16, 0) X(128, 128, 14, 4, 1, 2, 4, 0) X(128, 128, 15, 4, 1, 2, 2, 0) \
   X(128, 128, 16, 4, 1, 2, 6, 0) X(128, 128, 17, 4, 1, 2, 38, 0) X(128, 128, 18, 4, 1, 2, 64, 0) \
                                                 \
-  X(256, 256, 13, 4, 2, 2, 16, 0)
+  X(256, 256, 13, 4, 2, 2, 16, 0)                                                              \
+    \
+    \
+  X(128, 128, 24, 2, 2, 2, 128, 0) X(128, 128, 25, 4, 1, 2, 128, 0)                            \
+  X(128, 64, 25, 4, 1, 2, 128, 0) X(64, 128, 25, 4, 1, 2, 128, 0)
+
+constexpr int kConvDualVar = 20;
 
 struct ConvForm {
   int bm, bn, var, waves_m, waves_n, nstg, pf;
diff --git a/few_shot_seg_cwt_amd/csrc/conv_plans_x6.inc b/few_shot_seg_cwt_amd/csrc/conv_plans_x6.inc
--- a/few_shot_seg_cwt_amd/csrc/conv_plans_x6.inc
+++ b/few_shot_seg_cwt_amd/csrc/conv_plans_x6.inc
@@ -110,3 +110,7 @@
 {206082, 128, 576, 128, 128, 1, 4},
 {337014, 64, 576, 128, 64, 1, 5},
 {337014, 128, 576, 128, 128, 1, 5},
+{28322, 256, 192, 128, 128, 1, 4},
+{7200, 512, 384, 64, 128, 1, 5},
+{7200, 1024, 768, 128, 128, 1, 5},
+{7200, 2048, 1536, 128, 128, 1, 5},
diff --git a/few_shot_seg_cwt_amd/csrc/conv_x3s.hip b/few_shot_seg_cwt_amd/csrc/conv_x3s.hip
--- a/few_shot_seg_cwt_amd/csrc/conv_x3s.hip
+++ b/few_shot_seg_cwt_amd/csrc/conv_x3s.hip
@@ -229,6 +229,17 @@
   }
 }
 
+ConvPlan plan_conv_dual(int M, int Co, int K) {
+  ConvPlan p = plan_conv_s(6, M, Co, K);
+  const ConvForm* f = find_conv_form(6, p.bm, p.bn, p.var);
+  if (!f || !find_conv_form(6, p.bm, p.bn, f->var + kConvDualVar)) {
+    p.bm = 128;
+    p.bn = Co % 128 == 0 ? 128 : 64;
+    p.var = 5;
+  }
+  return p;
+}
+
 template <int PREC>
 static void launch_splitk_s(const ConvSArgs& a, int nsplit, hipStream_t st) {
   const long n = (long)a.M * (a.Co / 8);
@@ -242,13 +253,24 @@
   }
 }
 
-int launch_conv_x3s(ConvSArgs a, const ConvPlan& p, int stage, float* part_ws, size_t part_ws_floats,
-                    hipStream_t st, int prec) {
+static int launch_conv_s(ConvSArgs a, const ConvPlan& p, int stage, float* part_ws, size_t part_ws_floats,
+                         hipStream_t st, int prec, bool reduce) {
   if (prec != 0 && prec != 1 && prec != 3 && prec != 6)
     return fail(CWT_EARG, "conv precision must be 3 (bf16x3), 1 (bf16), 0 (exact fp32) or 6 (bf16x6)");
   const ConvForm* form = find_conv_form(prec, p.bm, p.bn, p.var);
   if (!form) return fail(CWT_EARG, "no such conv form (conv_forms.h)");
   const bool batched = prec == 6 && a.batch > 1;
+  if ((form->pf & 128) != 0) return fail(CWT_EARG, "a dual conv form is named by its base form");
+  if (a.xs2) {
+    if (prec != 6 || batched || a.kh != 1 || a.kw != 1 || a.stride != 1 || a.pad != 0)
+      return fail(CWT_EARG, "two-source conv: an x6 1x1 stride-1 conv only");
+    if (a.Ci2 <= 0 || a.Ci2 % 32 || a.K != a.Ci + a.Ci2 || a.kt_switch != a.Ci / 32 || a.stride2 < 1 ||
+        (a.Ho - 1) * a.stride2 >= a.Hi2 || (a.Wo - 1) * a.stride2 >= a.Wi2 ||
+        (long)a.N * a.Hi2 * a.Wi2 * a.Ci2 * 4 >= (1L << 31))
+      return fail(CWT_EARG, "two-source conv: bad second source");
+    form = find_conv_form(prec, p.bm, p.bn, form->var + kConvDualVar);
+    if (!form) return fail(CWT_EARG, "no dual form on this tile (conv_forms.h)");
+  }
   if ((prec == 0 || prec == 6) && (a.ys || a.res_s || (!a.y && !batched)))
     return fail(CWT_EARG, "fp32-operand conv: fp32 output and residual only");
   if (batched && (p.nsplit != 1 || !a.part || a.kh != 1 || a.kw != 1))
@@ -287,7 +309,7 @@
   else
     launch(FamX3s{});
   CWT_LAUNCH_CHECK();
-  if (nsplit > 1 && !batched) {
+  if (nsplit > 1 && !batched && reduce) {
     main.part = part_ws;
     if (prec == 1)
       launch_splitk_s<1>(main, nsplit, st);
@@ -300,4 +322,34 @@
   return 0;
 }
 
-}
+int launch_splitk_reduce_f32(const float* part, int nsplit, int M, int Co, const float* scale, const float* shift,
+                             int relu, float* y, hipStream_t st) {
+  if (!part || !scale || !shift || !y || nsplit < 1 || M < 1 || Co < 8 || Co % 8)
+    return fail(CWT_EARG, "split-K reduce: Co % 8, nsplit >= 1");
+  ConvSArgs a = {};
+  a.part = (float*)part;
+  a.M = M;
+  a.Co = Co;
+  a.scale = scale;
+  a.shift = shift;
+  a.relu = relu;
+  a.y = y;
+  a.y_ld = Co;
+  launch_splitk_s<0>(a, nsplit, st);
+  CWT_LAUNCH_CHECK();
+  return 0;
+}
+
+int launch_conv_x3s(ConvSArgs a, const ConvPlan& p, int stage, float* part_ws, size_t part_ws_floats,
+                    hipStream_t st, int prec) {
+  return launch_conv_s(a, p, stage, part_ws, part_ws_floats, st, prec, true);
+}
+
+int launch_conv_x3s_partials(ConvSArgs a, const ConvPlan& p, int stage, float* part_ws, size_t part_ws_floats,
+                             hipStream_t st, int prec) {
+  if (p.nsplit < 2 || a.batch > 1) return fail(CWT_EARG, "conv partials: a split-K plan of a single conv only");
+  if (a.res || a.res_s) return fail(CWT_EARG, "conv partials: the consumer's epilogue has no residual");
+  return launch_conv_s(a, p, stage, part_ws, part_ws_floats, st, prec, false);
+}
+
+}
diff --git a/few_shot_seg_cwt_amd/csrc/ctx.h b/few_shot_seg_cwt_amd/csrc/ctx.h
--- a/few_shot_seg_cwt_amd/csrc/ctx.h
+++ b/few_shot_seg_cwt_amd/csrc/ctx.h
@@ -164,12 +164,21 @@
   int res_ld;
   int relu;
   bool out_f32;
+  const float* x2 = nullptr;
+  int Hi2 = 0, Wi2 = 0, Ci2 = 0, stride2 = 0;
+};
+
+struct WinoSplitKSrc {
+  int nsplit;
+  const float *scale, *shift;
+  int relu;
 };
 
 ConvArgs make_args(const ConvCall& c);
 int force_conv_form(int prec, int bm, int bn, int Co, ConvPlan* p);
 int run_wino_conv(cwt_ctx* ctx, const float* x, int N, int H, int W, int Ci, int Co, int d, int m, const __bf16* us,
                   const __bf16* ul, const float* scale, const float* shift, const float* res, int res_ld, int relu,
-                  float* y, int y_ld, int y_off, int stage, hipStream_t st, int bm = 0, int bn = 0);
+                  float* y, int y_ld, int y_off, int stage, hipStream_t st, int bm = 0, int bn = 0,
+                  const WinoSplitKSrc* sk = nullptr);
 
 }
diff --git a/few_shot_seg_cwt_amd/csrc/kernels.h b/few_shot_seg_cwt_amd/csrc/kernels.h
--- a/few_shot_seg_cwt_amd/csrc/kernels.h
+++ b/few_shot_seg_cwt_amd/csrc/kernels.h
@@ -39,6 +39,8 @@
   int relu;
   int batch;
   long xs_bstride, ws_bstride, wl_bstride;
+  const __bf16* xs2;
+  int Hi2, Wi2, Ci2, stride2, kt_switch;
 };
 
 __host__ __device__ __forceinline__ long packed_k(int ci, int tap, int taps) {
@@ -99,6 +101,11 @@
 int launch_conv(ConvArgs a, const ConvPlan& p, int stage, float* part_ws, size_t part_ws_floats, hipStream_t st);
 int launch_splitk_epilogue(const ConvArgs& a, int nsplit, hipStream_t st);
 ConvPlan plan_conv_s(int prec, int M, int Co, int K, int batch = 0);
+ConvPlan plan_conv_dual(int M, int Co, int K);
+int launch_splitk_reduce_f32(const float* part, int nsplit, int M, int Co, const float* scale, const float* shift,
+                             int relu, float* y, hipStream_t st);
+int launch_fold_dual(const float* w3, const float* s3, const float* b3, int K1, const float* wd, const float* sd,
+                     const float* bd, int K2, int Co, float* out, float* shift_out, hipStream_t st);
 struct WinoGeom {
   int N, H, W, d;
   int m;
@@ -109,10 +116,14 @@
 WinoGeom wino_geom(int N, int H, int W, int d, int m = 2);
 int launch_wino_weights(const float* w_packed, int Co, int Ci, float* U, hipStream_t st, int m = 2);
 int launch_wino_in(const float* x, const WinoGeom& g, int Ci, float* V, hipStream_t st);
+int launch_wino_in_splitk(const float* part, int nsplit, const float* scale, const float* shift, int relu,
+                          const WinoGeom& g, int Ci, float* V, hipStream_t st);
 int launch_wino_out(const float* Mb, const WinoGeom& g, int Co, const float* scale, const float* shift, const float* res,
                     int res_ld, int relu, float* y, int y_ld, int y_off, hipStream_t st);
 int launch_conv_x3s(ConvSArgs a, const ConvPlan& p, int stage, float* part_ws, size_t part_ws_floats,
                     hipStream_t st, int prec = 3);
+int launch_conv_x3s_partials(ConvSArgs a, const ConvPlan& p, int stage, float* part_ws, size_t part_ws_floats,
+                             hipStream_t st, int prec);
 int launch_split_act(const float* x, long P, int C, int ld, __bf16* out, hipStream_t st);
 int launch_split_w3(const float* w, long R, int K, __bf16* ws, __bf16* wl, hipStream_t st);
 int launch_occupy(int nwg, int us, hipStream_t st);
diff --git a/few_shot_seg_cwt_amd/csrc/wino.hip b/few_shot_seg_cwt_amd/csrc/wino.hip
--- a/few_shot_seg_cwt_amd/csrc/wino.hip
+++ b/few_shot_seg_cwt_amd/csrc/wino.hip
@@ -108,8 +108,35 @@
   n = (int)(r / g.d);
 }
 
+struct WinoSplitK {
+  const float *scale, *shift;
+  long plane;
+  int ns, relu;
+};
+template <int NS>
+__device__ __forceinline__ f32x4 wino_load(const float* __restrict__ p, const WinoSplitK& k, const f32x4& sc,
+                                           const f32x4& sh) {
+  f32x4 v = *(const f32x4*)p;
+  if constexpr (NS != 1) {
+    const int ns = NS > 0 ? NS : k.ns;
+#pragma unroll
+    for (int s = 1; s < (NS > 0 ? NS : 64); ++s) {
+      if (s >= ns) break;
+      v += *(const f32x4*)(p + s * k.plane);
+    }
+#pragma unroll
+    for (int i = 0; i < 4; ++i) v[i] = fmaf(v[i], sc[i], sh[i]);
+    if (k.relu) {
+#pragma unroll
+      for (int i = 0; i < 4; ++i) v[i] = fmaxf(v[i], 0.f);
+    }
+  }
+  return v;
+}
+
+template <int NS>
 __global__ __launch_bounds__(256) void wino_in_kernel(const float* __restrict__ x, WinoGeom g, int Ci,
-                                                      float* __restrict__ V) {
+                                                      float* __restrict__ V, WinoSplitK k) {
   const int q4 = Ci >> 2;
   const long idx = wino_xcd_index();
   if (idx >= g.T * q4) return;
@@ -117,6 +144,11 @@
   const int c = (int)(idx - t * q4) * 4;
   int n, py, px, ti, tj;
   wino_tile(t, g, n, py, px, ti, tj);
+  f32x4 sc = {}, sh = {};
+  if constexpr (NS != 1) {
+    sc = *(const f32x4*)(k.scale + c);
+    sh = *(const f32x4*)(k.shift + c);
+  }
   f32x4 D[4][4];
 #pragma unroll
   for (int u = 0; u < 4; ++u) {
@@ -125,7 +157,8 @@
     for (int v = 0; v < 4; ++v) {
       const int ix = px + g.d * (2 * tj - 1 + v);
       const bool in = (unsigned)iy < (unsigned)g.H && (unsigned)ix < (unsigned)g.W;
-      D[u][v] = in ? *(const f32x4*)(x + (((long)n * g.H + iy) * g.W + ix) * Ci + c) : f32x4{0.f, 0.f, 0.f, 0.f};
+      D[u][v] = in ? wino_load<NS>(x + (((long)n * g.H + iy) * g.W + ix) * Ci + c, k, sc, sh)
+                   : f32x4{0.f, 0.f, 0.f, 0.f};
     }
   }
   f32x4 R[4][4];
@@ -147,6 +180,7 @@
 }
 
 __device__ __forceinline__ void wino4_bt(const f32x4 d[6], f32x4 r[6]) {
+#pragma clang fp contract(off)
   r[0] = 4.f * d[0] - 5.f * d[2] + d[4];
   r[1] = (d[3] + d[4]) - 4.f * (d[1] + d[2]);
   r[2] = (d[4] - d[3]) + 4.f * (d[1] - d[2]);
@@ -155,8 +189,9 @@
   r[5] = 4.f * d[1] - 5.f * d[3] + d[5];
 }
 
+template <int NS>
 __global__ __launch_bounds__(256) void wino4_in_kernel(const float* __restrict__ x, WinoGeom g, int Ci,
-                                                       float* __restrict__ V) {
+                                                       float* __restrict__ V, WinoSplitK k) {
   const int q4 = Ci >> 2;
   const long idx = wino_xcd_index();
   if (idx >= g.T * q4) return;
@@ -164,6 +199,11 @@
   const int c = (int)(idx - t * q4) * 4;
   int n, py, px, ti, tj;
   wino_tile(t, g, n, py, px, ti, tj);
+  f32x4 sc = {}, sh = {};
+  if constexpr (NS != 1) {
+    sc = *(const f32x4*)(k.scale + c);
+    sh = *(const f32x4*)(k.shift + c);
+  }
   f32x4 R[6][6];
 #pragma unroll
   for (int v = 0; v < 6; ++v) {
@@ -173,7 +213,8 @@
     for (int u = 0; u < 6; ++u) {
       const int iy = py + g.d * (4 * ti - 1 + u);
       const bool in = (unsigned)iy < (unsigned)g.H && (unsigned)ix < (unsigned)g.W;
-      D[u] = in ? *(const f32x4*)(x + (((long)n * g.H + iy) * g.W + ix) * Ci + c) : f32x4{0.f, 0.f, 0.f, 0.f};
+      D[u] = in ? wino_load<NS>(x + (((long)n * g.H + iy) * g.W + ix) * Ci + c, k, sc, sh)
+                : f32x4{0.f, 0.f, 0.f, 0.f};
     }
     f32x4 r[6];
     wino4_bt(D, r);
@@ -191,15 +232,33 @@
   }
 }
 
+template <int NS>
+static void launch_wino_in_ns(const float* x, const WinoGeom& g, int Ci, float* V, const WinoSplitK& k, hipStream_t st) {
+  const long n = g.T * (Ci / 4);
+  if (g.m == 4)
+    hipLaunchKernelGGL(wino4_in_kernel<NS>, dim3((unsigned)cdiv(n, 256)), dim3(256), 0, st, x, g, Ci, V, k);
+  else
+    hipLaunchKernelGGL(wino_in_kernel<NS>, dim3((unsigned)cdiv(n, 256)), dim3(256), 0, st, x, g, Ci, V, k);
+}
+
 int launch_wino_in(const float* x, const WinoGeom& g, int Ci, float* V, hipStream_t st) {
   if (Ci % 4) return fail(CWT_EARG, "wino_in: Ci % 4");
-  const long n = g.T * (Ci / 4);
-  if (g.m == 4)
-    hipLaunchKernelGGL(wino4_in_kernel, dim3((unsigned)cdiv(n, 256)), dim3(256), 0, st, x, g, Ci, V);
-  else if (g.m == 2)
-    hipLaunchKernelGGL(wino_in_kernel, dim3((unsigned)cdiv(n, 256)), dim3(256), 0, st, x, g, Ci, V);
+  if (g.m != 2 && g.m != 4) return fail(CWT_EARG, "winograd: output tile must be 2 or 4");
+  launch_wino_in_ns<1>(x, g, Ci, V, WinoSplitK{}, st);
+  CWT_LAUNCH_CHECK();
+  return 0;
+}
+
+int launch_wino_in_splitk(const float* part, int nsplit, const float* scale, const float* shift, int relu,
+                          const WinoGeom& g, int Ci, float* V, hipStream_t st) {
+  if (Ci % 4) return fail(CWT_EARG, "wino_in: Ci % 4");
+  if (g.m != 2 && g.m != 4) return fail(CWT_EARG, "winograd: output tile must be 2 or 4");
+  if (!part || !scale || !shift || nsplit < 1 || nsplit > 64) return fail(CWT_EARG, "wino_in: bad split-K partials");
+  const WinoSplitK k{scale, shift, (long)g.N * g.H * g.W * Ci, nsplit, relu};
+  if (nsplit == 2)
+    launch_wino_in_ns<2>(part, g, Ci, V, k, st);
   else
-    return fail(CWT_EARG, "winograd: output tile must be 2 or 4");
+    launch_wino_in_ns<0>(part, g, Ci, V, k, st);
   CWT_LAUNCH_CHECK();
   return 0;
 }
diff --git a/include/cwt_debug.h b/include/cwt_debug.h
--- a/include/cwt_debug.h
+++ b/include/cwt_debug.h
@@ -41,6 +41,16 @@
                        const float* res, int res_ld, int relu, float* y, int y_ld, int y_off, int bm, int bn,
                        int nsplit, void* stream);
 
+int cwt_debug_conv_x6_dual(cwt_ctx* ctx, const float* t, int N, int Ho, int Wo, int K1, const float* x, int Hi2,
+                           int Wi2, int K2, int stride2, const float* w3, const float* s3, const float* b3,
+                           const float* wd, const float* sd, const float* bd, int Co, int relu, float* y, int bm,
+                           int bn, int nsplit, void* stream);
+
+int cwt_debug_wino_in(cwt_ctx* ctx, const float* x, int nsplit, const float* scale, const float* shift, int relu,
+                      int N, int H, int W, int C, int d, int m, float* V, void* stream);
+int cwt_debug_splitk_epilogue(cwt_ctx* ctx, const float* part, int nsplit, int M, int Co, const float* scale,
+                              const float* shift, int relu, float* y, void* stream);
+
 int cwt_debug_cp4d_layer(cwt_ctx* ctx, const float* x, int B, int hA, int wA, int hB, int wB, int cin, int cout,
                          const float* Wa, const float* ba, const float* Wb, const float* bb, float* y, int variant,
                          void* stream);
```

Measured after the change: 399.2 episodes/s, median of 6. 2.9% higher.
